# juno181/Ex4DGS

Hardware: AMD Instinct MI355X
Metric: fwd+bwd ms/frame @1M Gaussians 1352x1014; achieved HBM GB/s vs peak (lower is better)
Workload: dtype f32; 1 GPU; cfg3: 1.0M static+dynamic (K=35), 1352x1014; P=1000000, HW=1370928, sh_degree=3, step=GaussianRasterizer forward + backward on a resident frame, parallelism=frame-sharded x1

## Files before the change

### ex4dgs_amd/build.py

```python
import os
import shutil
import subprocess
import sys

from . import isa_check

HERE = os.path.dirname(os.path.abspath(__file__))
CSRC = os.path.join(HERE, "csrc")
LIB = os.path.join(CSRC, "libex4d_hip.so")
ARCH = "gfx950"

SOURCES = {
    "ex4d_preprocess.hip": ["-ffp-contract=off", "-fno-slp-vectorize"],
    "ex4d_binning.hip": [],
    "ex4d_rowsort.hip": [],
    "ex4d_composite.hip": ["-ffp-contract=fast", "-munsafe-fp-atomics", "-fno-slp-vectorize"],
    "ex4d_api.hip": [],
    "ex4d_attributes.hip": ["-ffp-contract=off"],
    "ex4d_loss.hip": [],
    "ex4d_frames.hip": ["-ffp-contract=off"],
    "ex4d_optim.hip": ["-ffp-contract=off"],
    "ex4d_knn.hip": ["-ffp-contract=off"],
    "ex4d_densify.hip": ["-ffp-contract=off"],
    "ex4d_growth.hip": ["-ffp-contract=off"],
    "ex4d_regularizers.hip": ["-ffp-contract=off"],
    "ex4d_trainer.hip": [],
}
COMMON = ["-O3", "-std=c++17", "-fPIC", f"--offload-arch={ARCH}", "-fno-fast-math", "-Wall", "-Wno-unused-function"]


def _hipcc():
    for cand in (shutil.which("hipcc"), "/opt/rocm/bin/hipcc"):
        if cand and os.path.exists(cand):
            return cand
    raise RuntimeError("hipcc not found: libex4d_hip.so cannot be built")


def _without_remarks(text):
    out, skip = [], 0
    for line in text.splitlines():
        if "-Rpass-analysis=kernel-resource-usage" in line:
            skip = 2
            continue
        if skip and (line.strip().startswith("|") or line.split("|")[0].strip().isdigit()):
            skip -= 1
            continue
        skip = 0
        if "remark" in line and "generated" in line:
            continue
        out.append(line + "\n")
    return "".join(out)


def _no_vgpr_spills(src, remarks, obj):
    name, bad = None, []
    for line in remarks.splitlines():
        if "Function Name:" in line:
            name = line.split("Function Name:")[1].split("[")[0].strip()
        elif "VGPRs Spill:" in line:
            n = int(line.split("VGPRs Spill:")[1].split("[")[0])
            if n:
                bad.append((name, n))
    if bad:
        if os.path.exists(obj):
            os.remove(obj)
        raise RuntimeError(f"{src}: vector-register spills in {bad}: restructure the kernel or relax its __launch_bounds__")


shift_amount_in_last_vgpr = isa_check.shift_amount_in_last_vgpr


def _no_shift_amount_in_last_vgpr(src, obj):
    bad = shift_amount_in_last_vgpr(obj)
    if bad:
        os.remove(obj)
        raise RuntimeError(f"{src}: 64-bit shifts with their shift amount in the wave's last vector register (wrong results on gfx950 for waves "
                           f"allocated at the top of the register file): {bad}; change the kernel's __launch_bounds__ / register pressure")


def _no_packed_shift_clamps(src, obj):
    bad = isa_check.packed_shift_clamps(obj)
    if bad:
        os.remove(obj)
        raise RuntimeError(f"{src}: v_ashr_pk_* (its destination's upper 16 bits are used as zero and are not, on gfx950): {bad}; clamp the "
                           f"accumulator before the shift")


def _report_wait_state_violations(src, obj):
    bad = isa_check.wait_state_violations(obj)
    for kernel, rule, cons, prod in bad[:20]:
        sys.stderr.write(f"{src}: wait states: {rule}: `{prod}` -> `{cons}` in {kernel[:60]}\n")
    return bad


def _stale(target, deps):
    if not os.path.exists(target):
        return True
    t = os.path.getmtime(target)
    return any(os.path.getmtime(d) > t for d in deps)


def build(force=False, verbose=False, extra_flags=()):
    hipcc = _hipcc()
    headers = [os.path.join(CSRC, "ex4d_internal.h"), os.path.join(HERE, "..", "include", "ex4d_rasterizer.h"),
               os.path.join(HERE, "..", "include", "ex4d_attributes.h"), os.path.join(HERE, "..", "include", "ex4d_loss.h"), os.path.join(HERE, "..", "include", "ex4d_optim.h"), os.path.join(HERE, "..", "include", "ex4d_knn.h"), os.path.join(HERE, "..", "include", "ex4d_trainer.h"),
               os.path.join(HERE, "..", "include", "ex4d_densify.h"), os.path.join(HERE, "..", "include", "ex4d_regularizers.h"),
               os.path.join(CSRC, "ex4d_reg_rows.h"),
               os.path.abspath(__file__)]
    objs = []
    for src, flags in SOURCES.items():
        s = os.path.join(CSRC, src)
        o = os.path.join(CSRC, src.replace(".hip", ".o"))
        objs.append(o)
        if force or _stale(o, [s] + headers):
            cmd = [hipcc] + COMMON + flags + list(extra_flags) + os.environ.get("EX4D_EXTRA_HIPCC_FLAGS", "").split() + \
                  ["-Rpass-analysis=kernel-resource-usage", "-c", s, "-o", o]
            if verbose:
                print(" ".join(cmd), flush=True)
            r = subprocess.run(cmd, stderr=subprocess.PIPE, text=True)
            remarks = r.stderr or ""
            sys.stderr.write(_without_remarks(remarks))
            if r.returncode:
                raise subprocess.CalledProcessError(r.returncode, cmd)
            _no_vgpr_spills(src, remarks, o)
            _no_shift_amount_in_last_vgpr(src, o)
            _no_packed_shift_clamps(src, o)
            _report_wait_state_violations(src, o)
    if force or _stale(LIB, objs):
        cmd = [hipcc, "-shared", "-fPIC", f"--offload-arch={ARCH}", "-o", LIB] + objs
        if verbose:
            print(" ".join(cmd), flush=True)
        subprocess.check_call(cmd)
    return LIB


if __name__ == "__main__":
    print(build(force="--force" in sys.argv, verbose=True))
```

### ex4dgs_amd/csrc/ex4d_api.hip

```cpp
#include "ex4d_internal.h"
#include <atomic>
#include <cstdarg>
#include <cstdio>
#include <cstdlib>
#include <cstring>
#include <mutex>

namespace {

std::atomic<bool> g_prof_on{false};
std::atomic<int> g_bwd_variant{4};
std::atomic<int> g_tile_ids{0};
std::atomic<int> g_tile_rows{1};
std::atomic<int> g_depth_msd{3};
struct DepthSortWatch {
    std::mutex mu;
    uint32_t *word = nullptr;
    bool tried = false;
    std::atomic<int> hold{0}, backoff{64}, trips{0};
    uint32_t *get()
    {
        std::lock_guard<std::mutex> lock(mu);
        if (!tried) {
            tried = true;
// ... 225 lines not shown
const char *ex4d_target_arch(void) { return "gfx950"; }

size_t ex4d_geom_bytes(int32_t P) { size_t t; carve_geom(nullptr, P, nullptr, &t); return t; }
size_t ex4d_binning_bytes(int32_t R, int32_t W, int32_t H) { size_t t; carve_binning(nullptr, (uint32_t)R, W, H, nullptr, &t); return t; }
size_t ex4d_img_bytes(int32_t W, int32_t H) { size_t t; carve_img(nullptr, W, H, nullptr, &t); return t; }
void ex4d_geom_layout(int32_t P, Ex4dGeomLayout *out) { carve_geom(nullptr, P, out, nullptr); }
void ex4d_binning_layout(int32_t R, int32_t W, int32_t H, Ex4dBinningLayout *out) { carve_binning(nullptr, (uint32_t)R, W, H, out, nullptr); }
void ex4d_img_layout(int32_t W, int32_t H, Ex4dImgLayout *out) { carve_img(nullptr, W, H, out, nullptr); }
size_t ex4d_backward_scratch_bytes(int32_t P) { return ex4d_align_up((size_t)P * 16 * sizeof(float)); }

static int forward_impl(
    const Ex4dParams *prm, ShSplit split,
    const float *background, const float *means3D, const float *dir3D, const float *shs, const float *colors_precomp,
    const float *opacities, const float *scales, const float *rotations, const float *cov3D_precomp,
    const float *viewmatrix, const float *projmatrix, const float *campos, const float *subpixel_offset,
    ex4d_alloc_fn geom_alloc, void *geom_user, ex4d_alloc_fn binning_alloc, void *binning_user,
    ex4d_alloc_fn img_alloc, void *img_user,
    float *out_color, int32_t *radii, float *out_depth, float *out_acc, float *out_flow, int32_t *out_idx,
    void *stream_, int32_t *num_rendered)
{
    g_err[0] = 0;
    hipStream_t stream = (hipStream_t)stream_;
    if (!prm || !num_rendered) return fail(EX4D_ERR_ARG, "null params");
    const int P = prm->P, W = prm->W, H = prm->H;
    if (P <= 0 || W <= 0 || H <= 0) return fail(EX4D_ERR_ARG, "P, W, H must be positive (P == 0 is handled by the caller)");
    if (!means3D || !opacities || !background || !viewmatrix || !projmatrix || !campos)
        return fail(EX4D_ERR_ARG, "means3D, opacities, background, viewmatrix, projmatrix, campos are required");
    const bool is_split = split.rest[0] != nullptr || split.rest[1] != nullptr;
    if (((shs != nullptr || is_split) ? 1 : 0) + (colors_precomp != nullptr ? 1 : 0) != 1 || (shs != nullptr && is_split))
        return fail(EX4D_ERR_ARG, "Please provide excatly one of either SHs or precomputed colors!");
    if (is_split && prm->M != 16) return fail(EX4D_ERR_ARG, "split SH needs M == 16 (dc [n,1,3] + rest [n,15,3])");
    if (((scales == nullptr || rotations == nullptr) && cov3D_precomp == nullptr) ||
        ((scales != nullptr || rotations != nullptr) && cov3D_precomp != nullptr))
        return fail(EX4D_ERR_ARG, "Please provide exactly one of either scale/rotation pair or precomputed 3D covariance!");
    if (shs && prm->M < (prm->D + 1) * (prm->D + 1)) return fail(EX4D_ERR_ARG, "sh has fewer coefficients than the active degree needs");
    if (!out_color || !radii || !out_depth || !out_acc || !out_flow || !out_idx) return fail(EX4D_ERR_ARG, "null output");
    const int gx = (W + EX4D_TILE - 1) / EX4D_TILE, gy = (H + EX4D_TILE - 1) / EX4D_TILE;
    const int T = gx * gy;
    const bool async = prm->instance_capacity > 0;
    if (prm->instance_capacity < 0) return fail(EX4D_ERR_ARG, "instance_capacity must be >= 0");
    if (async && prm->debug) return fail(EX4D_ERR_ARG, "debug (synchronise after every stage) and instance_capacity > 0 (asynchronous forward) exclude each other");

    void *geom_buf = geom_alloc(geom_user, ex4d_geom_bytes(P));
    if (!geom_buf) return fail(EX4D_ERR_ALLOC, "geometry buffer allocation failed");
    GeomState g = carve_geom(geom_buf, P, nullptr, nullptr);
    void *img_buf = img_alloc(img_user, ex4d_img_bytes(W, H));
    if (!img_buf) return fail(EX4D_ERR_ALLOC, "image buffer allocation failed");
    ImgState im = carve_img(img_buf, W, H, nullptr, nullptr);

    uint32_t key_base = 0, key_invisible = 0xFFFFFFFFu;
    int key_bits = 32;
    if (prm->min_depth >= 0.0f && prm->max_depth > prm->min_depth && prm->max_depth < 3.0e38f) {
        uint32_t lo, hi;
        memcpy(&lo, &prm->min_depth, 4); memcpy(&hi, &prm->max_depth, 4);
        key_base = lo;
        key_invisible = hi - lo + 1u;
        key_bits = 1;
        while (key_bits < 32 && (key_invisible >> key_bits) != 0u) key_bits++;
    }
    const bool packed_rects = gx <= 255 && gy <= 255;
    int msd_mode = g_depth_msd.load(std::memory_order_relaxed);
    uint32_t *msd_watch = nullptr;
    if (!(packed_rects && ex4d_depth_sort_msd_applies((uint32_t)P, key_bits))) msd_mode = 0;
    else if (msd_mode == 3) msd_mode = depth_sort_auto_msd(stream, async, &msd_watch) ? 2 : 0;
    const bool msd_depth = msd_mode != 0;
    int msd_bits = ex4d_depth_sort_msd_bits((uint32_t)P, key_bits);
    {
        const int forced = g_depth_msd_bits.load(std::memory_order_relaxed);
        if (forced == EX4D_DLS_MSD_BITS || (forced == EX4D_DLS_MSD_BITS - 1 && ex4d_depth_sort_msd_bits(1u, key_bits) == forced)) msd_bits = forced;
    }
    const bool start_in_b = (ex4d_radix_passes((uint32_t)P, key_bits) & 1) != 0;
    uint32_t *keys0 = start_in_b ? g.sort_keys_b : g.sort_keys_a, *vals0 = start_in_b ? g.sort_vals_b : g.depth_order;
    uint32_t *keys1 = start_in_b ? g.sort_keys_a : g.sort_keys_b, *vals1 = start_in_b ? g.depth_order : g.sort_vals_b;
    if (msd_depth) { keys0 = g.sort_keys_a; vals0 = g.sort_vals_a; }

    HIP_TRY(ex4d_prepare_rank_lds(stream));
    g_prof.begin(0, stream);
    if (async) HIP_TRY(ex4d_launch_zero(g.total, 8 * sizeof(uint32_t), stream));
    GeomState gw = g;
    if (!g_geom_debug.load(std::memory_order_relaxed)) {
        gw.cov3D = nullptr; gw.tiles_touched = nullptr;
        if (packed_rects) gw.rects = nullptr;
    }
    STAGE(ex4d_launch_preprocess_fwd(*prm, means3D, dir3D, scales, rotations, opacities, shs, cov3D_precomp, colors_precomp,
                                     viewmatrix, projmatrix, campos, radii, gw, g.total + 1, split,
                                     keys0, (uint32_t *)nullptr, key_base, key_invisible, packed_rects ? g.rects4 : nullptr, stream,
                                     msd_depth ? reinterpret_cast<uint32_t *>(g.key_ranges) : nullptr, async), prm, stream);
    MARK(0, "preprocess_fwd");
    const size_t nblk = (size_t)(P + 63) / 64;
    const size_t rb_words = (size_t)(g.block_totals - g.total) + 2 * nblk;
    if (!async) {
        if (!g_readback.init(rb_words)) return fail(EX4D_ERR_HIP, "pinned read-back buffer allocation failed");
        if (g_readback_side.load(std::memory_order_relaxed)) {
            HIP_TRY(hipEventRecord(g_readback.ev_pre, stream));
            HIP_TRY(hipStreamWaitEvent(g_readback.side, g_readback.ev_pre, 0));
            HIP_TRY(hipMemcpyAsync(g_readback.host, g.total, rb_words * sizeof(uint32_t), hipMemcpyDeviceToHost, g_readback.side));
            HIP_TRY(hipEventRecord(g_readback.ev, g_readback.side));
        } else {
            HIP_TRY(hipMemcpyAsync(g_readback.host, g.total, rb_words * sizeof(uint32_t), hipMemcpyDeviceToHost, stream));
            HIP_TRY(hipEventRecord(g_readback.ev, stream));
        }
    }
    const bool rows_sort = g_tile_rows.load(std::memory_order_relaxed) != 0 && ex4d_tile_sort_rows_applies(P, gx, gy);
    const bool fused_scan = msd_mode == 2 && !rows_sort;
    const bool lsd_gather = !msd_depth && rows_sort && packed_rects;
    if (msd_depth) {
        STAGE(ex4d_depth_sort_msd(g.sort_keys_a, g.sort_vals_a, g.rects4, g.sort_keys_b, g.depth_order, g.rects4_b, (uint32_t)P, key_invisible,
                                  g.total, g.key_ranges, g.sort_hist, g.bucket_starts, (uint32_t)g_depth_local_cap.load(std::memory_order_relaxed), stream,
                                  fused_scan ? g.sorted_offsets : nullptr, fused_scan ? g.bucket_sums : nullptr, T, (fused_scan || rows_sort) ? im.ranges : nullptr,
                                  g_depth_local_threads.load(std::memory_order_relaxed), msd_watch, msd_bits), prm, stream);
        MARK(0, "depth_sort");
        if (!fused_scan && !rows_sort) {
            STAGE(ex4d_launch_scan_tiles(P, nullptr, g.rects4_b, nullptr, nullptr, g.sorted_offsets, g.scan_block_sums, T, im.ranges, async ? g.total : nullptr, stream), prm, stream);
            MARK(0, "scan_tiles");
        }
    } else {
        bool in_first = true;
        STAGE(ex4d_radix_sort_pairs(keys0, vals0, keys1, vals1, (uint32_t)P, key_bits, g.sort_hist, &in_first, stream, nullptr, true,
                                    lsd_gather ? g.rects4 : nullptr, lsd_gather ? g.rects4_b : nullptr, lsd_gather ? im.ranges : nullptr, T), prm, stream);
        if (in_first == start_in_b) return fail(EX4D_ERR_HIP, "internal: depth sort ended in the wrong buffer");
        MARK(0, "depth_sort");
        if (!lsd_gather) {
            STAGE(ex4d_launch_scan_tiles(P, g.rects, packed_rects ? g.rects4 : nullptr, g.depth_order, g.sorted_rects, g.sorted_offsets, g.scan_block_sums, T, im.ranges, async ? g.total : nullptr, stream), prm, stream);
            MARK(0, "scan_tiles");
        }
    }
    const uint2 *dup_rects = (msd_depth || lsd_gather) ? nullptr : g.sorted_rects;
    const uint32_t *dup_rects4 = (msd_depth || lsd_gather) ? g.rects4_b : nullptr;
    uint32_t R = 0;
    uint32_t segment_sum = 0;
    const uint32_t *n_dev = nullptr;
    bool has_flow;
    if (async) {
        static_assert(sizeof(Ex4dFrameStatus) == 8 * sizeof(uint32_t), "Ex4dFrameStatus mirrors the first eight frame-flag words");
        const bool count_later = fused_scan || (rows_sort && msd_depth) || lsd_gather;
        if (!count_later) HIP_TRY(hipMemcpyAsync(num_rendered, g.total, sizeof(Ex4dFrameStatus), hipMemcpyDefault, stream));
        R = (uint32_t)prm->instance_capacity;
        segment_sum = 0;
        n_dev = g.total;
        has_flow = prm->assume_no_flow == 0;
    } else {
        {
            static const bool spin = []{ const char *e = getenv("EX4D_READBACK_SPIN"); return e ? atoi(e) != 0 : true; }();
            if (spin) {
                hipError_t q = hipErrorNotReady;
                for (int i = 0; i < 20000 && (q = hipEventQuery(g_readback.ev)) == hipErrorNotReady; i++) { }
                if (q == hipErrorNotReady) q = hipEventSynchronize(g_readback.ev);
                HIP_TRY(q);
            } else HIP_TRY(hipEventSynchronize(g_readback.ev));
        }
        uint32_t instance_sum = 0;
        uint32_t chunk_flags = 0;
        for (size_t i = 0; i < nblk; i++) {
            const uint32_t seg = g_readback.host[(size_t)(g.block_totals - g.total) + 2 * i + 1];
            instance_sum += g_readback.host[(size_t)(g.block_totals - g.total) + 2 * i];
            segment_sum += seg & 0x3FFFFFFFu;
            chunk_flags |= seg;
        }
        has_flow = (chunk_flags & EX4D_CHUNK_FLOW) != 0u;
        if (prm->prefiltered && (chunk_flags & EX4D_CHUNK_FILTERED))
            return fail(EX4D_ERR_PREFILTERED, "Point is filtered although prefiltered is set. This shouldn't happen!");
        R = instance_sum;
        if (R > 0x7FFFFFFFu) return fail(EX4D_ERR_ARG, "more than 2^31-1 tile instances");
        *num_rendered = (int32_t)R;
    }

    void *bin_buf = binning_alloc(binning_user, ex4d_binning_bytes((int32_t)R, W, H));
    if (!bin_buf) return fail(EX4D_ERR_ALLOC, "binning buffer allocation failed");
    BinState b = carve_binning(bin_buf, R, W, H, nullptr, nullptr);

    const int passes = ex4d_radix_passes(R, tile_bits(T));
    uint32_t *k0 = (passes % 2 == 0) ? b.tile_ids : b.keys_tmp;
    uint32_t *v0 = (passes % 2 == 0) ? b.point_list : b.vals_tmp;
    uint32_t *k1 = (passes % 2 == 0) ? b.keys_tmp : b.tile_ids;
    uint32_t *v1 = (passes % 2 == 0) ? b.vals_tmp : b.point_list;
    if (rows_sort) {
        if (R > 0) {
            STAGE(ex4d_tile_sort_rows(P, gx, gy, g.depth_order, dup_rects4, dup_rects, b.keys_tmp, b.point_list,
                                      g_tile_ids.load(std::memory_order_relaxed) ? b.tile_ids : nullptr, R, segment_sum, g.row_hist, b.sort_hist, im.ranges,
                                      (async && (msd_depth || lsd_gather)) ? g.total : nullptr, stream), prm, stream);
        }
        if (async && (msd_depth || lsd_gather)) HIP_TRY(hipMemcpyAsync(num_rendered, g.total, sizeof(Ex4dFrameStatus), hipMemcpyDefault, stream));
        MARK(0, "tile_sort");
    } else if (R > 0 && ex4d_tile_sort_msd_applies(P, tile_bits(T))) {
        STAGE(ex4d_launch_duplicate(P, W, H, g.depth_order, g.sorted_offsets, g.scan_block_sums, dup_rects, dup_rects4, b.tile_ids, b.vals_tmp, R, stream,
                                    fused_scan ? g.sort_keys_b : nullptr, g.total + EX4D_FLAG_DPARAMS, g.bucket_sums, g.total, msd_bits), prm, stream);
        if (async && fused_scan) HIP_TRY(hipMemcpyAsync(num_rendered, g.total, sizeof(Ex4dFrameStatus), hipMemcpyDefault, stream));
        MARK(0, "duplicate");
        STAGE(ex4d_tile_sort_msd(b.tile_ids, b.vals_tmp, b.keys_tmp, b.point_list, g_tile_ids.load(std::memory_order_relaxed) ? b.tile_ids : nullptr,
                                 R, tile_bits(T), b.sort_hist, im.ranges, stream, n_dev), prm, stream);
        MARK(0, "tile_sort");
        MARK(0, "tile_ranges");
    } else {
// ... 74 lines not shown
                        viewmatrix, projmatrix, campos, subpixel_offset, geom_alloc, geom_user, binning_alloc, binning_user,
                        img_alloc, img_user, out_color, radii, out_depth, out_acc, out_flow, out_idx, stream_, num_rendered);
}

static bool split_ok(const Ex4dParams *prm, const float *const dc[2], const float *const rest[2], int n_static)
{
    if (!prm || n_static < 0 || n_static > prm->P) return false;
    if (n_static > 0 && (!dc[0] || !rest[0])) return false;
    if (n_static < prm->P && (!dc[1] || !rest[1])) return false;
    return true;
}

int ex4d_forward_split_sh(
    const Ex4dParams *prm, const float *background, const float *means3D, const float *dir3D, const Ex4dSplitSH *shs,
    const float *opacities, const float *scales, const float *rotations, const float *cov3D_precomp,
    const float *viewmatrix, const float *projmatrix, const float *campos, const float *subpixel_offset,
    ex4d_alloc_fn geom_alloc, void *geom_user, ex4d_alloc_fn binning_alloc, void *binning_user,
    ex4d_alloc_fn img_alloc, void *img_user,
    float *out_color, int32_t *radii, float *out_depth, float *out_acc, float *out_flow, int32_t *out_idx,
    void *stream_, int32_t *num_rendered)
{
    g_err[0] = 0;
    if (!shs || !split_ok(prm, shs->dc, shs->rest, shs->n_static)) return fail(EX4D_ERR_ARG, "split SH: null tensor or n_static outside [0, P]");
    const ShSplit sp = { { shs->dc[0], shs->dc[1] }, { shs->rest[0], shs->rest[1] }, shs->n_static };
    return forward_impl(prm, sp, background, means3D, dir3D, nullptr, nullptr, opacities, scales, rotations, cov3D_precomp,
                        viewmatrix, projmatrix, campos, subpixel_offset, geom_alloc, geom_user, binning_alloc, binning_user,
                        img_alloc, img_user, out_color, radii, out_depth, out_acc, out_flow, out_idx, stream_, num_rendered);
}

int ex4d_backward(
    const Ex4dParams *prm, int32_t num_rendered,
    const float *background, const float *means3D, const int32_t *radii,
    const float *shs, const float *colors_precomp, const float *scales, const float *rotations,
    const float *cov3D_precomp, const float *viewmatrix, const float *projmatrix, const float *campos,
    const float *subpixel_offset, const float *out_depth, const float *out_acc,
    const void *geom_buffer, const void *binning_buffer, const void *img_buffer,
    const float *dL_dout_color, const float *dL_dout_depth, const float *dL_dout_flow, const float *dL_dout_acc,
    float *dL_dmeans2D, float *dL_dcolors, float *dL_dopacity, float *dL_dmeans3D, float *dL_dcov3D, float *dL_dsh,
    float *dL_dscales, float *dL_drotations, float *dL_ddir, void *bwd_scratch, void *stream_)
{
    return backward_impl(prm, kNoSplit, kNoSplitGrad, num_rendered, background, means3D, radii, shs, colors_precomp, scales, rotations,
                         cov3D_precomp, viewmatrix, projmatrix, campos, subpixel_offset, out_depth, out_acc, geom_buffer, binning_buffer,
                         img_buffer, dL_dout_color, dL_dout_depth, dL_dout_flow, dL_dout_acc, dL_dmeans2D, dL_dcolors, dL_dopacity,
                         dL_dmeans3D, dL_dcov3D, dL_dsh, dL_dscales, dL_drotations, dL_ddir, bwd_scratch, stream_);
}

int ex4d_backward_split_sh(
    const Ex4dParams *prm, int32_t num_rendered,
    const float *background, const float *means3D, const int32_t *radii,
    const Ex4dSplitSH *shs, const float *scales, const float *rotations,
    const float *cov3D_precomp, const float *viewmatrix, const float *projmatrix, const float *campos,
    const float *subpixel_offset, const float *out_depth, const float *out_acc,
    const void *geom_buffer, const void *binning_buffer, const void *img_buffer,
    const float *dL_dout_color, const float *dL_dout_depth, const float *dL_dout_flow, const float *dL_dout_acc,
    float *dL_dmeans2D, float *dL_dcolors, float *dL_dopacity, float *dL_dmeans3D, float *dL_dcov3D, const Ex4dSplitSHGrad *dL_dsh,
    float *dL_dscales, float *dL_drotations, float *dL_ddir, void *bwd_scratch, void *stream_)
{
    g_err[0] = 0;
    if (!shs || !dL_dsh || !split_ok(prm, shs->dc, shs->rest, shs->n_static) || dL_dsh->n_static != shs->n_static ||
        !split_ok(prm, (const float *const *)dL_dsh->dc, (const float *const *)dL_dsh->rest, dL_dsh->n_static))
        return fail(EX4D_ERR_ARG, "split SH: null tensor, n_static outside [0, P] or mismatching gradient split");
    if (prm->M != 16) return fail(EX4D_ERR_ARG, "split SH needs M == 16 (dc [n,1,3] + rest [n,15,3])");
    const ShSplit sp = { { shs->dc[0], shs->dc[1] }, { shs->rest[0], shs->rest[1] }, shs->n_static };
    const ShSplitGrad gsp = { { dL_dsh->dc[0], dL_dsh->dc[1] }, { dL_dsh->rest[0], dL_dsh->rest[1] }, dL_dsh->n_static };
    return backward_impl(prm, sp, gsp, num_rendered, background, means3D, radii, nullptr, nullptr, scales, rotations,
                         cov3D_precomp, viewmatrix, projmatrix, campos, subpixel_offset, out_depth, out_acc, geom_buffer, binning_buffer,
                         img_buffer, dL_dout_color, dL_dout_depth, dL_dout_flow, dL_dout_acc, dL_dmeans2D, dL_dcolors, dL_dopacity,
                         dL_dmeans3D, dL_dcov3D, nullptr, dL_dscales, dL_drotations, dL_ddir, bwd_scratch, stream_);
}

int ex4d_set_option(const char *name, int value)
{
    if (name && !strcmp(name, "composite_bwd_variant") && (value == 4 || value == 8)) { g_bwd_variant.store(value); return EX4D_OK; }
    if (name && !strcmp(name, "composite_fwd_asm") && (value == 0 || value == 1)) { ex4d_set_fwd_asm(value); return EX4D_OK; }
    if (name && !strcmp(name, "binning_tile_ids") && (value == 0 || value == 1)) { g_tile_ids.store(value); return EX4D_OK; }
    if (name && !strcmp(name, "composite_clamp_always") && (value == 0 || value == 1)) { ex4d_set_clamp_always(value); return EX4D_OK; }
    if (name && !strcmp(name, "composite_bwd_pairs") && (value == 0 || value == 1)) { ex4d_set_bwd_pairs(value); return EX4D_OK; }
    if (name && !strcmp(name, "tile_sort_rows") && (value == 0 || value == 1)) { g_tile_rows.store(value); return EX4D_OK; }
    if (name && !strcmp(name, "rank_lds_atomics") && value >= -1 && value <= 1) { ex4d_set_rank_lds(value); return EX4D_OK; }
    if (name && !strcmp(name, "rows_probe")) { ex4d_set_rows_probe(value); return EX4D_OK; }
    if (name && !strcmp(name, "preprocess_sh_predicate") && (value == 0 || value == 1)) { ex4d_set_preprocess_tune(value); return EX4D_OK; }
    if (name && !strcmp(name, "geom_debug_arrays") && (value == 0 || value == 1)) { g_geom_debug.store(value); return EX4D_OK; }
    if (name && !strcmp(name, "preprocess_fast_path") && (value == 0 || value == 1)) { ex4d_set_preprocess_fast(value); return EX4D_OK; }
    if (name && !strcmp(name, "depth_sort_msd") && value >= 0 && value <= 3) { g_depth_msd.store(value); g_depth_watch.reset(); return EX4D_OK; }
    if (name && !strcmp(name, "depth_sort_local_cap") && value >= 0 && value <= 8192) { g_depth_local_cap.store(value); return EX4D_OK; }
    if (name && !strcmp(name, "readback_side_stream") && (value == 0 || value == 1)) { g_readback_side.store(value); return EX4D_OK; }
    if (name && !strcmp(name, "depth_sort_msd_bits") && (value == 0 || value == EX4D_DLS_MSD_BITS - 1 || value == EX4D_DLS_MSD_BITS)) { g_depth_msd_bits.store(value); return EX4D_OK; }
    if (name && !strcmp(name, "depth_sort_local_threads") && (value == 0 || value == 256 || value == 512)) { g_depth_local_threads.store(value); return EX4D_OK; }
    return fail(EX4D_ERR_ARG, "unknown option or value out of range");
}

int ex4d_debug_bwd_stats(unsigned long long *out8, int reset) { return ex4d_bwd_stats(out8, 8, reset) == hipSuccess ? EX4D_OK : EX4D_ERR_HIP; }
int ex4d_debug_rows_prof(unsigned long long *out8, int reset) { return ex4d_rows_prof(out8, reset) == hipSuccess ? EX4D_OK : EX4D_ERR_HIP; }
int ex4d_debug_bwd_stats16(unsigned long long *out16, int reset) { return ex4d_bwd_stats(out16, 16, reset) == hipSuccess ? EX4D_OK : EX4D_ERR_HIP; }

int ex4d_get_option(const char *name)
{
    if (name && !strcmp(name, "composite_bwd_variant")) return g_bwd_variant.load();
    if (name && !strcmp(name, "composite_fwd_asm")) return ex4d_get_fwd_asm();
    if (name && !strcmp(name, "binning_tile_ids")) return g_tile_ids.load();
    if (name && !strcmp(name, "composite_clamp_always")) return ex4d_get_clamp_always();
    if (name && !strcmp(name, "composite_bwd_pairs")) return ex4d_get_bwd_pairs();
    if (name && !strcmp(name, "tile_sort_rows")) return g_tile_rows.load();
    if (name && !strcmp(name, "rank_lds_atomics")) return ex4d_get_rank_lds();
    if (name && !strcmp(name, "rank_lds_atomics_in_use")) return ex4d_rank_lds_in_use();
    if (name && !strcmp(name, "preprocess_sh_predicate")) return ex4d_get_preprocess_tune();
    if (name && !strcmp(name, "geom_debug_arrays")) return g_geom_debug.load();
    if (name && !strcmp(name, "preprocess_fast_path")) return ex4d_get_preprocess_fast();
    if (name && !strcmp(name, "depth_sort_msd")) return g_depth_msd.load();
    if (name && !strcmp(name, "depth_sort_hold")) return g_depth_watch.hold.load();
    if (name && !strcmp(name, "depth_sort_trips")) return g_depth_watch.trips.load();
    if (name && !strcmp(name, "depth_sort_local_cap")) return g_depth_local_cap.load();
    if (name && !strcmp(name, "readback_side_stream")) return g_readback_side.load();
    if (name && !strcmp(name, "depth_sort_msd_bits")) return g_depth_msd_bits.load();
    if (name && !strcmp(name, "depth_sort_local_threads")) return g_depth_local_threads.load();
    return -1;
}

void ex4d_profile_enable(int on) { g_prof_on.store(on != 0); }

int ex4d_profile_read(int which, float *ms, const char **names, int max_stages)
{
    std::lock_guard<std::mutex> lock(g_prof.mu);
    if (which < 0 || which > 1 || !g_prof.created) return 0;
    const int n = g_prof.n[which] < max_stages ? g_prof.n[which] : max_stages;
    if (n == 0) return 0;
    if (hipEventSynchronize(g_prof.ev[which][g_prof.n[which]]) != hipSuccess) return 0;
    for (int i = 0; i < n; i++) {
        float t = 0.f;
        (void)hipEventElapsedTime(&t, g_prof.ev[which][i], g_prof.ev[which][i + 1]);
        ms[i] = t;
        if (names) names[i] = g_prof.names[which][i];
    }
    return n;
}

int ex4d_mark_visible(int32_t P, const float *means3D, const float *viewmatrix, const float *projmatrix,
                      float min_depth, float max_depth, uint8_t *present, void *stream_)
{
    g_err[0] = 0;
    if (P <= 0) return EX4D_OK;
    if (!means3D || !viewmatrix || !projmatrix || !present) return fail(EX4D_ERR_ARG, "null argument");
    HIP_TRY(ex4d_launch_mark_visible(P, means3D, viewmatrix, projmatrix, min_depth, max_depth, present, (hipStream_t)stream_));
    return EX4D_OK;
}

}
```

### ex4dgs_amd/csrc/ex4d_binning.hip

```cpp
#include "ex4d_internal.h"
#include <atomic>
#include <mutex>

__device__ int ex4d_g_rank_lds = 0;

namespace {

__global__ __launch_bounds__(256) void lds_rank_probe_kernel(uint32_t seed, int trials, int ndigits, uint32_t *__restrict__ bad)
{
    __shared__ uint32_t cnt[4][256];
    const int lane = threadIdx.x & 63, wave = threadIdx.x >> 6;
    uint32_t x = seed ^ (blockIdx.x * 0x9E3779B9u) ^ (threadIdx.x * 0x85EBCA6Bu);
    uint32_t nb = 0;
    for (int t = 0; t < trials; t++) {
        for (int i = lane; i < 256; i += 64) cnt[wave][i] = 0;
        __builtin_amdgcn_fence(__ATOMIC_RELEASE, "wavefront"); __builtin_amdgcn_wave_barrier(); __builtin_amdgcn_fence(__ATOMIC_ACQUIRE, "wavefront");
        x = x * 1664525u + 1013904223u;
        const uint32_t d = (x >> 16) % (uint32_t)ndigits;
        uint32_t expect = 0, same = 0;
        for (int l = 0; l < 64; l++) { const uint32_t dl = __shfl(d, l, 64); if (dl == d) { same++; if (l < lane) expect++; } }
        const uint32_t got = atomicAdd(&cnt[wave][d], 1u);
        const uint32_t got2 = atomicAdd(&cnt[wave][d], 1u);
        if (got != expect || got2 != same + expect) nb++;
    }
    if (nb) atomicAdd(bad, nb);
}

__device__ __forceinline__ int to_int_sat(float f)
{
    if (f != f) return 0;
    if (f >= 2147483648.0f) return 2147483647;
    if (f <= -2147483648.0f) return (-2147483647 - 1);
    return (int)f;
}

template <int ITEMS, int BINS, int COPIES>
__global__ __launch_bounds__(RS_THREADS) void rs_histogram_kernel(const uint32_t *__restrict__ keys, uint32_t n, int shift,
    uint32_t mask, uint32_t nblocks, uint32_t *__restrict__ hist, const uint32_t *__restrict__ n_dev)
{
    if (n_dev) { const uint32_t nd = *n_dev; n = nd < n ? nd : n; }
    __shared__ uint32_t h_all[COPIES * (BINS + 1)];
    uint32_t *h = h_all + (COPIES > 1 ? (threadIdx.x % COPIES) * (BINS + 1) : 0);
    for (int b = threadIdx.x; b < COPIES * (BINS + 1); b += RS_THREADS) h_all[b] = 0;
    __syncthreads();
    const uint32_t base = blockIdx.x * (RS_THREADS * ITEMS);
    if (base < n) {
        uint32_t k[ITEMS];
#pragma unroll
        for (int it = 0; it < ITEMS; it++) {
            const uint32_t i = base + it * RS_THREADS + threadIdx.x;
            k[it] = keys[i < n ? i : n - 1];
        }
#pragma unroll
        for (int it = 0; it < ITEMS; it++) {
            const uint32_t i = base + it * RS_THREADS + threadIdx.x;
            if (i < n) atomicAdd(&h[(k[it] >> shift) & mask], 1u);
        }
    }
    __syncthreads();
    for (int b = threadIdx.x; b < BINS; b += RS_THREADS) {
        uint32_t c = 0;
#pragma unroll
        for (int k = 0; k < COPIES; k++) c += h_all[k * (BINS + 1) + b];
        hist[(size_t)b * nblocks + blockIdx.x] = c;
    }
}

__global__ __launch_bounds__(256) void rs_scan_rows_kernel(uint32_t nblocks, uint32_t *__restrict__ hist, uint32_t bins)
{
    __shared__ uint32_t wave_sums[4];
    __shared__ uint32_t carry_s;
    uint32_t *row = hist + (size_t)blockIdx.x * nblocks;
    const int lane = threadIdx.x & 63, wave = threadIdx.x >> 6;
    const bool vec = ((((uintptr_t)row) & 15) == 0);
    if (threadIdx.x == 0) carry_s = 0;
    __syncthreads();
    for (uint32_t base = 0; base < nblocks; base += 2048) {
        const uint32_t i0 = base + 8 * threadIdx.x;
        uint32_t v[8];
        if (vec && i0 + 8 <= nblocks) {
            const uint4 a = *reinterpret_cast<const uint4 *>(row + i0), b = *reinterpret_cast<const uint4 *>(row + i0 + 4);
            v[0] = a.x; v[1] = a.y; v[2] = a.z; v[3] = a.w; v[4] = b.x; v[5] = b.y; v[6] = b.z; v[7] = b.w;
        } else {
#pragma unroll
            for (int k = 0; k < 8; k++) v[k] = (i0 + k < nblocks) ? row[i0 + k] : 0u;
        }
        uint32_t run = 0;
#pragma unroll
        for (int k = 0; k < 8; k++) { const uint32_t t = v[k]; v[k] = run; run += t; }
        uint32_t x = run;
#pragma unroll
        for (int o = 1; o < 64; o <<= 1) { uint32_t y = __shfl_up(x, o, 64); if (lane >= o) x += y; }
        if (lane == 63) wave_sums[wave] = x;
        __syncthreads();
        uint32_t woff = carry_s + x - run;
        for (int w = 0; w < wave; w++) woff += wave_sums[w];
        if (vec && i0 + 8 <= nblocks) {
            *reinterpret_cast<uint4 *>(row + i0) = make_uint4(woff + v[0], woff + v[1], woff + v[2], woff + v[3]);
            *reinterpret_cast<uint4 *>(row + i0 + 4) = make_uint4(woff + v[4], woff + v[5], woff + v[6], woff + v[7]);
        } else {
#pragma unroll
            for (int k = 0; k < 8; k++) if (i0 + k < nblocks) row[i0 + k] = woff + v[k];
        }
        __syncthreads();
        if (threadIdx.x == 255) carry_s = woff + run;
        __syncthreads();
    }
    if (threadIdx.x == 0) hist[(size_t)bins * nblocks + blockIdx.x] = carry_s;
}

struct DlsParams { uint32_t kmin, shift, inv_key; };
__device__ __forceinline__ DlsParams dls_params(const uint32_t *__restrict__ dparams) { return { dparams[0], dparams[1], dparams[2] }; }
__device__ __forceinline__ uint32_t dls_digit(uint32_t key, const DlsParams &q, uint32_t bins) { return key == q.inv_key ? bins - 1u : (key - q.kmin) >> q.shift; }

__device__ __forceinline__ DlsParams dls_reduce_ranges(const uint2 *__restrict__ ranges, uint32_t nranges, uint32_t inv_key, uint32_t bins, uint32_t *s_red )
{
    uint32_t kmax = 0u, nkmin = 0u;
    for (uint32_t base = 0; base < nranges; base += 8u * RS_THREADS) {
        uint2 p[8];
#pragma unroll
        for (int j = 0; j < 8; j++) { const uint32_t i = base + j * RS_THREADS + threadIdx.x; p[j] = i < nranges ? ranges[i] : make_uint2(0u, 0u); }
#pragma unroll
        for (int j = 0; j < 8; j++) { kmax = p[j].x > kmax ? p[j].x : kmax; nkmin = p[j].y > nkmin ? p[j].y : nkmin; }
    }
#pragma unroll
    for (int o = 32; o > 0; o >>= 1) {
        const uint32_t a = __shfl_xor(kmax, o, 64), b = __shfl_xor(nkmin, o, 64);
        kmax = a > kmax ? a : kmax; nkmin = b > nkmin ? b : nkmin;
    }
    if ((threadIdx.x & 63) == 0) { s_red[threadIdx.x >> 6] = kmax; s_red[4 + (threadIdx.x >> 6)] = nkmin; }
    __syncthreads();
    for (int w = 0; w < RS_THREADS / 64; w++) { kmax = s_red[w] > kmax ? s_red[w] : kmax; nkmin = s_red[4 + w] > nkmin ? s_red[4 + w] : nkmin; }
    uint32_t kmin = ~nkmin, shift = 0;
    if (kmax == 0u) kmin = 0u;
    else {
        const uint32_t range = kmax - kmin;
        while ((range >> shift) > bins - 2u) shift++;
    }
    return { kmin, shift, inv_key };
}

template <int ITEMS, int BINS>
__global__ __launch_bounds__(RS_THREADS) void dls_histogram_kernel(const uint32_t *__restrict__ keys, uint32_t n, uint32_t nblocks,
    uint32_t *__restrict__ hist, uint32_t *__restrict__ dparams, const uint2 *__restrict__ ranges, uint32_t nranges, uint32_t inv_key)
{
    __shared__ uint32_t h[BINS];
    __shared__ uint32_t s_red[8];
    for (int b = threadIdx.x; b < BINS; b += RS_THREADS) h[b] = 0;
    const uint32_t base = blockIdx.x * (RS_THREADS * ITEMS);
    uint32_t k[ITEMS];
    if (base < n) {
#pragma unroll
        for (int it = 0; it < ITEMS; it++) {
            const uint32_t i = base + it * RS_THREADS + threadIdx.x;
            k[it] = keys[i < n ? i : n - 1];
        }
    }
    const DlsParams q = dls_reduce_ranges(ranges, nranges, inv_key, (uint32_t)BINS, s_red);
    if (blockIdx.x == 0 && threadIdx.x == 0) { dparams[0] = q.kmin; dparams[1] = q.shift; dparams[2] = q.inv_key; dparams[3] = 0u; }
    if (base < n) {
#pragma unroll
        for (int it = 0; it < ITEMS; it++) {
            const uint32_t i = base + it * RS_THREADS + threadIdx.x;
            if (i < n) atomicAdd(&h[dls_digit(k[it], q, BINS)], 1u);
        }
    }
    __syncthreads();
    for (int b = threadIdx.x; b < BINS; b += RS_THREADS) hist[(size_t)b * nblocks + blockIdx.x] = h[b];
}

typedef Ex4dTsBlock TsBlock;
__device__ __forceinline__ TsBlock ts_block_from_table(const Ex4dTsBlock *__restrict__ table, uint32_t b)
{
    const uint2 *p = reinterpret_cast<const uint2 *>(table + b);
    const uint2 a = p[0], c = p[1], e = p[2];
    return { a.x, a.y, c.x, c.y, e.x, e.y };
}
struct TsLocateLds { uint32_t cnt[257], fb[257], st[257], wave_sums[8]; };
__device__ __forceinline__ TsBlock ts_locate_block(const uint32_t *__restrict__ totals, int nbuckets, uint32_t b, TsLocateLds &L)
{
    const int tid = threadIdx.x, lane = tid & 63, wave = tid >> 6;
    const uint32_t cnt = tid < nbuckets ? totals[tid] : 0u;
    const uint32_t nblk = (cnt + RS_CHUNK - 1) / RS_CHUNK;
    uint32_t x = cnt, y = nblk;
#pragma unroll
    for (int o = 1; o < 64; o <<= 1) { const uint32_t a = __shfl_up(x, o, 64), c = __shfl_up(y, o, 64); if (lane >= o) { x += a; y += c; } }
    if (lane == 63) { L.wave_sums[wave] = x; L.wave_sums[4 + wave] = y; }
    __syncthreads();
    uint32_t st = x - cnt, fb = y - nblk;
    for (int w = 0; w < wave; w++) { st += L.wave_sums[w]; fb += L.wave_sums[4 + w]; }
    L.cnt[tid] = cnt; L.fb[tid] = fb; L.st[tid] = st;
    if (tid == 255) { L.fb[256] = fb + nblk; L.st[256] = st + cnt; L.cnt[256] = 0; }
    __syncthreads();
    TsBlock t = { 0u, 0u, 0u, 0u, 0u, 0u };
    if (b < L.fb[256]) {
        uint32_t h = 0;
#pragma unroll
        for (uint32_t step = 128; step > 0; step >>= 1) if (L.fb[h + step] <= b) h += step;
        const uint32_t within = (b - L.fb[h]) * RS_CHUNK;
        t.start = L.st[h] + within;
        t.count = L.cnt[h] - within < RS_CHUNK ? L.cnt[h] - within : RS_CHUNK;
        t.bucket = h; t.fb_first = L.fb[h]; t.fb_next = L.fb[h + 1]; t.bucket_start = L.st[h];
    }
    return t;
}
template <int ITEMS, int BINS, int MODE, int NBITS>
__global__ __launch_bounds__(RS_THREADS) void rs_scatter_kernel(const uint32_t *__restrict__ keys_in,
    const uint32_t *__restrict__ vals_in, uint32_t *__restrict__ keys_out, uint32_t *__restrict__ vals_out,
    uint32_t n, int shift, int nbits, uint32_t nblocks, const uint32_t *__restrict__ hist,
    int low_bits, const uint32_t *__restrict__ bucket_totals, int nbuckets, uint2 *__restrict__ ranges, const uint32_t *__restrict__ n_dev,
    const uint32_t *__restrict__ rects_in = nullptr, uint32_t *__restrict__ rects_out = nullptr, uint32_t *__restrict__ bucket_starts = nullptr,
    const uint32_t *__restrict__ dparams = nullptr, uint32_t range_stride = 0, uint32_t out_cap = 0xFFFFFFFFu,
    const Ex4dTsBlock *__restrict__ block_table = nullptr)
{
    if (n_dev) { const uint32_t nd = *n_dev; n = nd < n ? nd : n; }
    if (MODE == 0 && ranges) for (uint32_t i = blockIdx.x * RS_THREADS + threadIdx.x; i < range_stride; i += gridDim.x * RS_THREADS) ranges[i] = make_uint2(0u, 0u);
    if (MODE != 2 && blockIdx.x * (uint32_t)(RS_THREADS * ITEMS) >= n) return;
    __shared__ uint32_t wave_cnt[4][BINS];
    __shared__ uint32_t local_start[BINS];
    __shared__ uint32_t global_base[BINS];
    __shared__ uint32_t scan_tmp[8];
    constexpr int STAGE_WORDS = (MODE == 2 ? 1 : 2) * RS_THREADS * ITEMS;
    __shared__ __attribute__((aligned(16))) uint32_t stage_w[STAGE_WORDS];
    uint2 *const stage = reinterpret_cast<uint2 *>(stage_w);
    __shared__ uint32_t stage_r[MODE == 3 ? RS_THREADS * ITEMS : 1];
    static_assert(sizeof(TsLocateLds) <= sizeof(uint32_t) * STAGE_WORDS, "the block table's scratch lives in the staging area");
    static_assert(sizeof(uint32_t) * (4 * BINS + 2 * BINS + 8) + sizeof(uint32_t) * STAGE_WORDS + sizeof(uint32_t) * (MODE == 3 ? RS_THREADS * ITEMS : 1) <= 80 * 1024,
                  "rs_scatter_kernel: static LDS beyond 80 KB (two workgroups per CU)");
    const int tid = threadIdx.x, lane = tid & 63, wave = tid >> 6;
    if (NBITS > 0) nbits = NBITS;
    const uint32_t mask = (1u << nbits) - 1u;
    const int nbins = 1 << nbits;
    DlsParams dq = { 0u, 0u, 0u };
    if (MODE == 3) dq = dls_params(dparams);
    auto digit_of = [&](uint32_t k) -> uint32_t { return MODE == 3 ? dls_digit(k, dq, (uint32_t)BINS) : ((k >> shift) & mask); };
    for (int i = lane; i < BINS; i += 64) wave_cnt[wave][i] = 0;
    __builtin_amdgcn_fence(__ATOMIC_RELEASE, "wavefront");
    __builtin_amdgcn_wave_barrier();
    __builtin_amdgcn_fence(__ATOMIC_ACQUIRE, "wavefront");

    const bool lds_rank = ex4d_g_rank_lds != 0;
    constexpr uint32_t CHUNK = RS_THREADS * ITEMS;
    uint32_t block_first = blockIdx.x * CHUNK, block_end = n, bucket = 0;
    TsBlock tb = { 0u, 0u, 0u, 0u, 0u, 0u };
    if (MODE == 2) {
        if (block_table) tb = ts_block_from_table(block_table, blockIdx.x);
        else {
            TsLocateLds &loc = *reinterpret_cast<TsLocateLds *>(stage_w);
            tb = ts_locate_block(bucket_totals, nbuckets, blockIdx.x, loc);
            __syncthreads();
        }
        if (tb.count == 0) return;
        block_first = tb.start; block_end = tb.start + tb.count; bucket = tb.bucket;
        if (block_first >= out_cap) return;
        if (block_end > out_cap) block_end = out_cap;
    }
    const uint32_t base = block_first + wave * (CHUNK / 4);
    const uint64_t lt = (1ull << lane) - 1ull;
    constexpr int BPT_PRE = BINS / RS_THREADS;
    uint32_t pre_pf[BPT_PRE], pre_gt[BPT_PRE], pre_hb[BPT_PRE];
#pragma unroll
    for (int k = 0; k < BPT_PRE; k++) {
        const int d = tid * BPT_PRE + k;
        const bool live = d < nbins;
        if (MODE == 2) {
            pre_pf[k] = live ? hist[(size_t)d * nblocks + tb.fb_first] : 0u;
            pre_gt[k] = live ? hist[(size_t)d * nblocks + tb.fb_next] : 0u;
        } else {
            pre_pf[k] = 0u;
            pre_gt[k] = live ? hist[(size_t)BINS * nblocks + d] : 0u;
        }
        pre_hb[k] = live ? hist[(size_t)d * nblocks + blockIdx.x] : 0u;
    }
    uint32_t key[ITEMS], val[ITEMS], pos[ITEMS], rct[MODE == 3 ? ITEMS : 1];
#pragma unroll
    for (int it = 0; it < ITEMS; it++) {
        const uint32_t i = base + it * 64 + lane;
        const uint32_t ic = i < block_end ? i : block_end - 1;
        key[it] = keys_in[ic];
        val[it] = (MODE == 2) ? 0u : (vals_in ? vals_in[ic] : ic);
        if constexpr (MODE == 3) rct[it] = rects_in[ic];
    }
#pragma unroll
    for (int it = 0; it < ITEMS; it++) {
        const uint32_t i = base + it * 64 + lane;
        const bool valid = i < block_end;
        const uint32_t d = digit_of(key[it]);
        if (lds_rank) {
            pos[it] = valid ? atomicAdd(&wave_cnt[wave][d], 1u) : 0u;
            continue;
        }
        const uint64_t vmask = __builtin_amdgcn_ballot_w64(valid);
        uint32_t plo = (uint32_t)vmask, phi = (uint32_t)(vmask >> 32);
        if (NBITS > 0) {
#pragma unroll
            for (int b = 0; b < NBITS; b++) {
                const uint64_t bal = __builtin_amdgcn_ballot_w64((d & (1u << b)) != 0u);
                uint32_t flip;
                asm("v_cndmask_b32_e64 %0, -1, 0, %1" : "=v"(flip) : "s"(bal));
                plo &= (uint32_t)bal ^ flip;
                phi &= (uint32_t)(bal >> 32) ^ flip;
            }
        } else {
            for (int b = 0; b < nbits; b++) {
                const uint32_t bit = (d >> b) & 1u;
                const uint64_t bal = __builtin_amdgcn_ballot_w64(bit != 0u);
                const uint32_t flip = bit - 1u;
                plo &= (uint32_t)bal ^ flip;
                phi &= (uint32_t)(bal >> 32) ^ flip;
            }
// ... 229 lines not shown
        lo += nbits;
    }
    if (sv != xv) {
        for (uint32_t i = tid; i < n; i += DLS_THREADS) { xv[i] = sv[i]; xr[i] = sr[i]; }
    }
}

__device__ __forceinline__ uint32_t rect4_count(uint32_t r) { return ((r >> 16) & 0xFFu) * (r >> 24); }
template <int THREADS>
__device__ __forceinline__ uint32_t dls_scan_chunk(DlsLds<THREADS> &L, uint32_t cn, uint32_t carry)
{
    constexpr int DLS_WAVES = THREADS / 64;
    const int tid = threadIdx.x, lane = tid & 63, wave = tid >> 6;
    uint32_t v[DLS_ITEMS], run = 0;
#pragma unroll
    for (int q = 0; q < DLS_ITEMS; q++) { const uint32_t i = tid * DLS_ITEMS + q; run += (i < cn) ? L.buf[i] : 0u; v[q] = run; }
    uint32_t x = run;
#pragma unroll
    for (int o = 1; o < 64; o <<= 1) { const uint32_t y = __shfl_up(x, o, 64); if (lane >= o) x += y; }
    if (lane == 63) L.scan_tmp[wave] = x;
    __syncthreads();
    uint32_t excl = carry + x - run, total = 0;
    for (int w = 0; w < DLS_WAVES; w++) { const uint32_t t = L.scan_tmp[w]; if (w < wave) excl += t; total += t; }
#pragma unroll
    for (int q = 0; q < DLS_ITEMS; q++) { const uint32_t i = tid * DLS_ITEMS + q; if (i < cn) L.buf[i] = excl + v[q]; }
    __syncthreads();
    return total;
}
template <int THREADS>
__device__ __forceinline__ uint32_t dls_scan_from_memory(DlsLds<THREADS> &L, const uint32_t *rects, uint32_t *local_incl, uint32_t n)
{
    constexpr int DLS_THREADS = THREADS, DLS_CAP = THREADS * DLS_ITEMS;
    const int tid = threadIdx.x;
    uint32_t carry = 0;
    for (uint32_t c0 = 0; c0 < n; c0 += DLS_CAP) {
        const uint32_t cn = (n - c0) < DLS_CAP ? (n - c0) : DLS_CAP;
        uint32_t r[DLS_ITEMS];
#pragma unroll
        for (int j = 0; j < DLS_ITEMS; j++) { const uint32_t p = tid + j * DLS_THREADS; r[j] = p < cn ? rects[c0 + p] : 0u; }
#pragma unroll
        for (int j = 0; j < DLS_ITEMS; j++) { const uint32_t p = tid + j * DLS_THREADS; if (p < cn) L.buf[p] = rect4_count(r[j]); }
        __syncthreads();
        carry += dls_scan_chunk(L, cn, carry);
#pragma unroll
        for (int j = 0; j < DLS_ITEMS; j++) { const uint32_t p = tid + j * DLS_THREADS; if (p < cn) local_incl[c0 + p] = L.buf[p]; }
        __syncthreads();
    }
    return carry;
}

template <int THREADS, int NBITS>
__device__ __forceinline__ void dls_lds_pass(DlsLds<THREADS> &L, uint32_t n, uint32_t m, int sh, int nbits)
{
    const int tid = threadIdx.x, lane = tid & 63, wave = tid >> 6;
    if (NBITS > 0) nbits = NBITS;
    const uint32_t mask = (1u << nbits) - 1u;
    const uint32_t wbase = wave * m;
    for (int i = lane; i < (1 << nbits); i += 64) L.cnt[wave][i] = 0;
    dls_wave_sync();
    uint32_t word[DLS_ITEMS], pos[DLS_ITEMS];
#pragma unroll
    for (int it = 0; it < DLS_ITEMS; it++) {
        word[it] = 0u; pos[it] = 0u;
        if ((uint32_t)(it * 64) < m) {
            const uint32_t i = wbase + it * 64 + lane;
            const bool valid = i < n;
            word[it] = valid ? L.buf[i] : 0u;
            pos[it] = dls_rank<NBITS>(L.cnt[wave], (word[it] >> sh) & mask, nbits, valid, lane);
        }
    }
    __syncthreads();
    dls_scan_counts(L, nbits);
#pragma unroll
    for (int it = 0; it < DLS_ITEMS; it++) {
        if ((uint32_t)(it * 64) < m) {
            const uint32_t i = wbase + it * 64 + lane;
            if (i < n) L.buf[L.cnt[wave][(word[it] >> sh) & mask] + pos[it]] = word[it];
        }
    }
    __syncthreads();
}

template <int THREADS>
__global__ __launch_bounds__(THREADS, THREADS == 512 ? 4 : 5) void depth_local_sort_kernel(uint32_t *kb, uint32_t *vb, uint32_t *rb, uint32_t *ka, uint32_t *va, uint32_t *ra,
    const uint32_t *__restrict__ starts, const uint32_t *__restrict__ totals, const uint32_t *__restrict__ dparams, uint32_t cap,
    uint32_t *__restrict__ local_incl, uint32_t *__restrict__ bucket_sums, int T, uint2 *__restrict__ ranges, uint32_t *__restrict__ watch)
{
    constexpr int DLS_THREADS = THREADS, DLS_WAVES = THREADS / 64, DLS_CAP = THREADS * DLS_ITEMS, IDX_BITS = DlsLds<THREADS>::IDX_BITS;
    __shared__ DlsLds<THREADS> L;
    const uint32_t b = blockIdx.x;
    const int tid = threadIdx.x;
    if (ranges) for (int i = b * DLS_THREADS + tid; i < T; i += gridDim.x * DLS_THREADS) ranges[i] = make_uint2(0u, 0u);
    const uint32_t n = totals[b], s = starts[b];
    const DlsParams dq = dls_params(dparams);
    const int rem = (int)dq.shift;
    const uint32_t inv_digit = gridDim.x - 1u;
    if (b == inv_digit || n == 0u) {
        if (bucket_sums && tid == 0) bucket_sums[b] = 0u;
        return;
    }
    const bool sorted_already = n < 2u || rem == 0;
    if (sorted_already || n > cap) {
        if (n > cap && watch && tid == 0) __hip_atomic_store(watch, 1u, __ATOMIC_RELAXED, __HIP_MEMORY_SCOPE_SYSTEM);
        if (!sorted_already) {
            dls_sort_through_memory(L, kb + s, vb + s, rb + s, ka + s, va + s, ra + s, n, rem, dq.kmin); __threadfence(); __syncthreads();
        }
        if (local_incl) {
            const uint32_t sum = dls_scan_from_memory(L, rb + s, local_incl + s, n);
            if (tid == 0) bucket_sums[b] = sum;
        }
        return;
    }
    const uint32_t remmask = (1u << rem) - 1u;
    {
        uint32_t k[DLS_ITEMS];
#pragma unroll
        for (int j = 0; j < DLS_ITEMS; j++) { const uint32_t p = tid + j * DLS_THREADS; k[j] = p < n ? kb[s + p] : 0u; }
#pragma unroll
        for (int j = 0; j < DLS_ITEMS; j++) { const uint32_t p = tid + j * DLS_THREADS; if (p < n) L.buf[p] = (((k[j] - dq.kmin) & remmask) << IDX_BITS) | p; }
    }
    __syncthreads();
    const int npass = (rem + 8) / 9;
    const uint32_t m = ((n + DLS_WAVES * 64 - 1) / (DLS_WAVES * 64)) * 64;
    if (rem == 16) { dls_lds_pass<THREADS, 8>(L, n, m, IDX_BITS, 8); dls_lds_pass<THREADS, 8>(L, n, m, IDX_BITS + 8, 8); }
    else if (rem == 17) { dls_lds_pass<THREADS, 9>(L, n, m, IDX_BITS, 9); dls_lds_pass<THREADS, 8>(L, n, m, IDX_BITS + 9, 8); }
    else {
        for (int pass = 0, lo = 0; pass < npass; pass++) {
            const int nbits = dls_pass_bits(rem, lo, npass, pass);
            dls_lds_pass<THREADS, 0>(L, n, m, IDX_BITS + lo, nbits);
            lo += nbits;
        }
    }
    uint32_t v[DLS_ITEMS], r[DLS_ITEMS];
#pragma unroll
    for (int j = 0; j < DLS_ITEMS; j++) {
        const uint32_t p = tid + j * DLS_THREADS;
        v[j] = 0u; r[j] = 0u;
        if (p < n) { const uint32_t idx = L.buf[p] & (DLS_CAP - 1u); v[j] = vb[s + idx]; r[j] = rb[s + idx]; }
    }
    asm volatile("s_waitcnt vmcnt(0)" ::: "memory");
    __syncthreads();
#pragma unroll
    for (int j = 0; j < DLS_ITEMS; j++) {
        const uint32_t p = tid + j * DLS_THREADS;
        if (p < n) { vb[s + p] = v[j]; rb[s + p] = r[j]; if (local_incl) L.buf[p] = rect4_count(r[j]); }
    }
    if (local_incl) {
        __syncthreads();
        const uint32_t sum = dls_scan_chunk(L, n, 0u);
#pragma unroll
        for (int j = 0; j < DLS_ITEMS; j++) { const uint32_t p = tid + j * DLS_THREADS; if (p < n) local_incl[s + p] = L.buf[p]; }
        if (tid == 0) bucket_sums[b] = sum;
    }
}

__device__ __forceinline__ uint2 unpack_rect(uint32_t p) { return make_uint2((p & 0xFFu) | (((p >> 8) & 0xFFu) << 16), ((p >> 16) & 0xFFu) | ((p >> 24) << 16)); }
__global__ __launch_bounds__(256) void scan_tiles_local_kernel(int P, const uint2 *__restrict__ rects, const uint32_t *__restrict__ rects4,
    const uint32_t *__restrict__ order, uint2 *__restrict__ sorted_rects, uint32_t *__restrict__ out, uint32_t *__restrict__ block_sums,
    int T, uint2 *__restrict__ ranges, uint32_t *__restrict__ frame_total)
{
    for (int i = blockIdx.x * 256 + threadIdx.x; i < T; i += gridDim.x * 256) ranges[i] = make_uint2(0u, 0u);
    __shared__ uint32_t cnt[SCAN_CHUNK];
    __shared__ uint32_t wave_sums[4];
    const int lane = threadIdx.x & 63, wave = threadIdx.x >> 6;
    const int block_first = blockIdx.x * SCAN_CHUNK;
#pragma unroll
    for (int it = 0; it < SCAN_CHUNK / 256; it++) {
        const int i = block_first + it * 256 + threadIdx.x;
        uint2 rc = make_uint2(0u, 0u);
        if (i < P) { rc = rects4 ? unpack_rect(rects4[order ? order[i] : (uint32_t)i]) : rects[order[i]]; if (sorted_rects) sorted_rects[i] = rc; }
        cnt[it * 256 + threadIdx.x] = (rc.y & 0xFFFFu) * (rc.y >> 16);
    }
    __syncthreads();
    uint32_t v[8];
    uint32_t run = 0;
#pragma unroll
    for (int k = 0; k < 8; k++) { run += cnt[threadIdx.x * 8 + k]; v[k] = run; }
    uint32_t x = run;
#pragma unroll
// ... 120 lines not shown
}

__global__ __launch_bounds__(256) void zero_fill_kernel(uint4 *__restrict__ p, size_t n16, uint32_t tail_words)
{
    const uint4 z = make_uint4(0u, 0u, 0u, 0u);
    for (size_t i = (size_t)blockIdx.x * 256 + threadIdx.x; i < n16; i += (size_t)gridDim.x * 256) p[i] = z;
    if (blockIdx.x == 0 && threadIdx.x < tail_words) reinterpret_cast<uint32_t *>(p + n16)[threadIdx.x] = 0u;
}

__global__ __launch_bounds__(256) void tile_ranges_kernel(uint32_t R, const uint32_t *__restrict__ tile_ids, uint2 *__restrict__ ranges,
    const uint32_t *__restrict__ n_dev)
{
    if (n_dev) { const uint32_t nd = *n_dev; R = nd < R ? nd : R; }
    const uint32_t i = blockIdx.x * 256 + threadIdx.x;
    if (i >= R) return;
    const uint32_t cur = tile_ids[i];
    if (i == 0) ranges[cur].x = 0;
    else {
        const uint32_t prev = tile_ids[i - 1];
        if (cur != prev) { ranges[prev].y = i; ranges[cur].x = i; }
    }
    if (i == R - 1) ranges[cur].y = R;
}

}

static std::atomic<int> g_rank_lds_option{-1};
static std::mutex g_rank_lds_mu;
static int g_rank_lds_device = -1, g_rank_lds_value = 0;
void ex4d_set_rank_lds(int v) { std::lock_guard<std::mutex> lock(g_rank_lds_mu); g_rank_lds_option.store(v); g_rank_lds_device = -1; }
int ex4d_get_rank_lds() { return g_rank_lds_option.load(); }
int ex4d_rank_lds_in_use() { return g_rank_lds_value; }
hipError_t ex4d_prepare_rank_lds(hipStream_t stream)
{
    int dev = -1;
    if (hipGetDevice(&dev) != hipSuccess) return hipGetLastError();
    std::lock_guard<std::mutex> lock(g_rank_lds_mu);
    if (dev == g_rank_lds_device) return hipSuccess;
    hipStreamCaptureStatus st = hipStreamCaptureStatusNone;
    if (hipStreamIsCapturing(stream, &st) == hipSuccess && st != hipStreamCaptureStatusNone) return hipSuccess;
    (void)hipGetLastError();
    int want = g_rank_lds_option.load();
    if (want < 0) {
        uint32_t *bad = nullptr, h = 1;
        hipError_t e = hipMalloc((void **)&bad, sizeof(uint32_t));
        if (e != hipSuccess) return e;
        (void)hipMemset(bad, 0, sizeof(uint32_t));
        for (int nd : { 1, 3, 17, 64, 256 })
            hipLaunchKernelGGL(lds_rank_probe_kernel, dim3(256), dim3(256), 0, 0, 0x5EEDu + nd, 200, nd, bad);
        e = hipMemcpy(&h, bad, sizeof(uint32_t), hipMemcpyDeviceToHost);
        (void)hipFree(bad);
        if (e != hipSuccess) return e;
        want = h == 0u ? 1 : 0;
    }
    hipError_t e = hipMemcpyToSymbol(HIP_SYMBOL(ex4d_g_rank_lds), &want, sizeof(int));
    if (e != hipSuccess) return e;
    g_rank_lds_device = dev; g_rank_lds_value = want;
    return hipSuccess;
}

#define RS_SMALL_ITEMS 8
static inline int rs_items_for(uint32_t n) { return n <= (2u << 20) ? RS_SMALL_ITEMS : RS_ITEMS; }
static inline uint32_t rs_blocks_for(uint32_t n) { const uint32_t c = RS_THREADS * rs_items_for(n); return (n + c - 1) / c; }
static inline int rs_max_bits_for(uint32_t n) { return rs_items_for(n) == RS_SMALL_ITEMS ? 9 : 8; }
size_t ex4d_radix_hist_words(uint32_t n) { return (size_t)1024 * rs_blocks_for(n) + 1024; }
int ex4d_radix_passes(uint32_t n, int end_bit) { const int mb = rs_max_bits_for(n); return (end_bit + mb - 1) / mb; }

hipError_t ex4d_radix_sort_pairs(uint32_t *keys_a, uint32_t *vals_a, uint32_t *keys_b, uint32_t *vals_b,
    uint32_t n, int end_bit, uint32_t *hist, bool *result_in_a, hipStream_t stream, const uint32_t *n_dev, bool iota_values,
    const uint32_t *gather_in, uint32_t *gather_out, uint2 *zero_ranges, int num_ranges)
{
    *result_in_a = true;
    if (n == 0) return hipSuccess;
    const uint32_t nb = rs_blocks_for(n);
    const bool small = rs_items_for(n) == RS_SMALL_ITEMS;
    uint32_t *kin = keys_a, *vin = iota_values ? nullptr : vals_a, *kout = keys_b, *vout = vals_b;
    uint32_t *vnext = vals_a;
    const int npass = ex4d_radix_passes(n, end_bit);
    for (int pass = 0, shift = 0; pass < npass; pass++) {
        const int nbits = (end_bit - shift + (npass - pass) - 1) / (npass - pass);
        const uint32_t mask = (1u << nbits) - 1u;
        if (small) {
            hipLaunchKernelGGL((rs_histogram_kernel<RS_SMALL_ITEMS, 512, 1>), dim3(nb), dim3(RS_THREADS), 0, stream, kin, n, shift, mask, nb, hist, n_dev);
            hipLaunchKernelGGL(rs_scan_rows_kernel, dim3(1u << nbits), dim3(256), 0, stream, nb, hist, 512u);
            const bool last = pass == npass - 1;
#define RS_SMALL_SCATTER(NB) hipLaunchKernelGGL((rs_scatter_kernel<RS_SMALL_ITEMS, 512, 0, NB>), dim3(nb), dim3(RS_THREADS), 0, stream, kin, vin, kout, vout, n, shift, nbits, nb, hist, 0, nullptr, 0, \
                last ? zero_ranges : (uint2 *)nullptr, n_dev, last ? gather_in : (const uint32_t *)nullptr, last ? gather_out : (uint32_t *)nullptr, (uint32_t *)nullptr, (const uint32_t *)nullptr, (uint32_t)num_ranges)
            if (nbits == 9) RS_SMALL_SCATTER(9); else if (nbits == 8) RS_SMALL_SCATTER(8); else RS_SMALL_SCATTER(0);
#undef RS_SMALL_SCATTER
        } else {
            hipLaunchKernelGGL((rs_histogram_kernel<RS_ITEMS, 256, 1>), dim3(nb), dim3(RS_THREADS), 0, stream, kin, n, shift, mask, nb, hist, n_dev);
            hipLaunchKernelGGL(rs_scan_rows_kernel, dim3(1u << nbits), dim3(256), 0, stream, nb, hist, 256u);
            const bool last = pass == npass - 1;
            hipLaunchKernelGGL((rs_scatter_kernel<RS_ITEMS, 256, 0, 0>), dim3(nb), dim3(RS_THREADS), 0, stream, kin, vin, kout, vout, n, shift, nbits, nb, hist, 0, nullptr, 0,
                last ? zero_ranges : (uint2 *)nullptr, n_dev, last ? gather_in : (const uint32_t *)nullptr, last ? gather_out : (uint32_t *)nullptr, (uint32_t *)nullptr, (const uint32_t *)nullptr, (uint32_t)num_ranges);
        }
        uint32_t *t = kin; kin = kout; kout = t;
        t = (pass == 0) ? vnext : vin; vin = vout; vout = t;
        *result_in_a = !*result_in_a;
        shift += nbits;
    }
    return hipGetLastError();
}

bool ex4d_depth_sort_msd_applies(uint32_t n, int key_bits) { return n <= (1u << 26) && key_bits - (EX4D_DLS_MSD_BITS - 1) + DLS_IDX_BITS <= 32; }
int ex4d_depth_sort_msd_bits(uint32_t n, int key_bits)
{
    const int narrow = EX4D_DLS_MSD_BITS - 1;
    return (n <= 1300000u && key_bits - (narrow - 1) + DLS_IDX_BITS <= 32) ? narrow : EX4D_DLS_MSD_BITS;
}
template <int MB>
static hipError_t depth_sort_msd_launch(uint32_t *ka, uint32_t *va, uint32_t *ra, uint32_t *kb, uint32_t *vb, uint32_t *rb, uint32_t n, uint32_t inv_key,
    uint32_t *flags, const uint2 *wave_ranges, uint32_t *hist, uint32_t *starts, uint32_t local_cap, hipStream_t stream,
    uint32_t *local_incl, uint32_t *bucket_sums, int T, uint2 *ranges, int local_threads, uint32_t *watch)
{
    if (n == 0) return hipSuccess;
    constexpr int BINS = 1 << MB;
    const uint32_t nb = rs_blocks_for(n);
    const bool small = rs_items_for(n) == RS_SMALL_ITEMS;
    uint32_t *dparams = flags + EX4D_FLAG_DPARAMS;
    const uint32_t nranges = (n + 255u) / 256u;
    if (local_threads != 256 && local_threads != 512) local_threads = (MB < EX4D_DLS_MSD_BITS || n > 1200000u) ? 512 : 256;
    const uint32_t kcap = (uint32_t)local_threads * DLS_ITEMS;
    if (local_cap == 0 || local_cap > kcap) local_cap = kcap;
    if (small) {
        hipLaunchKernelGGL((dls_histogram_kernel<RS_SMALL_ITEMS, BINS>), dim3(nb), dim3(RS_THREADS), 0, stream, ka, n, nb, hist, dparams, wave_ranges, nranges, inv_key);
        hipLaunchKernelGGL(rs_scan_rows_kernel, dim3(BINS), dim3(256), 0, stream, nb, hist, (uint32_t)BINS);
        hipLaunchKernelGGL((rs_scatter_kernel<RS_SMALL_ITEMS, BINS, 3, MB>), dim3(nb), dim3(RS_THREADS), 0, stream, ka, (const uint32_t *)nullptr, kb, vb, n, 0, MB, nb, hist,
            0, (const uint32_t *)nullptr, 0, (uint2 *)nullptr, (const uint32_t *)nullptr, ra, rb, starts, (const uint32_t *)dparams);
    } else {
        hipLaunchKernelGGL((dls_histogram_kernel<RS_ITEMS, BINS>), dim3(nb), dim3(RS_THREADS), 0, stream, ka, n, nb, hist, dparams, wave_ranges, nranges, inv_key);
        hipLaunchKernelGGL(rs_scan_rows_kernel, dim3(BINS), dim3(256), 0, stream, nb, hist, (uint32_t)BINS);
        hipLaunchKernelGGL((rs_scatter_kernel<RS_ITEMS, BINS, 3, MB>), dim3(nb), dim3(RS_THREADS), 0, stream, ka, (const uint32_t *)nullptr, kb, vb, n, 0, MB, nb, hist,
            0, (const uint32_t *)nullptr, 0, (uint2 *)nullptr, (const uint32_t *)nullptr, ra, rb, starts, (const uint32_t *)dparams);
    }
    if (local_threads == 256)
        hipLaunchKernelGGL(depth_local_sort_kernel<256>, dim3(BINS), dim3(256), 0, stream, kb, vb, rb, ka, va, ra, starts, hist + (size_t)BINS * nb, (const uint32_t *)dparams, local_cap,
            local_incl, bucket_sums, T, ranges, watch);
    else
        hipLaunchKernelGGL(depth_local_sort_kernel<512>, dim3(BINS), dim3(512), 0, stream, kb, vb, rb, ka, va, ra, starts, hist + (size_t)BINS * nb, (const uint32_t *)dparams, local_cap,
            local_incl, bucket_sums, T, ranges, watch);
    return hipGetLastError();
}

hipError_t ex4d_depth_sort_msd(uint32_t *ka, uint32_t *va, uint32_t *ra, uint32_t *kb, uint32_t *vb, uint32_t *rb, uint32_t n, uint32_t inv_key,
    uint32_t *flags, const uint2 *wave_ranges, uint32_t *hist, uint32_t *starts, uint32_t local_cap, hipStream_t stream,
    uint32_t *local_incl, uint32_t *bucket_sums, int T, uint2 *ranges, int local_threads, uint32_t *watch, int msd_bits)
{
    if (msd_bits == EX4D_DLS_MSD_BITS - 1)
        return depth_sort_msd_launch<EX4D_DLS_MSD_BITS - 1>(ka, va, ra, kb, vb, rb, n, inv_key, flags, wave_ranges, hist, starts, local_cap, stream, local_incl, bucket_sums, T, ranges, local_threads, watch);
    return depth_sort_msd_launch<EX4D_DLS_MSD_BITS>(ka, va, ra, kb, vb, rb, n, inv_key, flags, wave_ranges, hist, starts, local_cap, stream, local_incl, bucket_sums, T, ranges, local_threads, watch);
}

bool ex4d_tile_sort_msd_applies(int P, int tile_bits)
{
    if (tile_bits < 9 || tile_bits > 16) return false;
    const int low_bits = (tile_bits + 1) / 2;
    return (uint64_t)P <= (1ull << (32 - low_bits));
}
static inline int ts_clamp_bits(int tile_bits) { return tile_bits > 16 ? 16 : (tile_bits < 2 ? 2 : tile_bits); }
static inline uint32_t ts_max_blocks(uint32_t R, int tile_bits) { return rs_num_blocks(R) + (1u << (tile_bits - (tile_bits + 1) / 2)) + 1u; }
size_t ex4d_tile_sort_hist_words(uint32_t R, int tile_bits) { return (size_t)256 * (rs_num_blocks(R) + 1) + (size_t)256 * (ts_max_blocks(R, ts_clamp_bits(tile_bits)) + 1); }

hipError_t ex4d_tile_sort_msd(const uint32_t *keys, const uint32_t *vals, uint32_t *packed, uint32_t *point_list, uint32_t *tile_ids_out,
    uint32_t R, int tile_bits, uint32_t *hist, uint2 *ranges, hipStream_t stream, const uint32_t *n_dev)
{
    if (R == 0) return hipSuccess;
    const int low_bits = (tile_bits + 1) / 2, high_bits = tile_bits - low_bits;
    const uint32_t nbA = rs_num_blocks(R), nbB = ts_max_blocks(R, tile_bits);
    uint32_t *histB = hist + (size_t)256 * (nbA + 1);
    const uint32_t *totals = hist + (size_t)256 * nbA;
    hipLaunchKernelGGL((rs_histogram_kernel<RS_ITEMS, 256, 8>), dim3(nbA), dim3(RS_THREADS), 0, stream, keys, R, low_bits, (1u << high_bits) - 1u, nbA, hist, n_dev);
    hipLaunchKernelGGL(rs_scan_rows_kernel, dim3(1u << high_bits), dim3(256), 0, stream, nbA, hist, 256u);
#define TS_SCATTER_A(NB) hipLaunchKernelGGL((rs_scatter_kernel<RS_ITEMS, 256, 1, NB>), dim3(nbA), dim3(RS_THREADS), 0, stream, keys, vals, packed, (uint32_t *)nullptr, \
        R, low_bits, high_bits, nbA, hist, low_bits, (const uint32_t *)nullptr, 0, (uint2 *)nullptr, n_dev)
    if (high_bits == 6) TS_SCATTER_A(6); else if (high_bits == 7) TS_SCATTER_A(7); else if (high_bits == 8) TS_SCATTER_A(8); else TS_SCATTER_A(0);
#undef TS_SCATTER_A
    hipLaunchKernelGGL(ts_histogram_kernel, dim3(nbB), dim3(RS_THREADS), 0, stream, packed, totals, 1 << high_bits, 32 - low_bits, nbB, histB);
    hipLaunchKernelGGL(rs_scan_rows_kernel, dim3(1u << low_bits), dim3(256), 0, stream, nbB, histB, 256u);
#define TS_SCATTER_B(NB) hipLaunchKernelGGL((rs_scatter_kernel<RS_ITEMS, 256, 2, NB>), dim3(nbB), dim3(RS_THREADS), 0, stream, packed, (const uint32_t *)nullptr, tile_ids_out, point_list, \
        R, 32 - low_bits, low_bits, nbB, histB, low_bits, totals, 1 << high_bits, ranges, (const uint32_t *)nullptr)
    if (low_bits == 7) TS_SCATTER_B(7); else if (low_bits == 8) TS_SCATTER_B(8); else TS_SCATTER_B(0);
#undef TS_SCATTER_B
    return hipGetLastError();
}

size_t ex4d_tile_sort_pass_b_hist_words(uint32_t R) { return (size_t)256 * (rs_num_blocks(R) + 258) + (size_t)6 * (rs_num_blocks(R) + 258); }
size_t ex4d_tile_sort_pass_b_table_offset(uint32_t R) { return (size_t)256 * (rs_num_blocks(R) + 258); }
hipError_t ex4d_tile_sort_pass_b(const uint32_t *packed, const uint32_t *totals, int nbuckets, int low_bits, uint32_t stride, uint32_t R, uint32_t cap,
    uint32_t *histB, uint32_t *point_list, uint32_t *tile_ids_out, uint2 *ranges, hipStream_t stream, const Ex4dTsBlock *block_table)
{
    if (R == 0) return hipSuccess;
    const uint32_t nbB = ex4d_tile_sort_pass_b_blocks(R, nbuckets);
    hipLaunchKernelGGL(ts_histogram_kernel, dim3(nbB), dim3(RS_THREADS), 0, stream, packed, totals, nbuckets, 32 - low_bits, nbB, histB, cap, block_table);
    hipLaunchKernelGGL(rs_scan_rows_kernel, dim3(1u << low_bits), dim3(256), 0, stream, nbB, histB, 256u);
#define TS_SCATTER_B(NB) hipLaunchKernelGGL((rs_scatter_kernel<RS_ITEMS, 256, 2, NB>), dim3(nbB), dim3(RS_THREADS), 0, stream, packed, (const uint32_t *)nullptr, tile_ids_out, point_list, \
        R, 32 - low_bits, low_bits, nbB, histB, low_bits, totals, nbuckets, ranges, (const uint32_t *)nullptr, (const uint32_t *)nullptr, (uint32_t *)nullptr, (uint32_t *)nullptr, \
        (const uint32_t *)nullptr, stride, cap, block_table)
    if (low_bits == 7) TS_SCATTER_B(7); else if (low_bits == 8) TS_SCATTER_B(8); else TS_SCATTER_B(0);
#undef TS_SCATTER_B
    return hipGetLastError();
}

hipError_t ex4d_launch_scan_tiles(int P, const uint2 *rects, const uint32_t *rects4, const uint32_t *order, uint2 *sorted_rects, uint32_t *sorted_offsets,
    uint32_t *block_sums, int T, uint2 *ranges, uint32_t *frame_total, hipStream_t stream)
{
    const int nb = (P + SCAN_CHUNK - 1) / SCAN_CHUNK;
    hipLaunchKernelGGL(scan_tiles_local_kernel, dim3(nb), dim3(256), 0, stream, P, rects, rects4, order, sorted_rects, sorted_offsets, block_sums, T, ranges, frame_total);
    return hipGetLastError();
}

hipError_t ex4d_launch_duplicate(int P, int W, int H, const uint32_t *order, const uint32_t *sorted_offsets,
    const uint32_t *block_sums, const uint2 *sorted_rects, const uint32_t *sorted_rects4, uint32_t *tile_keys, uint32_t *vals, uint32_t cap, hipStream_t stream,
    const uint32_t *bucket_keys, const uint32_t *dparams, const uint32_t *bucket_sums, uint32_t *frame_total, int msd_bits)
{
    const int gx = (W + EX4D_TILE - 1) / EX4D_TILE, gy = (H + EX4D_TILE - 1) / EX4D_TILE;
    hipLaunchKernelGGL(duplicate_kernel, dim3((P + 255) / 256), dim3(256), 0, stream, P, gx, gy, order, sorted_offsets, block_sums,
        sorted_rects, sorted_rects4, tile_keys, vals, cap, bucket_keys, dparams, bucket_sums, 1 << msd_bits, frame_total);
    return hipGetLastError();
}

hipError_t ex4d_launch_zero(void *ptr, size_t bytes, hipStream_t stream)
{
    const size_t n16 = bytes / 16;
    const uint32_t tail_words = (uint32_t)((bytes % 16) / 4);
    if (bytes == 0) return hipSuccess;
    size_t blocks = (n16 + 1023) / 1024;
    if (blocks > 8192) blocks = 8192;
    if (blocks == 0) blocks = 1;
    hipLaunchKernelGGL(zero_fill_kernel, dim3((unsigned)blocks), dim3(256), 0, stream, (uint4 *)ptr, n16, tail_words);
    return hipGetLastError();
}

hipError_t ex4d_launch_tile_ranges(uint32_t R, int T, const uint32_t *tile_ids, uint2 *ranges, hipStream_t stream, const uint32_t *n_dev)
{
    (void)T;
    if (R > 0)
        hipLaunchKernelGGL(tile_ranges_kernel, dim3((R + 255) / 256), dim3(256), 0, stream, R, tile_ids, ranges, n_dev);
    return hipGetLastError();
}
```

### ex4dgs_amd/csrc/ex4d_internal.h

```cpp
#pragma once
#include <hip/hip_runtime.h>
#include <stdint.h>
#include <stddef.h>
#include "../../include/ex4d_rasterizer.h"
#include "../../include/ex4d_attributes.h"

#define EX4D_ALIGN 256

static inline size_t ex4d_align_up(size_t x) { return (x + (EX4D_ALIGN - 1)) & ~(size_t)(EX4D_ALIGN - 1); }

#define EX4D_RECORD_FLOATS 16
#define EX4D_DLS_MSD_BITS 10
#define EX4D_CHUNK_FLOW 0x80000000u
#define EX4D_CHUNK_FILTERED 0x40000000u
#define EX4D_DSUMS_MARK 0x44535553u

struct GeomState {
    float4 *records;
    float *cov3D;
    uint8_t *clamped;
    uint32_t *tiles_touched;
    uint2 *rects;
    uint2 *sorted_rects;
    uint32_t *rects4;
    uint32_t *depth_order;
    uint32_t *sorted_offsets;
    uint32_t *sort_keys_a, *sort_keys_b, *sort_vals_b;
    uint32_t *bucket_sums;
    uint2 *key_ranges;
    uint32_t *sort_vals_a, *rects4_b, *bucket_starts;
    uint32_t *scan_block_sums;
    uint32_t *sort_hist;
    uint32_t *total;
    uint32_t *block_totals;
    uint32_t *row_hist;
    float *sh_dsums;
};
struct BinState {
    uint32_t *point_list;
    uint32_t *tile_ids;
    uint32_t *vals_tmp, *keys_tmp;
    uint32_t *sort_hist;
    uint32_t *qlist;
    uint32_t *qcount;
};
struct ImgState {
    float *final_T;
    uint32_t *n_contrib;
    uint2 *ranges;
};

#define RS_THREADS 256
#define RS_ITEMS 16
#define RS_CHUNK (RS_THREADS * RS_ITEMS)
#define RS_BINS 256
#define SCAN_CHUNK 2048

static inline uint32_t rs_num_blocks(uint32_t n) { return (n + RS_CHUNK - 1) / RS_CHUNK; }
struct Ex4dTsBlock { uint32_t start, count, bucket, fb_first, fb_next, bucket_start; };
static inline uint32_t ex4d_tile_sort_pass_b_blocks(uint32_t R, int nbuckets) { return rs_num_blocks(R) + (uint32_t)nbuckets + 1u; }

struct ShSplit { const float *dc[2]; const float *rest[2]; int n_static; };
struct ShSplitGrad { float *dc[2]; float *rest[2]; int n_static; };

hipError_t ex4d_launch_preprocess_fwd(const Ex4dParams &prm, const float *means3D, const float *dir3D, const float *scales,
    const float *rotations, const float *opacities, const float *shs, const float *cov3D_precomp,
    const float *colors_precomp, const float *viewmatrix, const float *projmatrix, const float *campos,
    int32_t *radii, GeomState g, uint32_t *prefilter_violation, ShSplit split,
    uint32_t *depth_keys, uint32_t *depth_vals, uint32_t depth_key_base, uint32_t depth_key_invisible, uint32_t *rects4, hipStream_t stream,
    uint32_t *key_range_slots = nullptr, bool global_flags = true);

hipError_t ex4d_launch_mark_visible(int P, const float *means3D, const float *viewmatrix, const float *projmatrix,
    float min_depth, float max_depth, uint8_t *present, hipStream_t stream);

hipError_t ex4d_launch_preprocess_bwd(const Ex4dParams &prm, const float *means3D, const int32_t *radii,
    const float *shs, const float *scales, const float *rotations, const float *cov3D_ptr,
    const float *viewmatrix, const float *projmatrix, const float *campos, GeomState g, const float *acc16,
    float *dL_dmeans2D, float *dL_dcolors, float *dL_dopacity, float *dL_dmeans3D, float *dL_dcov3D, float *dL_dsh,
    float *dL_dscales, float *dL_drotations, float *dL_ddir, ShSplit split, ShSplitGrad gsplit, hipStream_t stream);

hipError_t ex4d_radix_sort_pairs(uint32_t *keys_a, uint32_t *vals_a, uint32_t *keys_b, uint32_t *vals_b,
    uint32_t n, int end_bit, uint32_t *hist, bool *result_in_a, hipStream_t stream, const uint32_t *n_dev = nullptr, bool iota_values = false,
    const uint32_t *gather_in = nullptr, uint32_t *gather_out = nullptr, uint2 *zero_ranges = nullptr, int num_ranges = 0);
size_t ex4d_radix_hist_words(uint32_t n);
int ex4d_radix_passes(uint32_t n, int end_bit);

bool ex4d_tile_sort_msd_applies(int P, int tile_bits);
size_t ex4d_tile_sort_hist_words(uint32_t R, int tile_bits);
hipError_t ex4d_tile_sort_msd(const uint32_t *keys, const uint32_t *vals, uint32_t *packed, uint32_t *point_list, uint32_t *tile_ids_out,
    uint32_t R, int tile_bits, uint32_t *hist, uint2 *ranges, hipStream_t stream, const uint32_t *n_dev = nullptr);

bool ex4d_tile_sort_rows_applies(int P, int gx, int gy);
size_t ex4d_tile_sort_rows_geom_words(uint32_t P);
size_t ex4d_tile_sort_rows_hist_words(uint32_t R);
void ex4d_set_rows_probe(int v);
hipError_t ex4d_rows_prof(unsigned long long *out8, int reset);
hipError_t ex4d_tile_sort_rows(int P, int gx, int gy, const uint32_t *order, const uint32_t *r4, const uint2 *r8, uint32_t *words,
    uint32_t *point_list, uint32_t *tile_ids_out, uint32_t cap, uint32_t S, uint32_t *histA, uint32_t *histB, uint2 *ranges, uint32_t *frame_total, hipStream_t stream);

hipError_t ex4d_launch_scan_tiles(int P, const uint2 *rects, const uint32_t *rects4, const uint32_t *order, uint2 *sorted_rects, uint32_t *sorted_offsets,
    uint32_t *block_sums, int T, uint2 *ranges, uint32_t *frame_total, hipStream_t stream);
hipError_t ex4d_launch_duplicate(int P, int W, int H, const uint32_t *order, const uint32_t *sorted_offsets,
    const uint32_t *block_sums, const uint2 *sorted_rects, const uint32_t *sorted_rects4, uint32_t *tile_keys, uint32_t *vals, uint32_t cap, hipStream_t stream,
    const uint32_t *bucket_keys = nullptr, const uint32_t *dparams = nullptr, const uint32_t *bucket_sums = nullptr, uint32_t *frame_total = nullptr,
    int msd_bits = EX4D_DLS_MSD_BITS);

#define EX4D_FLAG_DPARAMS 8
#define EX4D_FLAG_WORDS 64
bool ex4d_depth_sort_msd_applies(uint32_t n, int key_bits);
hipError_t ex4d_depth_sort_msd(uint32_t *ka, uint32_t *va, uint32_t *ra, uint32_t *kb, uint32_t *vb, uint32_t *rb, uint32_t n, uint32_t inv_key,
    uint32_t *flags, const uint2 *wave_ranges, uint32_t *hist, uint32_t *starts, uint32_t local_cap, hipStream_t stream,
    uint32_t *local_incl, uint32_t *bucket_sums, int T, uint2 *ranges, int local_threads,
    uint32_t *watch = nullptr,
    int msd_bits = EX4D_DLS_MSD_BITS);
int ex4d_depth_sort_msd_bits(uint32_t n, int key_bits);
void ex4d_set_rank_lds(int v);
int ex4d_get_rank_lds();
int ex4d_rank_lds_in_use();
hipError_t ex4d_prepare_rank_lds(hipStream_t stream);
hipError_t ex4d_launch_zero(void *ptr, size_t bytes, hipStream_t stream);
hipError_t ex4d_launch_tile_ranges(uint32_t R, int T, const uint32_t *tile_ids, uint2 *ranges, hipStream_t stream, const uint32_t *n_dev = nullptr);

void ex4d_set_preprocess_tune(int v);
int ex4d_get_preprocess_tune();
void ex4d_set_preprocess_fast(int v);
int ex4d_get_preprocess_fast();
void ex4d_set_fwd_asm(int on);
int ex4d_get_fwd_asm();
void ex4d_set_clamp_always(int on);
int ex4d_get_clamp_always();
void ex4d_set_bwd_pairs(int on);
int ex4d_get_bwd_pairs();
hipError_t ex4d_launch_composite_fwd(const Ex4dParams &prm, const uint2 *ranges, const uint32_t *point_list,
    const float *subpixel_offset, const float4 *records, const float *bg, float *final_T, uint32_t *n_contrib,
    float *out_color, float *out_depth, float *out_acc, float *out_flow, int32_t *out_idx, uint32_t *qlist, uint32_t *qcount,
    bool has_flow, hipStream_t stream);

hipError_t ex4d_launch_composite_bwd(const Ex4dParams &prm, const uint2 *ranges, const uint32_t *point_list,
    const float *subpixel_offset, const float *bg, const float4 *records, const float *out_depth, const float *out_acc,
    const float *final_T, const uint32_t *n_contrib, const float *dL_dpix, const float *dL_ddepth,
    const float *dL_dflow, const float *dL_dacc, float *acc16, const uint32_t *qlist, const uint32_t *qcount,
    int variant, hipStream_t stream);

hipError_t ex4d_bwd_stats(unsigned long long *out, int count, int reset);
```

### ex4dgs_amd/csrc/ex4d_preprocess.hip

```cpp
#include "ex4d_internal.h"
#include <atomic>
#include <cstdlib>
#include <cstdlib>

namespace {

__constant__ float kSH_C0 = 0.28209479177387814f;
__constant__ float kSH_C1 = 0.4886025119029199f;
__constant__ float kSH_C2[5] = { 1.0925484305920792f, -1.0925484305920792f, 0.31539156525252005f,
                                 -1.0925484305920792f, 0.5462742152960396f };
__constant__ float kSH_C3[7] = { -0.5900435899266435f, 2.890611442640554f, -0.4570457994644658f, 0.3731763325901154f,
                                 -0.4570457994644658f, 1.445305721320277f, -0.5900435899266435f };

struct Mat3 { float m[3][3]; };

__device__ __forceinline__ Mat3 mul(const Mat3 &a, const Mat3 &b)
{
    Mat3 o;
#pragma unroll
    for (int c = 0; c < 3; c++)
#pragma unroll
        for (int r = 0; r < 3; r++)
            o.m[c][r] = a.m[0][r] * b.m[c][0] + a.m[1][r] * b.m[c][1] + a.m[2][r] * b.m[c][2];
    return o;
}
__device__ __forceinline__ Mat3 transpose(const Mat3 &a)
{
    Mat3 o;
#pragma unroll
    for (int c = 0; c < 3; c++)
#pragma unroll
        for (int r = 0; r < 3; r++)
            o.m[c][r] = a.m[r][c];
    return o;
}
__device__ __forceinline__ Mat3 from_columns(float a0, float a1, float a2, float b0, float b1, float b2, float c0, float c1, float c2)
{
    Mat3 o;
    o.m[0][0] = a0; o.m[0][1] = a1; o.m[0][2] = a2;
    o.m[1][0] = b0; o.m[1][1] = b1; o.m[1][2] = b2;
    o.m[2][0] = c0; o.m[2][1] = c1; o.m[2][2] = c2;
    return o;
}

__device__ __forceinline__ int to_int_sat(float f)
{
    if (f != f) return 0;
    if (f >= 2147483648.0f) return 2147483647;
    if (f <= -2147483648.0f) return (-2147483647 - 1);
    return (int)f;
}

__device__ __forceinline__ float3 xform4x3(float3 p, const float *m)
{
    return make_float3(m[0] * p.x + m[4] * p.y + m[8] * p.z + m[12],
                       m[1] * p.x + m[5] * p.y + m[9] * p.z + m[13],
                       m[2] * p.x + m[6] * p.y + m[10] * p.z + m[14]);
}
__device__ __forceinline__ float4 xform4x4(float3 p, const float *m)
{
    return make_float4(m[0] * p.x + m[4] * p.y + m[8] * p.z + m[12],
                       m[1] * p.x + m[5] * p.y + m[9] * p.z + m[13],
                       m[2] * p.x + m[6] * p.y + m[10] * p.z + m[14],
                       m[3] * p.x + m[7] * p.y + m[11] * p.z + m[15]);
}

__device__ __forceinline__ bool frustum_test(float3 p, const float *vm, const float *pm, float min_depth, float max_depth,
                                             float3 &p_view, float &ndc_x, float &ndc_y)
{
    float4 h = xform4x4(p, pm);
    float inv_w = 1.0f / (h.w + 0.0000001f);
    ndc_x = h.x * inv_w;
    ndc_y = h.y * inv_w;
    p_view = xform4x3(p, vm);
    return !((p_view.z <= min_depth) || (p_view.z > max_depth) ||
             ((double)ndc_x < -1.3 || (double)ndc_x > 1.3 || (double)ndc_y < -1.3 || (double)ndc_y > 1.3));
}

__device__ __forceinline__ void tile_rect(float px, float py, int radius, int gx, int gy, int &x0, int &y0, int &x1, int &y1)
{
    x0 = min(gx, max(0, to_int_sat((px - (float)radius) / (float)EX4D_TILE)));
    y0 = min(gy, max(0, to_int_sat((py - (float)radius) / (float)EX4D_TILE)));
    x1 = min(gx, max(0, to_int_sat((px + (float)radius + (float)EX4D_TILE - 1.0f) / (float)EX4D_TILE)));
    y1 = min(gy, max(0, to_int_sat((py + (float)radius + (float)EX4D_TILE - 1.0f) / (float)EX4D_TILE)));
}

__device__ __forceinline__ Mat3 rotation_from_quat(float r, float x, float y, float z)
{
    return from_columns(
        1.f - 2.f * (y * y + z * z), 2.f * (x * y - r * z), 2.f * (x * z + r * y),
        2.f * (x * y + r * z), 1.f - 2.f * (x * x + z * z), 2.f * (y * z - r * x),
        2.f * (x * z - r * y), 2.f * (y * z + r * x), 1.f - 2.f * (x * x + y * y));
}

struct Cov2DCtx { float3 t; float txtz, tytz, limx, limy; Mat3 Wm, T, Vrk, cov; };
__device__ __forceinline__ void cov2d_common(float3 mean, float fx, float fy, float tanx, float tany, const float *cov3D,
                                             const float *vm, Cov2DCtx &c)
{
    c.t = xform4x3(mean, vm);
    c.limx = 1.3f * tanx;
    c.limy = 1.3f * tany;
    c.txtz = c.t.x / c.t.z;
    c.tytz = c.t.y / c.t.z;
    c.t.x = fminf(c.limx, fmaxf(-c.limx, c.txtz)) * c.t.z;
    c.t.y = fminf(c.limy, fmaxf(-c.limy, c.tytz)) * c.t.z;
    Mat3 J = from_columns(fx / c.t.z, 0.0f, -(fx * c.t.x) / (c.t.z * c.t.z),
                          0.0f, fy / c.t.z, -(fy * c.t.y) / (c.t.z * c.t.z),
                          0.0f, 0.0f, 0.0f);
    c.Wm = from_columns(vm[0], vm[4], vm[8], vm[1], vm[5], vm[9], vm[2], vm[6], vm[10]);
    c.T = mul(c.Wm, J);
    c.Vrk = from_columns(cov3D[0], cov3D[1], cov3D[2], cov3D[1], cov3D[3], cov3D[4], cov3D[2], cov3D[4], cov3D[5]);
    Mat3 Tt = transpose(c.T);
    Mat3 Vt = transpose(c.Vrk);
    Mat3 TV = mul(Tt, Vt);
    c.cov = mul(TV, c.T);
}

template <int W>
__device__ __forceinline__ void wave_store_rows(float *__restrict__ dst_wave, const float (&vals)[W], float *lds, int nrows, int lane)
{
#pragma unroll
    for (int i = 0; i < W; i++) lds[lane * W + i] = vals[i];
    __builtin_amdgcn_fence(__ATOMIC_RELEASE, "wavefront");
    __builtin_amdgcn_wave_barrier();
    __builtin_amdgcn_fence(__ATOMIC_ACQUIRE, "wavefront");
#pragma unroll
    for (int i = 0; i < W; i++) {
        const int e = i * 64 + lane;
        if (e < nrows * W) dst_wave[e] = lds[e];
    }
    __builtin_amdgcn_fence(__ATOMIC_RELEASE, "wavefront");
    __builtin_amdgcn_wave_barrier();
    __builtin_amdgcn_fence(__ATOMIC_ACQUIRE, "wavefront");
}

__device__ __forceinline__ void cov3d_from_scale_rotation(float scale_modifier, float s0, float s1, float s2, float4 q, float (&cov3D)[6])
{
    Mat3 S = from_columns(1.0f, 0.f, 0.f, 0.f, 1.0f, 0.f, 0.f, 0.f, 1.0f);
    S.m[0][0] = scale_modifier * s0;
    S.m[1][1] = scale_modifier * s1;
    S.m[2][2] = scale_modifier * s2;
    Mat3 R = rotation_from_quat(q.x, q.y, q.z, q.w);
    Mat3 Mx = mul(S, R);
    Mat3 Sigma = mul(transpose(Mx), Mx);
    cov3D[0] = Sigma.m[0][0]; cov3D[1] = Sigma.m[0][1]; cov3D[2] = Sigma.m[0][2];
    cov3D[3] = Sigma.m[1][1]; cov3D[4] = Sigma.m[1][2]; cov3D[5] = Sigma.m[2][2];
}

#define SH_ROW 52

__device__ __forceinline__ void wave_sync_lds()
{
    __builtin_amdgcn_fence(__ATOMIC_RELEASE, "wavefront");
    __builtin_amdgcn_wave_barrier();
    __builtin_amdgcn_fence(__ATOMIC_ACQUIRE, "wavefront");
}

struct ShPrefetch { float4 v[13]; };
__device__ __forceinline__ bool mask_bit(uint64_t need, int g)
{
    const uint32_t half = (g & 32) ? (uint32_t)(need >> 32) : (uint32_t)need;
    return ((half >> (g & 31)) & 1u) != 0u;
}
__device__ __forceinline__ void wave_issue_sh(const float *__restrict__ shs_wave, ShPrefetch &pf, int nrows, int nvec, int lane, uint64_t need)
{
    const float4 *src = reinterpret_cast<const float4 *>(shs_wave);
    if (nrows == 64 && nvec == 12 && need == ~0ull) {
#pragma unroll
        for (int it = 0; it < 12; it++) pf.v[it] = src[it * 64 + lane];
        return;
    }
#pragma unroll
    for (int it = 0; it < 12; it++) {
        const int q = it * 64 + lane;
        const int g = q / 12, v = q - 12 * g;
        pf.v[it] = (g < nrows && v < nvec && mask_bit(need, g)) ? src[q] : make_float4(0.f, 0.f, 0.f, 0.f);
    }
}
__device__ __forceinline__ bool wave_issue_sh_split(const ShSplit &sp, int wave_first, int nrows, ShPrefetch &pf, int lane, uint64_t need)
{
    const bool all_dynamic = wave_first >= sp.n_static, all_static = wave_first + nrows <= sp.n_static;
    if (nrows <= 0 || !(all_dynamic || all_static)) return false;
    const int part = all_dynamic ? 1 : 0;
    const size_t r0 = (size_t)(wave_first - (part ? sp.n_static : 0));
    const float *rest = sp.rest[part] + r0 * 45, *dc = sp.dc[part] + r0 * 3;
    if (((((uintptr_t)rest) | ((uintptr_t)dc)) & 15) != 0 || nrows != 64) return false;
#pragma unroll
    for (int it = 0; it < 12; it++) {
        const int q = it * 64 + lane;
        const int r_lo = (4 * q) / 45, r_hi = (4 * q + 3) / 45;
        const bool want = q < 720 && (mask_bit(need, r_lo & 63) || mask_bit(need, r_hi & 63));
        pf.v[it] = want ? reinterpret_cast<const float4 *>(rest)[q] : make_float4(0.f, 0.f, 0.f, 0.f);
    }
    {
        const int r_lo = (4 * lane) / 3, r_hi = (4 * lane + 3) / 3;
        const bool want = lane < 48 && (mask_bit(need, r_lo & 63) || mask_bit(need, r_hi & 63));
        pf.v[12] = want ? reinterpret_cast<const float4 *>(dc)[lane] : make_float4(0.f, 0.f, 0.f, 0.f);
    }
    return true;
}

#define SH_HALF_FLOATS (32 * SH_ROW)
#define SH_HALF_DC_OFFSET (32 * 45)
__device__ __forceinline__ void wave_commit_sh_half(float *lds, const ShPrefetch &pf, int lane, int h)
{
#pragma unroll
    for (int i = 0; i < 6; i++) {
        const int it = 6 * h + i;
        const int q = it * 64 + lane;
        const int g = q / 12 - 32 * h, v = q % 12;
        *reinterpret_cast<float4 *>(lds + g * SH_ROW + 4 * v) = pf.v[it];
    }
    wave_sync_lds();
}
__device__ __forceinline__ void wave_commit_sh_split_half(float *lds, const ShPrefetch &pf, int lane, int h)
{
#pragma unroll
    for (int it = 0; it < 12; it++) {
        const int q = it * 64 + lane - 360 * h;
        if (q >= 0 && q < 360) reinterpret_cast<float4 *>(lds)[q] = pf.v[it];
    }
    const int d = lane - 24 * h;
    if (d >= 0 && d < 24) reinterpret_cast<float4 *>(lds + SH_HALF_DC_OFFSET)[d] = pf.v[12];
    wave_sync_lds();
}


__device__ __forceinline__ void wave_load_sh_half(const float *__restrict__ shs_wave, float *lds, int nrows, int nvec, int lane, int h, uint64_t need)
{
    const float4 *src = reinterpret_cast<const float4 *>(shs_wave);
    float4 t[6];
#pragma unroll
    for (int i = 0; i < 6; i++) {
        const int q = (6 * h + i) * 64 + lane;
        const int g = q / 12, v = q - 12 * g;
        t[i] = (g < nrows && v < nvec && mask_bit(need, g)) ? src[q] : make_float4(0.f, 0.f, 0.f, 0.f);
    }
#pragma unroll
    for (int i = 0; i < 6; i++) {
        const int q = (6 * h + i) * 64 + lane;
        const int g = q / 12 - 32 * h, v = q % 12;
        *reinterpret_cast<float4 *>(lds + g * SH_ROW + 4 * v) = t[i];
    }
    wave_sync_lds();
}
__device__ __forceinline__ bool wave_sh_split_stageable(const ShSplit &sp, int wave_first, int nrows)
{
    const bool all_dynamic = wave_first >= sp.n_static, all_static = wave_first + nrows <= sp.n_static;
    if (nrows != 64 || !(all_dynamic || all_static)) return false;
    const int part = all_dynamic ? 1 : 0;
    const size_t r0 = (size_t)(wave_first - (part ? sp.n_static : 0));
    return ((((uintptr_t)(sp.rest[part] + r0 * 45)) | ((uintptr_t)(sp.dc[part] + r0 * 3))) & 15) == 0;
}
__device__ __forceinline__ void wave_load_sh_split_half(const ShSplit &sp, int wave_first, float *lds, int lane, int h, uint64_t need)
{
    const int part = wave_first >= sp.n_static ? 1 : 0;
    const size_t r0 = (size_t)(wave_first - (part ? sp.n_static : 0)) + 32 * h;
    const float4 *rest = reinterpret_cast<const float4 *>(sp.rest[part] + r0 * 45);
    const uint32_t need_h = (uint32_t)(need >> (32 * h));
    float4 t[6];
#pragma unroll
    for (int i = 0; i < 6; i++) {
        const int q = i * 64 + lane;
        const int r_lo = (4 * q) / 45, r_hi = (4 * q + 3) / 45;
        const bool want = q < 360 && (((need_h >> r_lo) | (need_h >> (r_hi & 31))) & 1u);
        t[i] = want ? rest[q] : make_float4(0.f, 0.f, 0.f, 0.f);
    }
#pragma unroll
    for (int i = 0; i < 6; i++) { const int q = i * 64 + lane; if (q < 360) reinterpret_cast<float4 *>(lds)[q] = t[i]; }
    wave_sync_lds();
}

__device__ __forceinline__ void wave_store_sh_split_half(const ShSplitGrad &sp, int first, const float *lds, int lane)
{
    wave_sync_lds();
    const int part = first >= sp.n_static ? 1 : 0;
    const size_t r0 = (size_t)(first - (part ? sp.n_static : 0));
    float4 *rest = reinterpret_cast<float4 *>(sp.rest[part] + r0 * 45), *dc = reinterpret_cast<float4 *>(sp.dc[part] + r0 * 3);
#pragma unroll
    for (int i = 0; i < 6; i++) { const int q = i * 64 + lane; if (q < 360) rest[q] = reinterpret_cast<const float4 *>(lds)[q]; }
    if (lane < 24) dc[lane] = reinterpret_cast<const float4 *>(lds + SH_HALF_DC_OFFSET)[lane];
}

__device__ __forceinline__ void wave_store_sh_half(float *__restrict__ dst_half, const float *lds, int nrows, int lane)
{
    wave_sync_lds();
    float4 *dst = reinterpret_cast<float4 *>(dst_half);
#pragma unroll
    for (int it = 0; it < 6; it++) {
        const int q = it * 64 + lane;
        const int g = q / 12, v = q - 12 * g;
        if (g < nrows) dst[q] = *reinterpret_cast<const float4 *>(lds + g * SH_ROW + 4 * v);
    }
}





__device__ __forceinline__ void sh_direction_sums(const float *sh, int D, float x, float y, float z,
                                                  float (&dRGBdx)[3], float (&dRGBdy)[3], float (&dRGBdz)[3])
{
#define SHK(k) sh[3 * (k) + ch]
    if (D > 0) {
#pragma unroll
        for (int ch = 0; ch < 3; ch++) {
            dRGBdx[ch] = -kSH_C1 * SHK(3);
            dRGBdy[ch] = -kSH_C1 * SHK(1);
            dRGBdz[ch] = kSH_C1 * SHK(2);
        }
        if (D > 1) {
            const float xx = x * x, yy = y * y, zz = z * z, xy = x * y, yz = y * z, xz = x * z;
#pragma unroll
            for (int ch = 0; ch < 3; ch++) {
                dRGBdx[ch] += kSH_C2[0] * y * SHK(4) + kSH_C2[2] * 2.f * -x * SHK(6) + kSH_C2[3] * z * SHK(7) + kSH_C2[4] * 2.f * x * SHK(8);
                dRGBdy[ch] += kSH_C2[0] * x * SHK(4) + kSH_C2[1] * z * SHK(5) + kSH_C2[2] * 2.f * -y * SHK(6) + kSH_C2[4] * 2.f * -y * SHK(8);
                dRGBdz[ch] += kSH_C2[1] * y * SHK(5) + kSH_C2[2] * 2.f * 2.f * z * SHK(6) + kSH_C2[3] * x * SHK(7);
            }
            if (D > 2) {
#pragma unroll
                for (int ch = 0; ch < 3; ch++) {
                    dRGBdx[ch] += (
                        kSH_C3[0] * SHK(9) * 3.f * 2.f * xy +
                        kSH_C3[1] * SHK(10) * yz +
                        kSH_C3[2] * SHK(11) * -2.f * xy +
                        kSH_C3[3] * SHK(12) * -3.f * 2.f * xz +
                        kSH_C3[4] * SHK(13) * (-3.f * xx + 4.f * zz - yy) +
                        kSH_C3[5] * SHK(14) * 2.f * xz +
                        kSH_C3[6] * SHK(15) * 3.f * (xx - yy));
                    dRGBdy[ch] += (
                        kSH_C3[0] * SHK(9) * 3.f * (xx - yy) +
                        kSH_C3[1] * SHK(10) * xz +
                        kSH_C3[2] * SHK(11) * (-3.f * yy + 4.f * zz - xx) +
                        kSH_C3[3] * SHK(12) * -3.f * 2.f * yz +
                        kSH_C3[4] * SHK(13) * -2.f * xy +
                        kSH_C3[5] * SHK(14) * -2.f * yz +
                        kSH_C3[6] * SHK(15) * -3.f * 2.f * xy);
                    dRGBdz[ch] += (
                        kSH_C3[1] * SHK(10) * xy +
                        kSH_C3[2] * SHK(11) * 4.f * 2.f * yz +
                        kSH_C3[3] * SHK(12) * 3.f * (2.f * zz - xx - yy) +
                        kSH_C3[4] * SHK(13) * 4.f * 2.f * xz +
                        kSH_C3[5] * SHK(14) * (xx - yy));
                }
            }
        }
    }
#undef SHK
}

template <bool FAST>
__global__ __launch_bounds__(256) void preprocess_fwd_kernel(
    int P, int D_, int M_,
    const float *__restrict__ means3D, const float *__restrict__ dir3D, const float *__restrict__ scales, float scale_modifier,
    const float *__restrict__ rotations, const float *__restrict__ opacities, const float *__restrict__ shs,
    const float *__restrict__ cov3D_precomp_, const float *__restrict__ colors_precomp_,
    const float *__restrict__ viewmatrix, const float *__restrict__ projmatrix, const float *__restrict__ campos,
    int W, int H, float tanx, float tany, float fx, float fy, float kernel_size, float min_depth, float max_depth,
    int prefiltered, uint32_t *__restrict__ prefilter_violation,
    int32_t *__restrict__ radii, float4 *__restrict__ records, float *__restrict__ cov3Ds,
    uint8_t *__restrict__ clamped, uint32_t *__restrict__ tiles_touched, uint2 *__restrict__ rects,
    uint32_t *__restrict__ depth_keys, uint32_t *__restrict__ depth_vals, uint32_t depth_key_base, uint32_t depth_key_invisible,
    uint32_t *__restrict__ total_instances, const ShSplit sp_, float *__restrict__ sh_dsums, int sh_predicate, uint32_t *__restrict__ rects4,
    uint32_t *__restrict__ key_range_slots, int global_flags)
{
    const int D = FAST ? 3 : D_, M = FAST ? 16 : M_;
    const float *__restrict__ cov3D_precomp = FAST ? nullptr : cov3D_precomp_;
    const float *__restrict__ colors_precomp = FAST ? nullptr : colors_precomp_;
    ShSplit sp = sp_;
    if (FAST) { sp.dc[0] = sp.dc[1] = sp.rest[0] = sp.rest[1] = nullptr; sp.n_static = 0; __builtin_assume(shs != nullptr); }
    __shared__ __attribute__((aligned(16))) float sh_lds[4 * SH_HALF_FLOATS];
    const int lane = threadIdx.x & 63, wave = threadIdx.x >> 6;
    __shared__ uint32_t s_kr[4];
    if (key_range_slots) {
        if (threadIdx.x < 4) s_kr[threadIdx.x] = 0u;
        __syncthreads();
    }
    const int wc = (int)blockIdx.x * 4 + wave;
    if (wc >= ((P + 63) >> 6)) return;
    const int idx = wc * 64 + lane;
    const bool in_range = idx < P;
    float vm[16], pm[16];
#pragma unroll
    for (int i = 0; i < 16; i++) { vm[i] = viewmatrix[i]; pm[i] = projmatrix[i]; }

    const int ncoef = (D + 1) * (D + 1);
    const bool split = sp.rest[0] != nullptr || sp.rest[1] != nullptr;
    const bool staged = (shs != nullptr || split) && (M == 16);
    const int wave_first = wc * 64;
    const int wave_rows = (P - wave_first) < 64 ? (P - wave_first) : 64;
    ShPrefetch pf;
    bool prefetched = false;
    bool pre_ok = false;
    float3 pre_p = make_float3(0.f, 0.f, 0.f), pre_view = make_float3(0.f, 0.f, 0.f);
    float pre_nx = 0.f, pre_ny = 0.f;
    uint64_t need = ~0ull;
    if (sh_predicate) {
        if (in_range) {
            pre_p = make_float3(means3D[3 * (size_t)idx], means3D[3 * (size_t)idx + 1], means3D[3 * (size_t)idx + 2]);
            pre_ok = frustum_test(pre_p, vm, pm, min_depth, max_depth, pre_view, pre_nx, pre_ny);
        }
        need = __ballot(pre_ok);
    }
    if (staged) {
        if (split) prefetched = wave_issue_sh_split(sp, wave_first, wave_rows, pf, lane, need);
        else { wave_issue_sh(shs + (size_t)wave_first * 48, pf, wave_rows, (ncoef * 3 + 3) / 4, lane, need); prefetched = true; }
    }
    float4 in_q = make_float4(0.f, 0.f, 0.f, 0.f);
    float in_s0 = 0.f, in_s1 = 0.f, in_s2 = 0.f, in_op = 0.f, in_d0 = 0.f, in_d1 = 0.f, in_d2 = 0.f;
    if (in_range) {
        if (!cov3D_precomp) {
            in_q = reinterpret_cast<const float4 *>(rotations)[idx];
            in_s0 = scales[3 * (size_t)idx]; in_s1 = scales[3 * (size_t)idx + 1]; in_s2 = scales[3 * (size_t)idx + 2];
        }
        in_op = opacities[idx];
        if (dir3D) { in_d0 = dir3D[3 * (size_t)idx]; in_d1 = dir3D[3 * (size_t)idx + 1]; in_d2 = dir3D[3 * (size_t)idx + 2]; }
    }

    if (staged && prefetched) {
        float *lds0 = sh_lds + wave * SH_HALF_FLOATS;
        if (split) wave_commit_sh_split_half(lds0, pf, lane, 0);
        else wave_commit_sh_half(lds0, pf, lane, 0);
    }

    int out_radius = 0;
    uint32_t out_tiles = 0;
    uint32_t depth_key = depth_key_invisible;
    uint2 rect = make_uint2(0u, 0u);
    bool visible = false, filtered = false;
    float3 p = make_float3(0.f, 0.f, 0.f), conic = make_float3(0.f, 0.f, 0.f);
    float pix_x = 0.f, pix_y = 0.f, depth = 0.f, coef = 0.f;
    if (in_range) do {
        float3 p_view; float ndc_x, ndc_y;
        bool in_view;
        if (sh_predicate) { p = pre_p; p_view = pre_view; ndc_x = pre_nx; ndc_y = pre_ny; in_view = pre_ok; }
        else {
            p = make_float3(means3D[3 * (size_t)idx], means3D[3 * (size_t)idx + 1], means3D[3 * (size_t)idx + 2]);
            in_view = frustum_test(p, vm, pm, min_depth, max_depth, p_view, ndc_x, ndc_y);
        }
        if (!in_view) {
            if (prefiltered) { filtered = true; if (global_flags) atomicOr(prefilter_violation, 1u); }
            break;
        }
        float cov3D[6];
        if (cov3D_precomp) {
#pragma unroll
            for (int i = 0; i < 6; i++) cov3D[i] = cov3D_precomp[6 * (size_t)idx + i];
        } else {
            cov3d_from_scale_rotation(scale_modifier, in_s0, in_s1, in_s2, in_q, cov3D);
            if (cov3Ds) {
#pragma unroll
                for (int i = 0; i < 6; i++) cov3Ds[6 * (size_t)idx + i] = cov3D[i];
            }
        }
        Cov2DCtx c;
        cov2d_common(p, fx, fy, tanx, tany, cov3D, vm, c);
        const float det_0 = (float)fmax(1e-6, (double)(c.cov.m[0][0] * c.cov.m[1][1] - c.cov.m[0][1] * c.cov.m[0][1]));
        const float det_1 = (float)fmax(1e-6, (double)((c.cov.m[0][0] + kernel_size) * (c.cov.m[1][1] + kernel_size) - c.cov.m[0][1] * c.cov.m[0][1]));
        coef = (float)sqrt((double)det_0 / ((double)det_1 + 1e-6) + 1e-6);
        if ((double)det_0 <= 1e-6 || (double)det_1 <= 1e-6) coef = 0.0f;
        const float ca = c.cov.m[0][0] + kernel_size, cb = c.cov.m[0][1], cc = c.cov.m[1][1] + kernel_size;

        const float det = ca * cc - cb * cb;
        if (det == 0.0f) break;
        const float det_inv = 1.f / det;
        conic = make_float3(cc * det_inv, -cb * det_inv, ca * det_inv);
        const float mid = 0.5f * (ca + cc);
        const float lambda1 = mid + sqrtf(fmaxf(0.1f, mid * mid - det));
        const float lambda2 = mid - sqrtf(fmaxf(0.1f, mid * mid - det));
        const float my_radius = ceilf(3.f * sqrtf(fmaxf(lambda1, lambda2)));
        pix_x = (float)((((double)ndc_x + 1.0) * (double)W - 1.0) * 0.5);
        pix_y = (float)((((double)ndc_y + 1.0) * (double)H - 1.0) * 0.5);
        const int gx = (W + EX4D_TILE - 1) / EX4D_TILE, gy = (H + EX4D_TILE - 1) / EX4D_TILE;
        const int ri = to_int_sat(my_radius);
        int x0, y0, x1, y1;
        tile_rect(pix_x, pix_y, ri, gx, gy, x0, y0, x1, y1);
        const uint32_t area = (uint32_t)(x1 - x0) * (uint32_t)(y1 - y0);
        if (area == 0) break;
        rect = make_uint2((uint32_t)x0 | ((uint32_t)y0 << 16), (uint32_t)(x1 - x0) | ((uint32_t)(y1 - y0) << 16));
        visible = true;
        depth = p_view.z;
        out_radius = ri;
        out_tiles = area;
        depth_key = __float_as_uint(p_view.z) - depth_key_base;
    } while (0);

    if (key_range_slots) {
        uint32_t kmax = visible ? depth_key : 0u, nkmin = visible ? ~depth_key : 0u;
#pragma unroll
        for (int o = 32; o > 0; o >>= 1) {
            const uint32_t a = __shfl_xor(kmax, o, 64), b = __shfl_xor(nkmin, o, 64);
            kmax = a > kmax ? a : kmax; nkmin = b > nkmin ? b : nkmin;
        }
        if (lane == 0) {
            atomicMax(&s_kr[0], kmax); atomicMax(&s_kr[1], nkmin);
            const int nchunks = (P + 63) >> 6, mine = nchunks - (int)blockIdx.x * 4;
            const uint32_t t = atomicAdd(&s_kr[2], 1u);
            if ((int)t == (mine < 4 ? mine : 4) - 1)
                reinterpret_cast<uint2 *>(key_range_slots)[blockIdx.x] = make_uint2(__hip_atomic_load(&s_kr[0], __ATOMIC_RELAXED, __HIP_MEMORY_SCOPE_WORKGROUP),
                                                                                    __hip_atomic_load(&s_kr[1], __ATOMIC_RELAXED, __HIP_MEMORY_SCOPE_WORKGROUP));
        }
    }
    float coefv[16][3];
    if (staged) {
        float *lds = sh_lds + wave * SH_HALF_FLOATS;
        float tmp[48];
#pragma unroll
        for (int f = 0; f < 48; f++) tmp[f] = 0.f;
        const int r = lane & 31;
        if (split) {
            if (prefetched) {
#pragma unroll
                for (int h = 0; h < 2; h++) {
                    if (h == 1) wave_commit_sh_split_half(lds, pf, lane, 1);
                    if (visible && (lane >> 5) == h) {
#pragma unroll
                        for (int f = 0; f < 3; f++) tmp[f] = lds[SH_HALF_DC_OFFSET + r * 3 + f];
#pragma unroll
                        for (int f = 3; f < 48; f++) if (f < ncoef * 3) tmp[f] = lds[r * 45 + (f - 3)];
                    }
                    wave_sync_lds();
                }
            } else if (visible) {
                const int part = idx >= sp.n_static;
                const size_t row = (size_t)(idx - (part ? sp.n_static : 0));
#pragma unroll
                for (int f = 0; f < 3; f++) tmp[f] = sp.dc[part][row * 3 + f];
#pragma unroll
                for (int f = 3; f < 48; f++) if (f < ncoef * 3) tmp[f] = sp.rest[part][row * 45 + (f - 3)];
            }
        } else {
            const int nvec = (ncoef * 3 + 3) / 4;
#pragma unroll
            for (int h = 0; h < 2; h++) {
                if (h == 1) wave_commit_sh_half(lds, pf, lane, 1);
                if (visible && (lane >> 5) == h) {
                    const float4 *row = reinterpret_cast<const float4 *>(lds + r * SH_ROW);
#pragma unroll
                    for (int v = 0; v < 12; v++) {
                        if (v < nvec) { const float4 t4 = row[v]; tmp[4 * v] = t4.x; tmp[4 * v + 1] = t4.y; tmp[4 * v + 2] = t4.z; tmp[4 * v + 3] = t4.w; }
                    }
                }
                wave_sync_lds();
            }
        }
#pragma unroll
        for (int k = 0; k < 16; k++) { coefv[k][0] = tmp[3 * k]; coefv[k][1] = tmp[3 * k + 1]; coefv[k][2] = tmp[3 * k + 2]; }
    } else if (shs && visible) {
        const float *sh = shs + (size_t)idx * M * 3;
#pragma unroll
        for (int k = 0; k < 16; k++)
#pragma unroll
            for (int ch = 0; ch < 3; ch++) coefv[k][ch] = (k < ncoef && k < M) ? sh[3 * k + ch] : 0.f;
    }
    if (visible) {
        float res[3];
        if (colors_precomp) {
            res[0] = colors_precomp[3 * (size_t)idx]; res[1] = colors_precomp[3 * (size_t)idx + 1]; res[2] = colors_precomp[3 * (size_t)idx + 2];
        } else {
            float dx = p.x - campos[0], dy = p.y - campos[1], dz = p.z - campos[2];
            const float len = sqrtf(dx * dx + dy * dy + dz * dz);
            const float x = dx / len, y = dy / len, z = dz / len;
            uint8_t clamp_bits = 0;
#pragma unroll
            for (int ch = 0; ch < 3; ch++) {
#define SHK(k) coefv[k][ch]
                float result = kSH_C0 * SHK(0);
                if (D > 0) {
                    result = result - kSH_C1 * y * SHK(1) + kSH_C1 * z * SHK(2) - kSH_C1 * x * SHK(3);
                    if (D > 1) {
                        const float xx = x * x, yy = y * y, zz = z * z, xy = x * y, yz = y * z, xz = x * z;
                        result = result +
                            kSH_C2[0] * xy * SHK(4) +
                            kSH_C2[1] * yz * SHK(5) +
                            kSH_C2[2] * (2.0f * zz - xx - yy) * SHK(6) +
                            kSH_C2[3] * xz * SHK(7) +
                            kSH_C2[4] * (xx - yy) * SHK(8);
                        if (D > 2) {
                            result = result +
                                kSH_C3[0] * y * (3.0f * xx - yy) * SHK(9) +
                                kSH_C3[1] * xy * z * SHK(10) +
                                kSH_C3[2] * y * (4.0f * zz - xx - yy) * SHK(11) +
                                kSH_C3[3] * z * (2.0f * zz - 3.0f * xx - 3.0f * yy) * SHK(12) +
                                kSH_C3[4] * x * (4.0f * zz - xx - yy) * SHK(13) +
                                kSH_C3[5] * z * (xx - yy) * SHK(14) +
                                kSH_C3[6] * x * (xx - 3.0f * yy) * SHK(15);
                        }
                    }
                }
#undef SHK
                result += 0.5f;
                if (result < 0) clamp_bits |= (uint8_t)(1u << ch);
                res[ch] = fmaxf(result, 0.0f);
            }
            clamped[idx] = clamp_bits;
            if (sh_dsums) {
                float dRGBdx[3] = { 0, 0, 0 }, dRGBdy[3] = { 0, 0, 0 }, dRGBdz[3] = { 0, 0, 0 };
                sh_direction_sums(&coefv[0][0], D, x, y, z, dRGBdx, dRGBdy, dRGBdz);
                float *o = sh_dsums + 9 * (size_t)idx;
#pragma unroll
                for (int ch = 0; ch < 3; ch++) { o[ch] = dRGBdx[ch]; o[3 + ch] = dRGBdy[ch]; o[6 + ch] = dRGBdz[ch]; }
            }
        }
        const float w_op = in_op * coef;
        float tau;
        if (w_op < (1.0f / 255.0f)) tau = -__builtin_inff();
        else if (!(conic.x > 0.f && conic.z > 0.f && conic.x * conic.z - conic.y * conic.y > 0.f)) tau = __builtin_inff();
        else tau = logf(255.0f * w_op) + 0.01f;
        float4 *rec = records + 4 * (size_t)idx;
        rec[0] = make_float4(pix_x, pix_y, conic.x, conic.y);
        rec[1] = make_float4(conic.z, tau, -conic.y / conic.z, -conic.y / conic.x);
        rec[2] = make_float4(depth, res[0], res[1], res[2]);
        rec[3] = make_float4(in_d0, in_d1, in_d2, w_op);
    }
    const bool chunk_flow = __ballot(visible && (in_d0 != 0.f || in_d1 != 0.f || in_d2 != 0.f)) != 0ull;
    const bool chunk_filtered = prefiltered && __ballot(filtered) != 0ull;
    if (global_flags && chunk_flow) {
        if (lane == 0) prefilter_violation[1] = 1u;
    }
    if (idx == 0) prefilter_violation[2] = sh_dsums ? EX4D_DSUMS_MARK : 0u;
    if (in_range) {
        radii[idx] = out_radius;
        if (tiles_touched) tiles_touched[idx] = out_tiles;
        if (rects) rects[idx] = rect;
        if (rects4) rects4[idx] = (rect.x & 0xFFu) | ((rect.x >> 16) << 8) | ((rect.y & 0xFFu) << 16) | ((rect.y >> 16) << 24);
        depth_keys[idx] = depth_key;
        if (depth_vals) depth_vals[idx] = (uint32_t)idx;
    }
    uint32_t wave_sum = out_tiles, wave_seg = visible ? (rect.y >> 16) : 0u;
#pragma unroll
    for (int o = 32; o > 0; o >>= 1) { wave_sum += __shfl_xor(wave_sum, o, 64); wave_seg += __shfl_xor(wave_seg, o, 64); }
    if (lane == 0) reinterpret_cast<uint2 *>(total_instances)[wc] = make_uint2(wave_sum, wave_seg | (chunk_flow ? EX4D_CHUNK_FLOW : 0u) | (chunk_filtered ? EX4D_CHUNK_FILTERED : 0u));
}

__global__ __launch_bounds__(256) void mark_visible_kernel(int P, const float *__restrict__ means3D,
    const float *__restrict__ viewmatrix, const float *__restrict__ projmatrix, float min_depth, float max_depth,
    uint8_t *__restrict__ present)
{
    const int idx = blockIdx.x * 256 + threadIdx.x;
    if (idx >= P) return;
    float vm[16], pm[16];
#pragma unroll
    for (int i = 0; i < 16; i++) { vm[i] = viewmatrix[i]; pm[i] = projmatrix[i]; }
    const float3 p = make_float3(means3D[3 * (size_t)idx], means3D[3 * (size_t)idx + 1], means3D[3 * (size_t)idx + 2]);
    float3 pv; float nx, ny;
    present[idx] = frustum_test(p, vm, pm, min_depth, max_depth, pv, nx, ny) ? 1 : 0;
}

template <bool DSUMS>
__global__ __launch_bounds__(256) void preprocess_bwd_kernel(
    int P, int D, int M,
    const float *__restrict__ means3D, const int32_t *__restrict__ radii, const float *__restrict__ shs,
    const uint8_t *__restrict__ clamped, const float *__restrict__ scales, const float *__restrict__ rotations,
    float scale_modifier, const float *__restrict__ cov3Ds, const float *__restrict__ viewmatrix,
    const float *__restrict__ projmatrix, const float *__restrict__ campos,
    int W, int H, float fx, float fy, float tanx, float tany, float kernel_size,
    const float *__restrict__ acc16, const float4 *__restrict__ records,
    float *__restrict__ dL_dmeans2D, float *__restrict__ dL_dcolors, float *__restrict__ dL_dopacity,
    float *__restrict__ dL_dmeans3D, float *__restrict__ dL_dcov3D, float *__restrict__ dL_dsh,
    float *__restrict__ dL_dscales, float *__restrict__ dL_drotations, float *__restrict__ dL_ddir, const ShSplit sp, const ShSplitGrad gsp,
    const float *__restrict__ sh_dsums, const uint32_t *__restrict__ frame_flags)
{
    __shared__ __attribute__((aligned(16))) float sh_lds[4 * SH_HALF_FLOATS];
    const int idx = blockIdx.x * 256 + threadIdx.x;
    const int lane = threadIdx.x & 63, wave = threadIdx.x >> 6;
    const bool in_range = idx < P;
    const bool split = sp.rest[0] != nullptr || sp.rest[1] != nullptr;
    const bool staged = (shs != nullptr || split) && (M == 16);
    float *lds_row_base = sh_lds + wave * SH_HALF_FLOATS;
    const bool dsums_ok = !DSUMS || frame_flags[3] == EX4D_DSUMS_MARK;
    const int wave_first = blockIdx.x * 256 + wave * 64;
    const int wave_rows = (P - wave_first) < 64 ? (P - wave_first) : 64;
    const bool prefetched = staged && (split ? wave_sh_split_stageable(sp, wave_first, wave_rows) : true);
    int in_radius = 0;
    float4 in_r0 = make_float4(0.f, 0.f, 0.f, 0.f), in_r1 = in_r0, in_r2 = in_r0, in_r3 = in_r0, in_q = in_r0;
    float in_mean[3] = { 0.f, 0.f, 0.f }, in_cov[6] = { 0.f, 0.f, 0.f, 0.f, 0.f, 0.f }, in_s[3] = { 0.f, 0.f, 0.f };
    uint8_t in_clamped = 0;
    if (in_range) {
        in_radius = radii[idx];
        const float4 *row = reinterpret_cast<const float4 *>(acc16 + 16 * (size_t)idx);
        in_r0 = row[0]; in_r1 = row[1]; in_r2 = row[2]; in_r3 = row[3];
#pragma unroll
        for (int i = 0; i < 3; i++) in_mean[i] = means3D[3 * (size_t)idx + i];
        if (!scales) {
#pragma unroll
            for (int i = 0; i < 6; i++) in_cov[i] = cov3Ds[6 * (size_t)idx + i];
        }
        if (scales) {
            in_q = reinterpret_cast<const float4 *>(rotations)[idx];
#pragma unroll
            for (int i = 0; i < 3; i++) in_s[i] = scales[3 * (size_t)idx + i];
        }
        if (shs || split) in_clamped = clamped[idx];
    }
    const bool visible = in_range && (in_radius > 0);
    float g_mean2D[3] = { 0, 0, 0 }, g_color[3] = { 0, 0, 0 }, g_dir[3] = { 0, 0, 0 }, g_opacity = 0;
    float g_mean3D[3] = { 0, 0, 0 }, g_cov[6] = { 0, 0, 0, 0, 0, 0 }, g_scale[3] = { 0, 0, 0 }, g_rot[4] = { 0, 0, 0, 0 };
    float3 sh_dir = make_float3(0.f, 0.f, 0.f), sh_dir_orig = make_float3(0.f, 0.f, 0.f);
    float sh_dRGB[3] = { 0.f, 0.f, 0.f }, sh_j[3] = { 0.f, 0.f, 0.f };
    if (visible && (shs || split)) {
        const float3 dir_orig = make_float3(in_mean[0] - campos[0], in_mean[1] - campos[1], in_mean[2] - campos[2]);
        const float len = sqrtf(dir_orig.x * dir_orig.x + dir_orig.y * dir_orig.y + dir_orig.z * dir_orig.z);
        sh_dir = make_float3(dir_orig.x / len, dir_orig.y / len, dir_orig.z / len);
        sh_dir_orig = dir_orig;
        const float gc[3] = { in_r1.w, in_r2.x, in_r2.y };
#pragma unroll
        for (int ch = 0; ch < 3; ch++) sh_dRGB[ch] = gc[ch] * (((in_clamped >> ch) & 1) ? 0.f : 1.f);
    }
    if (shs || split) {
        float dRGBdx[3] = { 0, 0, 0 }, dRGBdy[3] = { 0, 0, 0 }, dRGBdz[3] = { 0, 0, 0 };
        const int r = lane & 31;
        const uint64_t need_rows = __ballot(visible);
        if (DSUMS) {
            if (visible) {
                const float *o = sh_dsums + 9 * (size_t)idx;
// ... 153 lines not shown
            }
        }
#undef DSH
    }
    bool store_staged = prefetched;
    if (split && prefetched) {
        const int part = wave_first >= gsp.n_static ? 1 : 0;
        const size_t r0 = (size_t)(wave_first - (part ? gsp.n_static : 0));
        store_staged = ((((uintptr_t)(gsp.rest[part] + r0 * 45)) | ((uintptr_t)(gsp.dc[part] + r0 * 3))) & 15) == 0;
    }
    if (M == 16 && split && !store_staged) {
        if (in_range) {
            const int part = idx >= gsp.n_static;
            const size_t row = (size_t)(idx - (part ? gsp.n_static : 0));
            float *dc = gsp.dc[part] + row * 3, *rest = gsp.rest[part] + row * 45;
#pragma unroll
            for (int ch = 0; ch < 3; ch++) dc[ch] = g_sh[0][ch];
#pragma unroll
            for (int k = 1; k < 16; k++)
#pragma unroll
                for (int ch = 0; ch < 3; ch++) rest[3 * (k - 1) + ch] = g_sh[k][ch];
        }
    } else if (M == 16) {
#pragma unroll
        for (int h = 0; h < 2; h++) {
            wave_sync_lds();
            if ((lane >> 5) == h) {
                const int r = lane & 31;
                if (split) {
#pragma unroll
                    for (int ch = 0; ch < 3; ch++) lds_row_base[SH_HALF_DC_OFFSET + r * 3 + ch] = g_sh[0][ch];
#pragma unroll
                    for (int k = 1; k < 16; k++)
#pragma unroll
                        for (int ch = 0; ch < 3; ch++) lds_row_base[r * 45 + 3 * (k - 1) + ch] = g_sh[k][ch];
                } else {
                    float4 *row = reinterpret_cast<float4 *>(lds_row_base + r * SH_ROW);
#pragma unroll
                    for (int v = 0; v < 12; v++) {
                        float t[4];
#pragma unroll
                        for (int e = 0; e < 4; e++) { const int f = 4 * v + e; t[e] = g_sh[f / 3][f % 3]; }
                        row[v] = make_float4(t[0], t[1], t[2], t[3]);
                    }
                }
            }
            const int first = wave_first + 32 * h;
            const int nrows_sh = (P - first) < 32 ? (P - first) : 32;
            if (split) wave_store_sh_split_half(gsp, first, lds_row_base, lane);
            else wave_store_sh_half(dL_dsh + (size_t)first * 48, lds_row_base, nrows_sh, lane);
        }
        wave_sync_lds();
    }
    {
        const int nrows = (P - wave_first) < 64 ? (P - wave_first) : 64;
        wave_store_rows<3>(dL_dmeans2D + 3 * (size_t)wave_first, g_mean2D, lds_row_base, nrows, lane);
        if (dL_dcolors) wave_store_rows<3>(dL_dcolors + 3 * (size_t)wave_first, g_color, lds_row_base, nrows, lane);
        wave_store_rows<3>(dL_dmeans3D + 3 * (size_t)wave_first, g_mean3D, lds_row_base, nrows, lane);
        wave_store_rows<3>(dL_dscales + 3 * (size_t)wave_first, g_scale, lds_row_base, nrows, lane);
        wave_store_rows<3>(dL_ddir + 3 * (size_t)wave_first, g_dir, lds_row_base, nrows, lane);
        if (dL_dcov3D) wave_store_rows<6>(dL_dcov3D + 6 * (size_t)wave_first, g_cov, lds_row_base, nrows, lane);
    }
    if (!in_range) return;
    dL_dopacity[idx] = g_opacity;
    reinterpret_cast<float4 *>(dL_drotations)[idx] = make_float4(g_rot[0], g_rot[1], g_rot[2], g_rot[3]);
    if (M != 16) {
#pragma unroll
        for (int k = 0; k < 16; k++)
            if (k < M) {
#pragma unroll
                for (int ch = 0; ch < 3; ch++) dL_dsh[((size_t)idx * M + k) * 3 + ch] = g_sh[k][ch];
            }
        for (int k = 16; k < M; k++)
            for (int ch = 0; ch < 3; ch++) dL_dsh[((size_t)idx * M + k) * 3 + ch] = 0.f;
    }
}

}

static int preprocess_option_default() { const char *e = getenv("EX4D_PREPROCESS_SH_PREDICATE"); return e ? (atoi(e) != 0) : 1; }
static std::atomic<int> g_preprocess_fast{1};
void ex4d_set_preprocess_fast(int v) { g_preprocess_fast.store(v); }
int ex4d_get_preprocess_fast() { return g_preprocess_fast.load(); }
static std::atomic<int> g_preprocess_tune{preprocess_option_default()};
void ex4d_set_preprocess_tune(int v) { g_preprocess_tune.store(v != 0); }
int ex4d_get_preprocess_tune() { return g_preprocess_tune.load(); }

hipError_t ex4d_launch_preprocess_fwd(const Ex4dParams &prm, const float *means3D, const float *dir3D, const float *scales,
    const float *rotations, const float *opacities, const float *shs, const float *cov3D_precomp,
    const float *colors_precomp, const float *viewmatrix, const float *projmatrix, const float *campos,
    int32_t *radii, GeomState g, uint32_t *prefilter_violation, ShSplit split,
    uint32_t *depth_keys, uint32_t *depth_vals, uint32_t depth_key_base, uint32_t depth_key_invisible, uint32_t *rects4, hipStream_t stream,
    uint32_t *key_range_slots, bool global_flags)
{
    const float fy = prm.H / (2.0f * prm.tanfovy);
    const float fx = prm.W / (2.0f * prm.tanfovx);
    const bool is_split = split.rest[0] != nullptr || split.rest[1] != nullptr;
    const bool fast = g_preprocess_fast.load(std::memory_order_relaxed) != 0 && shs != nullptr && !is_split && prm.D == 3 && prm.M == 16 &&
                      cov3D_precomp == nullptr && colors_precomp == nullptr && scales != nullptr && rotations != nullptr;
#define PF_ARGS prm.P, prm.D, prm.M, means3D, dir3D, scales, prm.scale_modifier, rotations, opacities, shs, cov3D_precomp, colors_precomp, \
        viewmatrix, projmatrix, campos, prm.W, prm.H, prm.tanfovx, prm.tanfovy, fx, fy, prm.kernel_size, \
        prm.min_depth, prm.max_depth, prm.prefiltered, prefilter_violation, \
        radii, g.records, g.cov3D, g.clamped, g.tiles_touched, g.rects, depth_keys, depth_vals, depth_key_base, depth_key_invisible, g.block_totals, split, \
        (prm.prepare_backward && (shs != nullptr || is_split)) ? g.sh_dsums : (float *)nullptr, \
        g_preprocess_tune.load(std::memory_order_relaxed), rects4, key_range_slots, global_flags ? 1 : 0
    if (fast) hipLaunchKernelGGL(preprocess_fwd_kernel<true>, dim3((prm.P + 255) / 256), dim3(256), 0, stream, PF_ARGS);
    else hipLaunchKernelGGL(preprocess_fwd_kernel<false>, dim3((prm.P + 255) / 256), dim3(256), 0, stream, PF_ARGS);
#undef PF_ARGS
    return hipGetLastError();
}

hipError_t ex4d_launch_mark_visible(int P, const float *means3D, const float *viewmatrix, const float *projmatrix,
    float min_depth, float max_depth, uint8_t *present, hipStream_t stream)
{
    hipLaunchKernelGGL(mark_visible_kernel, dim3((P + 255) / 256), dim3(256), 0, stream,
        P, means3D, viewmatrix, projmatrix, min_depth, max_depth, present);
    return hipGetLastError();
}

hipError_t ex4d_launch_preprocess_bwd(const Ex4dParams &prm, const float *means3D, const int32_t *radii,
    const float *shs, const float *scales, const float *rotations, const float *cov3D_ptr,
    const float *viewmatrix, const float *projmatrix, const float *campos, GeomState g, const float *acc16,
    float *dL_dmeans2D, float *dL_dcolors, float *dL_dopacity, float *dL_dmeans3D, float *dL_dcov3D, float *dL_dsh,
    float *dL_dscales, float *dL_drotations, float *dL_ddir, ShSplit split, ShSplitGrad gsplit, hipStream_t stream)
{
    const float fy = prm.H / (2.0f * prm.tanfovy);
    const float fx = prm.W / (2.0f * prm.tanfovx);
#define PB_ARGS prm.P, prm.D, prm.M, means3D, radii, shs, g.clamped, scales, rotations, prm.scale_modifier, cov3D_ptr, \
        viewmatrix, projmatrix, campos, prm.W, prm.H, fx, fy, prm.tanfovx, prm.tanfovy, prm.kernel_size, acc16, g.records, \
        dL_dmeans2D, dL_dcolors, dL_dopacity, dL_dmeans3D, dL_dcov3D, dL_dsh, dL_dscales, dL_drotations, dL_ddir, split, gsplit
    const bool has_sh = shs != nullptr || split.rest[0] != nullptr || split.rest[1] != nullptr;
    if (prm.prepare_backward && has_sh)
        hipLaunchKernelGGL(preprocess_bwd_kernel<true>, dim3((prm.P + 255) / 256), dim3(256), 0, stream, PB_ARGS, (const float *)g.sh_dsums, (const uint32_t *)g.total);
    else
        hipLaunchKernelGGL(preprocess_bwd_kernel<false>, dim3((prm.P + 255) / 256), dim3(256), 0, stream, PB_ARGS, (const float *)nullptr, (const uint32_t *)g.total);
#undef PB_ARGS
    return hipGetLastError();
}
```

Baseline: 0.6548 ms/frame.

## Offload SH colour evaluation onto extra rider blocks of depth-sort kernels

```diff
diff --git a/ex4dgs_amd/build.py b/ex4dgs_amd/build.py
--- a/ex4dgs_amd/build.py
+++ b/ex4dgs_amd/build.py
@@ -105,7 +105,7 @@
     headers = [os.path.join(CSRC, "ex4d_internal.h"), os.path.join(HERE, "..", "include", "ex4d_rasterizer.h"),
                os.path.join(HERE, "..", "include", "ex4d_attributes.h"), os.path.join(HERE, "..", "include", "ex4d_loss.h"), os.path.join(HERE, "..", "include", "ex4d_optim.h"), os.path.join(HERE, "..", "include", "ex4d_knn.h"), os.path.join(HERE, "..", "include", "ex4d_trainer.h"),
                os.path.join(HERE, "..", "include", "ex4d_densify.h"), os.path.join(HERE, "..", "include", "ex4d_regularizers.h"),
-               os.path.join(CSRC, "ex4d_reg_rows.h"),
+               os.path.join(CSRC, "ex4d_reg_rows.h"), os.path.join(CSRC, "ex4d_sh_colour.h"),
                os.path.abspath(__file__)]
     objs = []
     for src, flags in SOURCES.items():
diff --git a/ex4dgs_amd/csrc/ex4d_api.hip b/ex4dgs_amd/csrc/ex4d_api.hip
--- a/ex4dgs_amd/csrc/ex4d_api.hip
+++ b/ex4dgs_amd/csrc/ex4d_api.hip
@@ -331,10 +331,11 @@
         gw.cov3D = nullptr; gw.tiles_touched = nullptr;
         if (packed_rects) gw.rects = nullptr;
     }
+    ShRide sh_ride = {};
     STAGE(ex4d_launch_preprocess_fwd(*prm, means3D, dir3D, scales, rotations, opacities, shs, cov3D_precomp, colors_precomp,
                                      viewmatrix, projmatrix, campos, radii, gw, g.total + 1, split,
                                      keys0, (uint32_t *)nullptr, key_base, key_invisible, packed_rects ? g.rects4 : nullptr, stream,
-                                     msd_depth ? reinterpret_cast<uint32_t *>(g.key_ranges) : nullptr, async), prm, stream);
+                                     msd_depth ? reinterpret_cast<uint32_t *>(g.key_ranges) : nullptr, async, msd_depth ? &sh_ride : nullptr), prm, stream);
     MARK(0, "preprocess_fwd");
     const size_t nblk = (size_t)(P + 63) / 64;
     const size_t rb_words = (size_t)(g.block_totals - g.total) + 2 * nblk;
@@ -357,7 +358,7 @@
         STAGE(ex4d_depth_sort_msd(g.sort_keys_a, g.sort_vals_a, g.rects4, g.sort_keys_b, g.depth_order, g.rects4_b, (uint32_t)P, key_invisible,
                                   g.total, g.key_ranges, g.sort_hist, g.bucket_starts, (uint32_t)g_depth_local_cap.load(std::memory_order_relaxed), stream,
                                   fused_scan ? g.sorted_offsets : nullptr, fused_scan ? g.bucket_sums : nullptr, T, (fused_scan || rows_sort) ? im.ranges : nullptr,
-                                  g_depth_local_threads.load(std::memory_order_relaxed), msd_watch, msd_bits), prm, stream);
+                                  g_depth_local_threads.load(std::memory_order_relaxed), msd_watch, msd_bits, &sh_ride), prm, stream);
         MARK(0, "depth_sort");
         if (!fused_scan && !rows_sort) {
             STAGE(ex4d_launch_scan_tiles(P, nullptr, g.rects4_b, nullptr, nullptr, g.sorted_offsets, g.scan_block_sums, T, im.ranges, async ? g.total : nullptr, stream), prm, stream);
@@ -598,6 +599,7 @@
     if (name && !strcmp(name, "preprocess_sh_predicate") && (value == 0 || value == 1)) { ex4d_set_preprocess_tune(value); return EX4D_OK; }
     if (name && !strcmp(name, "geom_debug_arrays") && (value == 0 || value == 1)) { g_geom_debug.store(value); return EX4D_OK; }
     if (name && !strcmp(name, "preprocess_fast_path") && (value == 0 || value == 1)) { ex4d_set_preprocess_fast(value); return EX4D_OK; }
+    if (name && !strcmp(name, "preprocess_sh_ride") && value >= 0 && value <= 2) { ex4d_set_preprocess_sh_ride(value); return EX4D_OK; }
     if (name && !strcmp(name, "depth_sort_msd") && value >= 0 && value <= 3) { g_depth_msd.store(value); g_depth_watch.reset(); return EX4D_OK; }
     if (name && !strcmp(name, "depth_sort_local_cap") && value >= 0 && value <= 8192) { g_depth_local_cap.store(value); return EX4D_OK; }
     if (name && !strcmp(name, "readback_side_stream") && (value == 0 || value == 1)) { g_readback_side.store(value); return EX4D_OK; }
@@ -623,6 +625,7 @@
     if (name && !strcmp(name, "preprocess_sh_predicate")) return ex4d_get_preprocess_tune();
     if (name && !strcmp(name, "geom_debug_arrays")) return g_geom_debug.load();
     if (name && !strcmp(name, "preprocess_fast_path")) return ex4d_get_preprocess_fast();
+    if (name && !strcmp(name, "preprocess_sh_ride")) return ex4d_get_preprocess_sh_ride();
     if (name && !strcmp(name, "depth_sort_msd")) return g_depth_msd.load();
     if (name && !strcmp(name, "depth_sort_hold")) return g_depth_watch.hold.load();
     if (name && !strcmp(name, "depth_sort_trips")) return g_depth_watch.trips.load();
diff --git a/ex4dgs_amd/csrc/ex4d_binning.hip b/ex4dgs_amd/csrc/ex4d_binning.hip
--- a/ex4dgs_amd/csrc/ex4d_binning.hip
+++ b/ex4dgs_amd/csrc/ex4d_binning.hip
@@ -1,6 +1,9 @@
 #include "ex4d_internal.h"
+#include "ex4d_sh_colour.h"
 #include <atomic>
 #include <mutex>
+#include <cstdio>
+#include <cstdlib>
 
 __device__ int ex4d_g_rank_lds = 0;
 
@@ -66,10 +69,15 @@
     }
 }
 
-__global__ __launch_bounds__(256) void rs_scan_rows_kernel(uint32_t nblocks, uint32_t *__restrict__ hist, uint32_t bins)
-{
-    __shared__ uint32_t wave_sums[4];
-    __shared__ uint32_t carry_s;
+template <bool RIDE>
+__global__ __launch_bounds__(256) void rs_scan_rows_kernel(uint32_t nblocks, uint32_t *__restrict__ hist, uint32_t bins, const ShRide ride)
+{
+    struct Own { uint32_t wave_sums[4]; uint32_t carry_s; };
+    __shared__ __attribute__((aligned(16))) unsigned char smem[RIDE && 4 * SH_RIDE_SLICE_BYTES > sizeof(Own) ? 4 * SH_RIDE_SLICE_BYTES : sizeof(Own)];
+    if (RIDE && blockIdx.x >= bins) { sh_ride_block(ride, (int)(blockIdx.x - bins), 4, smem); return; }
+    Own &own = *reinterpret_cast<Own *>(smem);
+    uint32_t (&wave_sums)[4] = own.wave_sums;
+    uint32_t &carry_s = own.carry_s;
     uint32_t *row = hist + (size_t)blockIdx.x * nblocks;
     const int lane = threadIdx.x & 63, wave = threadIdx.x >> 6;
     const bool vec = ((((uintptr_t)row) & 15) == 0);
@@ -142,10 +150,15 @@
 
 template <int ITEMS, int BINS>
 __global__ __launch_bounds__(RS_THREADS) void dls_histogram_kernel(const uint32_t *__restrict__ keys, uint32_t n, uint32_t nblocks,
-    uint32_t *__restrict__ hist, uint32_t *__restrict__ dparams, const uint2 *__restrict__ ranges, uint32_t nranges, uint32_t inv_key)
-{
-    __shared__ uint32_t h[BINS];
-    __shared__ uint32_t s_red[8];
+    uint32_t *__restrict__ hist, uint32_t *__restrict__ dparams, const uint2 *__restrict__ ranges, uint32_t nranges, uint32_t inv_key, const ShRide ride)
+{
+    struct Own { uint32_t h[BINS]; uint32_t s_red[8]; };
+    __shared__ __attribute__((aligned(16))) unsigned char smem[4 * SH_RIDE_SLICE_BYTES > sizeof(Own) ? 4 * SH_RIDE_SLICE_BYTES : sizeof(Own)];
+    static_assert(RS_THREADS == 256, "four SH wave slices per rider workgroup");
+    if (blockIdx.x >= nblocks) { sh_ride_block(ride, (int)(blockIdx.x - nblocks), 4, smem); return; }
+    Own &own = *reinterpret_cast<Own *>(smem);
+    uint32_t (&h)[BINS] = own.h;
+    uint32_t (&s_red)[8] = own.s_red;
     for (int b = threadIdx.x; b < BINS; b += RS_THREADS) h[b] = 0;
     const uint32_t base = blockIdx.x * (RS_THREADS * ITEMS);
     uint32_t k[ITEMS];
@@ -211,21 +224,35 @@
     int low_bits, const uint32_t *__restrict__ bucket_totals, int nbuckets, uint2 *__restrict__ ranges, const uint32_t *__restrict__ n_dev,
     const uint32_t *__restrict__ rects_in = nullptr, uint32_t *__restrict__ rects_out = nullptr, uint32_t *__restrict__ bucket_starts = nullptr,
     const uint32_t *__restrict__ dparams = nullptr, uint32_t range_stride = 0, uint32_t out_cap = 0xFFFFFFFFu,
-    const Ex4dTsBlock *__restrict__ block_table = nullptr)
-{
+    const Ex4dTsBlock *__restrict__ block_table = nullptr, const ShRide ride = ShRide{})
+{
+    constexpr int STAGE_WORDS = (MODE == 2 ? 1 : 2) * RS_THREADS * ITEMS;
+    struct Own {
+        uint32_t wave_cnt[4][BINS];
+        uint32_t local_start[BINS];
+        uint32_t global_base[BINS];
+        uint32_t scan_tmp[8];
+        __attribute__((aligned(16))) uint32_t stage_w[STAGE_WORDS];
+        uint32_t stage_r[MODE == 3 ? RS_THREADS * ITEMS : 1];
+    };
+    constexpr size_t RIDE_BYTES = MODE == 3 ? 4 * SH_RIDE_SLICE_BYTES : 0;
+    __shared__ __attribute__((aligned(16))) unsigned char smem[sizeof(Own) > RIDE_BYTES ? sizeof(Own) : RIDE_BYTES];
+    if constexpr (MODE == 3) {
+        if (blockIdx.x >= nblocks) { sh_ride_block(ride, (int)(blockIdx.x - nblocks), 4, smem); return; }
+    }
     if (n_dev) { const uint32_t nd = *n_dev; n = nd < n ? nd : n; }
     if (MODE == 0 && ranges) for (uint32_t i = blockIdx.x * RS_THREADS + threadIdx.x; i < range_stride; i += gridDim.x * RS_THREADS) ranges[i] = make_uint2(0u, 0u);
     if (MODE != 2 && blockIdx.x * (uint32_t)(RS_THREADS * ITEMS) >= n) return;
-    __shared__ uint32_t wave_cnt[4][BINS];
-    __shared__ uint32_t local_start[BINS];
-    __shared__ uint32_t global_base[BINS];
-    __shared__ uint32_t scan_tmp[8];
-    constexpr int STAGE_WORDS = (MODE == 2 ? 1 : 2) * RS_THREADS * ITEMS;
-    __shared__ __attribute__((aligned(16))) uint32_t stage_w[STAGE_WORDS];
+    Own &own = *reinterpret_cast<Own *>(smem);
+    uint32_t (&wave_cnt)[4][BINS] = own.wave_cnt;
+    uint32_t (&local_start)[BINS] = own.local_start;
+    uint32_t (&global_base)[BINS] = own.global_base;
+    uint32_t (&scan_tmp)[8] = own.scan_tmp;
+    uint32_t *const stage_w = own.stage_w;
     uint2 *const stage = reinterpret_cast<uint2 *>(stage_w);
-    __shared__ uint32_t stage_r[MODE == 3 ? RS_THREADS * ITEMS : 1];
+    uint32_t *const stage_r = own.stage_r;
     static_assert(sizeof(TsLocateLds) <= sizeof(uint32_t) * STAGE_WORDS, "the block table's scratch lives in the staging area");
-    static_assert(sizeof(uint32_t) * (4 * BINS + 2 * BINS + 8) + sizeof(uint32_t) * STAGE_WORDS + sizeof(uint32_t) * (MODE == 3 ? RS_THREADS * ITEMS : 1) <= 80 * 1024,
+    static_assert(sizeof(smem) <= 80 * 1024,
                   "rs_scatter_kernel: static LDS beyond 80 KB (two workgroups per CU)");
     const int tid = threadIdx.x, lane = tid & 63, wave = tid >> 6;
     if (NBITS > 0) nbits = NBITS;
@@ -621,19 +648,23 @@
 }
 
 template <int THREADS>
-__global__ __launch_bounds__(THREADS, THREADS == 512 ? 4 : 5) void depth_local_sort_kernel(uint32_t *kb, uint32_t *vb, uint32_t *rb, uint32_t *ka, uint32_t *va, uint32_t *ra,
+__global__ __launch_bounds__(THREADS, 4) void depth_local_sort_kernel(uint32_t *kb, uint32_t *vb, uint32_t *rb, uint32_t *ka, uint32_t *va, uint32_t *ra,
     const uint32_t *__restrict__ starts, const uint32_t *__restrict__ totals, const uint32_t *__restrict__ dparams, uint32_t cap,
-    uint32_t *__restrict__ local_incl, uint32_t *__restrict__ bucket_sums, int T, uint2 *__restrict__ ranges, uint32_t *__restrict__ watch)
+    uint32_t *__restrict__ local_incl, uint32_t *__restrict__ bucket_sums, int T, uint2 *__restrict__ ranges, uint32_t *__restrict__ watch,
+    uint32_t nbins, const ShRide ride)
 {
     constexpr int DLS_THREADS = THREADS, DLS_WAVES = THREADS / 64, DLS_CAP = THREADS * DLS_ITEMS, IDX_BITS = DlsLds<THREADS>::IDX_BITS;
-    __shared__ DlsLds<THREADS> L;
+    constexpr size_t RIDE_BYTES = (size_t)DLS_WAVES * SH_RIDE_SLICE_BYTES;
+    __shared__ __attribute__((aligned(16))) unsigned char smem[sizeof(DlsLds<THREADS>) > RIDE_BYTES ? sizeof(DlsLds<THREADS>) : RIDE_BYTES];
+    if (blockIdx.x >= nbins) { sh_ride_block(ride, (int)(blockIdx.x - nbins), DLS_WAVES, smem); return; }
+    DlsLds<THREADS> &L = *reinterpret_cast<DlsLds<THREADS> *>(smem);
     const uint32_t b = blockIdx.x;
     const int tid = threadIdx.x;
-    if (ranges) for (int i = b * DLS_THREADS + tid; i < T; i += gridDim.x * DLS_THREADS) ranges[i] = make_uint2(0u, 0u);
+    if (ranges) for (int i = b * DLS_THREADS + tid; i < T; i += nbins * DLS_THREADS) ranges[i] = make_uint2(0u, 0u);
     const uint32_t n = totals[b], s = starts[b];
     const DlsParams dq = dls_params(dparams);
     const int rem = (int)dq.shift;
-    const uint32_t inv_digit = gridDim.x - 1u;
+    const uint32_t inv_digit = nbins - 1u;
     if (b == inv_digit || n == 0u) {
         if (bucket_sums && tid == 0) bucket_sums[b] = 0u;
         return;
@@ -920,7 +951,7 @@
         const uint32_t mask = (1u << nbits) - 1u;
         if (small) {
             hipLaunchKernelGGL((rs_histogram_kernel<RS_SMALL_ITEMS, 512, 1>), dim3(nb), dim3(RS_THREADS), 0, stream, kin, n, shift, mask, nb, hist, n_dev);
-            hipLaunchKernelGGL(rs_scan_rows_kernel, dim3(1u << nbits), dim3(256), 0, stream, nb, hist, 512u);
+            hipLaunchKernelGGL(rs_scan_rows_kernel<false>, dim3(1u << nbits), dim3(256), 0, stream, nb, hist, 512u, ShRide{});
             const bool last = pass == npass - 1;
 #define RS_SMALL_SCATTER(NB) hipLaunchKernelGGL((rs_scatter_kernel<RS_SMALL_ITEMS, 512, 0, NB>), dim3(nb), dim3(RS_THREADS), 0, stream, kin, vin, kout, vout, n, shift, nbits, nb, hist, 0, nullptr, 0, \
                 last ? zero_ranges : (uint2 *)nullptr, n_dev, last ? gather_in : (const uint32_t *)nullptr, last ? gather_out : (uint32_t *)nullptr, (uint32_t *)nullptr, (const uint32_t *)nullptr, (uint32_t)num_ranges)
@@ -928,7 +959,7 @@
 #undef RS_SMALL_SCATTER
         } else {
             hipLaunchKernelGGL((rs_histogram_kernel<RS_ITEMS, 256, 1>), dim3(nb), dim3(RS_THREADS), 0, stream, kin, n, shift, mask, nb, hist, n_dev);
-            hipLaunchKernelGGL(rs_scan_rows_kernel, dim3(1u << nbits), dim3(256), 0, stream, nb, hist, 256u);
+            hipLaunchKernelGGL(rs_scan_rows_kernel<false>, dim3(1u << nbits), dim3(256), 0, stream, nb, hist, 256u, ShRide{});
             const bool last = pass == npass - 1;
             hipLaunchKernelGGL((rs_scatter_kernel<RS_ITEMS, 256, 0, 0>), dim3(nb), dim3(RS_THREADS), 0, stream, kin, vin, kout, vout, n, shift, nbits, nb, hist, 0, nullptr, 0,
                 last ? zero_ranges : (uint2 *)nullptr, n_dev, last ? gather_in : (const uint32_t *)nullptr, last ? gather_out : (uint32_t *)nullptr, (uint32_t *)nullptr, (const uint32_t *)nullptr, (uint32_t)num_ranges);
@@ -947,10 +978,29 @@
     const int narrow = EX4D_DLS_MSD_BITS - 1;
     return (n <= 1300000u && key_bits - (narrow - 1) + DLS_IDX_BITS <= 32) ? narrow : EX4D_DLS_MSD_BITS;
 }
+static const int *sh_ride_permille()
+{
+    static int pm[3] = { 0, 0, 420 };
+    static const bool parsed = [] {
+        const char *e = getenv("EX4D_SH_RIDE_SPLIT");
+        int a, b, c;
+        if (e && sscanf(e, "%d,%d,%d", &a, &b, &c) == 3 && a >= 0 && b >= 0 && c >= 0 && a + b + c <= 1000) { pm[0] = a; pm[1] = b; pm[2] = c; }
+        return true;
+    }();
+    (void)parsed;
+    return pm;
+}
+void ex4d_sh_ride_split(int count, int out[4])
+{
+    const int *pm = sh_ride_permille();
+    int left = count;
+    for (int i = 0; i < 3; i++) { out[i] = (int)(((long long)count * pm[i]) / 1000); left -= out[i]; }
+    out[3] = left;
+}
 template <int MB>
 static hipError_t depth_sort_msd_launch(uint32_t *ka, uint32_t *va, uint32_t *ra, uint32_t *kb, uint32_t *vb, uint32_t *rb, uint32_t n, uint32_t inv_key,
     uint32_t *flags, const uint2 *wave_ranges, uint32_t *hist, uint32_t *starts, uint32_t local_cap, hipStream_t stream,
-    uint32_t *local_incl, uint32_t *bucket_sums, int T, uint2 *ranges, int local_threads, uint32_t *watch)
+    uint32_t *local_incl, uint32_t *bucket_sums, int T, uint2 *ranges, int local_threads, uint32_t *watch, const ShRide *ride)
 {
     if (n == 0) return hipSuccess;
     constexpr int BINS = 1 << MB;
@@ -961,33 +1011,40 @@
     if (local_threads != 256 && local_threads != 512) local_threads = (MB < EX4D_DLS_MSD_BITS || n > 1200000u) ? 512 : 256;
     const uint32_t kcap = (uint32_t)local_threads * DLS_ITEMS;
     if (local_cap == 0 || local_cap > kcap) local_cap = kcap;
-    if (small) {
-        hipLaunchKernelGGL((dls_histogram_kernel<RS_SMALL_ITEMS, BINS>), dim3(nb), dim3(RS_THREADS), 0, stream, ka, n, nb, hist, dparams, wave_ranges, nranges, inv_key);
-        hipLaunchKernelGGL(rs_scan_rows_kernel, dim3(BINS), dim3(256), 0, stream, nb, hist, (uint32_t)BINS);
-        hipLaunchKernelGGL((rs_scatter_kernel<RS_SMALL_ITEMS, BINS, 3, MB>), dim3(nb), dim3(RS_THREADS), 0, stream, ka, (const uint32_t *)nullptr, kb, vb, n, 0, MB, nb, hist,
-            0, (const uint32_t *)nullptr, 0, (uint2 *)nullptr, (const uint32_t *)nullptr, ra, rb, starts, (const uint32_t *)dparams);
-    } else {
-        hipLaunchKernelGGL((dls_histogram_kernel<RS_ITEMS, BINS>), dim3(nb), dim3(RS_THREADS), 0, stream, ka, n, nb, hist, dparams, wave_ranges, nranges, inv_key);
-        hipLaunchKernelGGL(rs_scan_rows_kernel, dim3(BINS), dim3(256), 0, stream, nb, hist, (uint32_t)BINS);
-        hipLaunchKernelGGL((rs_scatter_kernel<RS_ITEMS, BINS, 3, MB>), dim3(nb), dim3(RS_THREADS), 0, stream, ka, (const uint32_t *)nullptr, kb, vb, n, 0, MB, nb, hist,
-            0, (const uint32_t *)nullptr, 0, (uint2 *)nullptr, (const uint32_t *)nullptr, ra, rb, starts, (const uint32_t *)dparams);
-    }
+    ShRide r[4] = { ShRide{}, ShRide{}, ShRide{}, ShRide{} };
+    uint32_t extra[4] = { 0u, 0u, 0u, 0u };
+    if (ride && ride->count > 0) {
+        int part[4];
+        ex4d_sh_ride_split(ride->count, part);
+        for (int i = 0, first = ride->first; i < 4; i++) {
+            r[i] = *ride; r[i].first = first; r[i].count = part[i];
+            extra[i] = ex4d_sh_ride_blocks(r[i], i == 3 ? local_threads / 64 : 4);
+            first += part[i];
+        }
+    }
+#define DLS_PARTITION(ITEMS_) \
+        hipLaunchKernelGGL((dls_histogram_kernel<ITEMS_, BINS>), dim3(nb + extra[0]), dim3(RS_THREADS), 0, stream, ka, n, nb, hist, dparams, wave_ranges, nranges, inv_key, r[0]); \
+        hipLaunchKernelGGL(rs_scan_rows_kernel<true>, dim3(BINS + extra[1]), dim3(256), 0, stream, nb, hist, (uint32_t)BINS, r[1]); \
+        hipLaunchKernelGGL((rs_scatter_kernel<ITEMS_, BINS, 3, MB>), dim3(nb + extra[2]), dim3(RS_THREADS), 0, stream, ka, (const uint32_t *)nullptr, kb, vb, n, 0, MB, nb, hist, \
+            0, (const uint32_t *)nullptr, 0, (uint2 *)nullptr, (const uint32_t *)nullptr, ra, rb, starts, (const uint32_t *)dparams, 0u, 0xFFFFFFFFu, (const Ex4dTsBlock *)nullptr, r[2])
+    if (small) { DLS_PARTITION(RS_SMALL_ITEMS); } else { DLS_PARTITION(RS_ITEMS); }
+#undef DLS_PARTITION
     if (local_threads == 256)
-        hipLaunchKernelGGL(depth_local_sort_kernel<256>, dim3(BINS), dim3(256), 0, stream, kb, vb, rb, ka, va, ra, starts, hist + (size_t)BINS * nb, (const uint32_t *)dparams, local_cap,
-            local_incl, bucket_sums, T, ranges, watch);
+        hipLaunchKernelGGL(depth_local_sort_kernel<256>, dim3(BINS + extra[3]), dim3(256), 0, stream, kb, vb, rb, ka, va, ra, starts, hist + (size_t)BINS * nb, (const uint32_t *)dparams, local_cap,
+            local_incl, bucket_sums, T, ranges, watch, (uint32_t)BINS, r[3]);
     else
-        hipLaunchKernelGGL(depth_local_sort_kernel<512>, dim3(BINS), dim3(512), 0, stream, kb, vb, rb, ka, va, ra, starts, hist + (size_t)BINS * nb, (const uint32_t *)dparams, local_cap,
-            local_incl, bucket_sums, T, ranges, watch);
+        hipLaunchKernelGGL(depth_local_sort_kernel<512>, dim3(BINS + extra[3]), dim3(512), 0, stream, kb, vb, rb, ka, va, ra, starts, hist + (size_t)BINS * nb, (const uint32_t *)dparams, local_cap,
+            local_incl, bucket_sums, T, ranges, watch, (uint32_t)BINS, r[3]);
     return hipGetLastError();
 }
 
 hipError_t ex4d_depth_sort_msd(uint32_t *ka, uint32_t *va, uint32_t *ra, uint32_t *kb, uint32_t *vb, uint32_t *rb, uint32_t n, uint32_t inv_key,
     uint32_t *flags, const uint2 *wave_ranges, uint32_t *hist, uint32_t *starts, uint32_t local_cap, hipStream_t stream,
-    uint32_t *local_incl, uint32_t *bucket_sums, int T, uint2 *ranges, int local_threads, uint32_t *watch, int msd_bits)
+    uint32_t *local_incl, uint32_t *bucket_sums, int T, uint2 *ranges, int local_threads, uint32_t *watch, int msd_bits, const ShRide *ride)
 {
     if (msd_bits == EX4D_DLS_MSD_BITS - 1)
-        return depth_sort_msd_launch<EX4D_DLS_MSD_BITS - 1>(ka, va, ra, kb, vb, rb, n, inv_key, flags, wave_ranges, hist, starts, local_cap, stream, local_incl, bucket_sums, T, ranges, local_threads, watch);
-    return depth_sort_msd_launch<EX4D_DLS_MSD_BITS>(ka, va, ra, kb, vb, rb, n, inv_key, flags, wave_ranges, hist, starts, local_cap, stream, local_incl, bucket_sums, T, ranges, local_threads, watch);
+        return depth_sort_msd_launch<EX4D_DLS_MSD_BITS - 1>(ka, va, ra, kb, vb, rb, n, inv_key, flags, wave_ranges, hist, starts, local_cap, stream, local_incl, bucket_sums, T, ranges, local_threads, watch, ride);
+    return depth_sort_msd_launch<EX4D_DLS_MSD_BITS>(ka, va, ra, kb, vb, rb, n, inv_key, flags, wave_ranges, hist, starts, local_cap, stream, local_incl, bucket_sums, T, ranges, local_threads, watch, ride);
 }
 
 bool ex4d_tile_sort_msd_applies(int P, int tile_bits)
@@ -1009,13 +1066,13 @@
     uint32_t *histB = hist + (size_t)256 * (nbA + 1);
     const uint32_t *totals = hist + (size_t)256 * nbA;
     hipLaunchKernelGGL((rs_histogram_kernel<RS_ITEMS, 256, 8>), dim3(nbA), dim3(RS_THREADS), 0, stream, keys, R, low_bits, (1u << high_bits) - 1u, nbA, hist, n_dev);
-    hipLaunchKernelGGL(rs_scan_rows_kernel, dim3(1u << high_bits), dim3(256), 0, stream, nbA, hist, 256u);
+    hipLaunchKernelGGL(rs_scan_rows_kernel<false>, dim3(1u << high_bits), dim3(256), 0, stream, nbA, hist, 256u, ShRide{});
 #define TS_SCATTER_A(NB) hipLaunchKernelGGL((rs_scatter_kernel<RS_ITEMS, 256, 1, NB>), dim3(nbA), dim3(RS_THREADS), 0, stream, keys, vals, packed, (uint32_t *)nullptr, \
         R, low_bits, high_bits, nbA, hist, low_bits, (const uint32_t *)nullptr, 0, (uint2 *)nullptr, n_dev)
     if (high_bits == 6) TS_SCATTER_A(6); else if (high_bits == 7) TS_SCATTER_A(7); else if (high_bits == 8) TS_SCATTER_A(8); else TS_SCATTER_A(0);
 #undef TS_SCATTER_A
     hipLaunchKernelGGL(ts_histogram_kernel, dim3(nbB), dim3(RS_THREADS), 0, stream, packed, totals, 1 << high_bits, 32 - low_bits, nbB, histB);
-    hipLaunchKernelGGL(rs_scan_rows_kernel, dim3(1u << low_bits), dim3(256), 0, stream, nbB, histB, 256u);
+    hipLaunchKernelGGL(rs_scan_rows_kernel<false>, dim3(1u << low_bits), dim3(256), 0, stream, nbB, histB, 256u, ShRide{});
 #define TS_SCATTER_B(NB) hipLaunchKernelGGL((rs_scatter_kernel<RS_ITEMS, 256, 2, NB>), dim3(nbB), dim3(RS_THREADS), 0, stream, packed, (const uint32_t *)nullptr, tile_ids_out, point_list, \
         R, 32 - low_bits, low_bits, nbB, histB, low_bits, totals, 1 << high_bits, ranges, (const uint32_t *)nullptr)
     if (low_bits == 7) TS_SCATTER_B(7); else if (low_bits == 8) TS_SCATTER_B(8); else TS_SCATTER_B(0);
@@ -1031,7 +1088,7 @@
     if (R == 0) return hipSuccess;
     const uint32_t nbB = ex4d_tile_sort_pass_b_blocks(R, nbuckets);
     hipLaunchKernelGGL(ts_histogram_kernel, dim3(nbB), dim3(RS_THREADS), 0, stream, packed, totals, nbuckets, 32 - low_bits, nbB, histB, cap, block_table);
-    hipLaunchKernelGGL(rs_scan_rows_kernel, dim3(1u << low_bits), dim3(256), 0, stream, nbB, histB, 256u);
+    hipLaunchKernelGGL(rs_scan_rows_kernel<false>, dim3(1u << low_bits), dim3(256), 0, stream, nbB, histB, 256u, ShRide{});
 #define TS_SCATTER_B(NB) hipLaunchKernelGGL((rs_scatter_kernel<RS_ITEMS, 256, 2, NB>), dim3(nbB), dim3(RS_THREADS), 0, stream, packed, (const uint32_t *)nullptr, tile_ids_out, point_list, \
         R, 32 - low_bits, low_bits, nbB, histB, low_bits, totals, nbuckets, ranges, (const uint32_t *)nullptr, (const uint32_t *)nullptr, (uint32_t *)nullptr, (uint32_t *)nullptr, \
         (const uint32_t *)nullptr, stride, cap, block_table)
diff --git a/ex4dgs_amd/csrc/ex4d_internal.h b/ex4dgs_amd/csrc/ex4d_internal.h
--- a/ex4dgs_amd/csrc/ex4d_internal.h
+++ b/ex4dgs_amd/csrc/ex4d_internal.h
@@ -63,12 +63,22 @@
 struct ShSplit { const float *dc[2]; const float *rest[2]; int n_static; };
 struct ShSplitGrad { float *dc[2]; float *rest[2]; int n_static; };
 
+struct ShRide {
+    const float *shs, *means3D, *campos;
+    const int32_t *radii;
+    float4 *records;
+    uint8_t *clamped;
+    float *sh_dsums;
+    int P, first, count;
+};
+static inline uint32_t ex4d_sh_ride_blocks(const ShRide &r, int waves) { return r.count > 0 ? (uint32_t)((r.count + waves - 1) / waves) : 0u; }
+
 hipError_t ex4d_launch_preprocess_fwd(const Ex4dParams &prm, const float *means3D, const float *dir3D, const float *scales,
     const float *rotations, const float *opacities, const float *shs, const float *cov3D_precomp,
     const float *colors_precomp, const float *viewmatrix, const float *projmatrix, const float *campos,
     int32_t *radii, GeomState g, uint32_t *prefilter_violation, ShSplit split,
     uint32_t *depth_keys, uint32_t *depth_vals, uint32_t depth_key_base, uint32_t depth_key_invisible, uint32_t *rects4, hipStream_t stream,
-    uint32_t *key_range_slots = nullptr, bool global_flags = true);
+    uint32_t *key_range_slots = nullptr, bool global_flags = true, ShRide *ride = nullptr);
 
 hipError_t ex4d_launch_mark_visible(int P, const float *means3D, const float *viewmatrix, const float *projmatrix,
     float min_depth, float max_depth, uint8_t *present, hipStream_t stream);
@@ -112,7 +122,8 @@
     uint32_t *flags, const uint2 *wave_ranges, uint32_t *hist, uint32_t *starts, uint32_t local_cap, hipStream_t stream,
     uint32_t *local_incl, uint32_t *bucket_sums, int T, uint2 *ranges, int local_threads,
     uint32_t *watch = nullptr,
-    int msd_bits = EX4D_DLS_MSD_BITS);
+    int msd_bits = EX4D_DLS_MSD_BITS,
+    const ShRide *ride = nullptr);
 int ex4d_depth_sort_msd_bits(uint32_t n, int key_bits);
 void ex4d_set_rank_lds(int v);
 int ex4d_get_rank_lds();
@@ -125,6 +136,9 @@
 int ex4d_get_preprocess_tune();
 void ex4d_set_preprocess_fast(int v);
 int ex4d_get_preprocess_fast();
+void ex4d_set_preprocess_sh_ride(int v);
+int ex4d_get_preprocess_sh_ride();
+void ex4d_sh_ride_split(int count, int out[4]);
 void ex4d_set_fwd_asm(int on);
 int ex4d_get_fwd_asm();
 void ex4d_set_clamp_always(int on);
diff --git a/ex4dgs_amd/csrc/ex4d_preprocess.hip b/ex4dgs_amd/csrc/ex4d_preprocess.hip
--- a/ex4dgs_amd/csrc/ex4d_preprocess.hip
+++ b/ex4dgs_amd/csrc/ex4d_preprocess.hip
@@ -1,16 +1,10 @@
 #include "ex4d_internal.h"
+#include "ex4d_sh_colour.h"
 #include <atomic>
 #include <cstdlib>
 #include <cstdlib>
 
 namespace {
-
-__constant__ float kSH_C0 = 0.28209479177387814f;
-__constant__ float kSH_C1 = 0.4886025119029199f;
-__constant__ float kSH_C2[5] = { 1.0925484305920792f, -1.0925484305920792f, 0.31539156525252005f,
-                                 -1.0925484305920792f, 0.5462742152960396f };
-__constant__ float kSH_C3[7] = { -0.5900435899266435f, 2.890611442640554f, -0.4570457994644658f, 0.3731763325901154f,
-                                 -0.4570457994644658f, 1.445305721320277f, -0.5900435899266435f };
 
 struct Mat3 { float m[3][3]; };
 
@@ -147,36 +141,6 @@
     cov3D[3] = Sigma.m[1][1]; cov3D[4] = Sigma.m[1][2]; cov3D[5] = Sigma.m[2][2];
 }
 
-#define SH_ROW 52
-
-__device__ __forceinline__ void wave_sync_lds()
-{
-    __builtin_amdgcn_fence(__ATOMIC_RELEASE, "wavefront");
-    __builtin_amdgcn_wave_barrier();
-    __builtin_amdgcn_fence(__ATOMIC_ACQUIRE, "wavefront");
-}
-
-struct ShPrefetch { float4 v[13]; };
-__device__ __forceinline__ bool mask_bit(uint64_t need, int g)
-{
-    const uint32_t half = (g & 32) ? (uint32_t)(need >> 32) : (uint32_t)need;
-    return ((half >> (g & 31)) & 1u) != 0u;
-}
-__device__ __forceinline__ void wave_issue_sh(const float *__restrict__ shs_wave, ShPrefetch &pf, int nrows, int nvec, int lane, uint64_t need)
-{
-    const float4 *src = reinterpret_cast<const float4 *>(shs_wave);
-    if (nrows == 64 && nvec == 12 && need == ~0ull) {
-#pragma unroll
-        for (int it = 0; it < 12; it++) pf.v[it] = src[it * 64 + lane];
-        return;
-    }
-#pragma unroll
-    for (int it = 0; it < 12; it++) {
-        const int q = it * 64 + lane;
-        const int g = q / 12, v = q - 12 * g;
-        pf.v[it] = (g < nrows && v < nvec && mask_bit(need, g)) ? src[q] : make_float4(0.f, 0.f, 0.f, 0.f);
-    }
-}
 __device__ __forceinline__ bool wave_issue_sh_split(const ShSplit &sp, int wave_first, int nrows, ShPrefetch &pf, int lane, uint64_t need)
 {
     const bool all_dynamic = wave_first >= sp.n_static, all_static = wave_first + nrows <= sp.n_static;
@@ -199,20 +163,6 @@
     }
     return true;
 }
-
-#define SH_HALF_FLOATS (32 * SH_ROW)
-#define SH_HALF_DC_OFFSET (32 * 45)
-__device__ __forceinline__ void wave_commit_sh_half(float *lds, const ShPrefetch &pf, int lane, int h)
-{
-#pragma unroll
-    for (int i = 0; i < 6; i++) {
-        const int it = 6 * h + i;
-        const int q = it * 64 + lane;
-        const int g = q / 12 - 32 * h, v = q % 12;
-        *reinterpret_cast<float4 *>(lds + g * SH_ROW + 4 * v) = pf.v[it];
-    }
-    wave_sync_lds();
-}
 __device__ __forceinline__ void wave_commit_sh_split_half(float *lds, const ShPrefetch &pf, int lane, int h)
 {
 #pragma unroll
@@ -298,58 +248,8 @@
 
 
 
-__device__ __forceinline__ void sh_direction_sums(const float *sh, int D, float x, float y, float z,
-                                                  float (&dRGBdx)[3], float (&dRGBdy)[3], float (&dRGBdz)[3])
-{
-#define SHK(k) sh[3 * (k) + ch]
-    if (D > 0) {
-#pragma unroll
-        for (int ch = 0; ch < 3; ch++) {
-            dRGBdx[ch] = -kSH_C1 * SHK(3);
-            dRGBdy[ch] = -kSH_C1 * SHK(1);
-            dRGBdz[ch] = kSH_C1 * SHK(2);
-        }
-        if (D > 1) {
-            const float xx = x * x, yy = y * y, zz = z * z, xy = x * y, yz = y * z, xz = x * z;
-#pragma unroll
-            for (int ch = 0; ch < 3; ch++) {
-                dRGBdx[ch] += kSH_C2[0] * y * SHK(4) + kSH_C2[2] * 2.f * -x * SHK(6) + kSH_C2[3] * z * SHK(7) + kSH_C2[4] * 2.f * x * SHK(8);
-                dRGBdy[ch] += kSH_C2[0] * x * SHK(4) + kSH_C2[1] * z * SHK(5) + kSH_C2[2] * 2.f * -y * SHK(6) + kSH_C2[4] * 2.f * -y * SHK(8);
-                dRGBdz[ch] += kSH_C2[1] * y * SHK(5) + kSH_C2[2] * 2.f * 2.f * z * SHK(6) + kSH_C2[3] * x * SHK(7);
-            }
-            if (D > 2) {
-#pragma unroll
-                for (int ch = 0; ch < 3; ch++) {
-                    dRGBdx[ch] += (
-                        kSH_C3[0] * SHK(9) * 3.f * 2.f * xy +
-                        kSH_C3[1] * SHK(10) * yz +
-                        kSH_C3[2] * SHK(11) * -2.f * xy +
-                        kSH_C3[3] * SHK(12) * -3.f * 2.f * xz +
-                        kSH_C3[4] * SHK(13) * (-3.f * xx + 4.f * zz - yy) +
-                        kSH_C3[5] * SHK(14) * 2.f * xz +
-                        kSH_C3[6] * SHK(15) * 3.f * (xx - yy));
-                    dRGBdy[ch] += (
-                        kSH_C3[0] * SHK(9) * 3.f * (xx - yy) +
-                        kSH_C3[1] * SHK(10) * xz +
-                        kSH_C3[2] * SHK(11) * (-3.f * yy + 4.f * zz - xx) +
-                        kSH_C3[3] * SHK(12) * -3.f * 2.f * yz +
-                        kSH_C3[4] * SHK(13) * -2.f * xy +
-                        kSH_C3[5] * SHK(14) * -2.f * yz +
-                        kSH_C3[6] * SHK(15) * -3.f * 2.f * xy);
-                    dRGBdz[ch] += (
-                        kSH_C3[1] * SHK(10) * xy +
-                        kSH_C3[2] * SHK(11) * 4.f * 2.f * yz +
-                        kSH_C3[3] * SHK(12) * 3.f * (2.f * zz - xx - yy) +
-                        kSH_C3[4] * SHK(13) * 4.f * 2.f * xz +
-                        kSH_C3[5] * SHK(14) * (xx - yy));
-                }
-            }
-        }
-    }
-#undef SHK
-}
-
-template <bool FAST>
+
+template <bool FAST, bool COLOUR = true>
 __global__ __launch_bounds__(256) void preprocess_fwd_kernel(
     int P, int D_, int M_,
     const float *__restrict__ means3D, const float *__restrict__ dir3D, const float *__restrict__ scales, float scale_modifier,
@@ -369,7 +269,8 @@
     const float *__restrict__ colors_precomp = FAST ? nullptr : colors_precomp_;
     ShSplit sp = sp_;
     if (FAST) { sp.dc[0] = sp.dc[1] = sp.rest[0] = sp.rest[1] = nullptr; sp.n_static = 0; __builtin_assume(shs != nullptr); }
-    __shared__ __attribute__((aligned(16))) float sh_lds[4 * SH_HALF_FLOATS];
+    static_assert(FAST || COLOUR, "the geometry half exists for the FAST input combination only");
+    __shared__ __attribute__((aligned(16))) float sh_lds[COLOUR ? 4 * SH_HALF_FLOATS : 4];
     const int lane = threadIdx.x & 63, wave = threadIdx.x >> 6;
     __shared__ uint32_t s_kr[4];
     if (key_range_slots) {
@@ -386,7 +287,7 @@
 
     const int ncoef = (D + 1) * (D + 1);
     const bool split = sp.rest[0] != nullptr || sp.rest[1] != nullptr;
-    const bool staged = (shs != nullptr || split) && (M == 16);
+    const bool staged = COLOUR && (shs != nullptr || split) && (M == 16);
     const int wave_first = wc * 64;
     const int wave_rows = (P - wave_first) < 64 ? (P - wave_first) : 64;
     ShPrefetch pf;
@@ -502,7 +403,8 @@
         }
     }
     float coefv[16][3];
-    if (staged) {
+    if (!COLOUR) {
+    } else if (staged) {
         float *lds = sh_lds + wave * SH_HALF_FLOATS;
         float tmp[48];
 #pragma unroll
@@ -554,45 +456,15 @@
             for (int ch = 0; ch < 3; ch++) coefv[k][ch] = (k < ncoef && k < M) ? sh[3 * k + ch] : 0.f;
     }
     if (visible) {
-        float res[3];
-        if (colors_precomp) {
+        float res[3] = { 0.f, 0.f, 0.f };
+        if (!COLOUR) {
+        } else if (colors_precomp) {
             res[0] = colors_precomp[3 * (size_t)idx]; res[1] = colors_precomp[3 * (size_t)idx + 1]; res[2] = colors_precomp[3 * (size_t)idx + 2];
         } else {
             float dx = p.x - campos[0], dy = p.y - campos[1], dz = p.z - campos[2];
             const float len = sqrtf(dx * dx + dy * dy + dz * dz);
             const float x = dx / len, y = dy / len, z = dz / len;
-            uint8_t clamp_bits = 0;
-#pragma unroll
-            for (int ch = 0; ch < 3; ch++) {
-#define SHK(k) coefv[k][ch]
-                float result = kSH_C0 * SHK(0);
-                if (D > 0) {
-                    result = result - kSH_C1 * y * SHK(1) + kSH_C1 * z * SHK(2) - kSH_C1 * x * SHK(3);
-                    if (D > 1) {
-                        const float xx = x * x, yy = y * y, zz = z * z, xy = x * y, yz = y * z, xz = x * z;
-                        result = result +
-                            kSH_C2[0] * xy * SHK(4) +
-                            kSH_C2[1] * yz * SHK(5) +
-                            kSH_C2[2] * (2.0f * zz - xx - yy) * SHK(6) +
-                            kSH_C2[3] * xz * SHK(7) +
-                            kSH_C2[4] * (xx - yy) * SHK(8);
-                        if (D > 2) {
-                            result = result +
-                                kSH_C3[0] * y * (3.0f * xx - yy) * SHK(9) +
-                                kSH_C3[1] * xy * z * SHK(10) +
-                                kSH_C3[2] * y * (4.0f * zz - xx - yy) * SHK(11) +
-                                kSH_C3[3] * z * (2.0f * zz - 3.0f * xx - 3.0f * yy) * SHK(12) +
-                                kSH_C3[4] * x * (4.0f * zz - xx - yy) * SHK(13) +
-                                kSH_C3[5] * z * (xx - yy) * SHK(14) +
-                                kSH_C3[6] * x * (xx - 3.0f * yy) * SHK(15);
-                        }
-                    }
-                }
-#undef SHK
-                result += 0.5f;
-                if (result < 0) clamp_bits |= (uint8_t)(1u << ch);
-                res[ch] = fmaxf(result, 0.0f);
-            }
+            const uint8_t clamp_bits = sh_eval_rgb(coefv, D, x, y, z, res);
             clamped[idx] = clamp_bits;
             if (sh_dsums) {
                 float dRGBdx[3] = { 0, 0, 0 }, dRGBdy[3] = { 0, 0, 0 }, dRGBdz[3] = { 0, 0, 0 };
@@ -610,7 +482,8 @@
         float4 *rec = records + 4 * (size_t)idx;
         rec[0] = make_float4(pix_x, pix_y, conic.x, conic.y);
         rec[1] = make_float4(conic.z, tau, -conic.y / conic.z, -conic.y / conic.x);
-        rec[2] = make_float4(depth, res[0], res[1], res[2]);
+        if (COLOUR) rec[2] = make_float4(depth, res[0], res[1], res[2]);
+        else reinterpret_cast<float *>(rec + 2)[0] = depth;
         rec[3] = make_float4(in_d0, in_d1, in_d2, w_op);
     }
     const bool chunk_flow = __ballot(visible && (in_d0 != 0.f || in_d1 != 0.f || in_d2 != 0.f)) != 0ull;
@@ -631,6 +504,12 @@
 #pragma unroll
     for (int o = 32; o > 0; o >>= 1) { wave_sum += __shfl_xor(wave_sum, o, 64); wave_seg += __shfl_xor(wave_seg, o, 64); }
     if (lane == 0) reinterpret_cast<uint2 *>(total_instances)[wc] = make_uint2(wave_sum, wave_seg | (chunk_flow ? EX4D_CHUNK_FLOW : 0u) | (chunk_filtered ? EX4D_CHUNK_FILTERED : 0u));
+}
+
+__global__ __launch_bounds__(256) void sh_colour_kernel(const ShRide r)
+{
+    __shared__ __attribute__((aligned(16))) unsigned char smem[4 * SH_RIDE_SLICE_BYTES];
+    sh_ride_block(r, (int)blockIdx.x, 4, smem);
 }
 
 __global__ __launch_bounds__(256) void mark_visible_kernel(int P, const float *__restrict__ means3D,
@@ -950,6 +829,9 @@
 static std::atomic<int> g_preprocess_fast{1};
 void ex4d_set_preprocess_fast(int v) { g_preprocess_fast.store(v); }
 int ex4d_get_preprocess_fast() { return g_preprocess_fast.load(); }
+static std::atomic<int> g_preprocess_sh_ride{0};
+void ex4d_set_preprocess_sh_ride(int v) { g_preprocess_sh_ride.store(v); }
+int ex4d_get_preprocess_sh_ride() { return g_preprocess_sh_ride.load(); }
 static std::atomic<int> g_preprocess_tune{preprocess_option_default()};
 void ex4d_set_preprocess_tune(int v) { g_preprocess_tune.store(v != 0); }
 int ex4d_get_preprocess_tune() { return g_preprocess_tune.load(); }
@@ -959,8 +841,9 @@
     const float *colors_precomp, const float *viewmatrix, const float *projmatrix, const float *campos,
     int32_t *radii, GeomState g, uint32_t *prefilter_violation, ShSplit split,
     uint32_t *depth_keys, uint32_t *depth_vals, uint32_t depth_key_base, uint32_t depth_key_invisible, uint32_t *rects4, hipStream_t stream,
-    uint32_t *key_range_slots, bool global_flags)
-{
+    uint32_t *key_range_slots, bool global_flags, ShRide *ride)
+{
+    if (ride) ride->count = 0;
     const float fy = prm.H / (2.0f * prm.tanfovy);
     const float fx = prm.W / (2.0f * prm.tanfovx);
     const bool is_split = split.rest[0] != nullptr || split.rest[1] != nullptr;
@@ -972,7 +855,15 @@
         radii, g.records, g.cov3D, g.clamped, g.tiles_touched, g.rects, depth_keys, depth_vals, depth_key_base, depth_key_invisible, g.block_totals, split, \
         (prm.prepare_backward && (shs != nullptr || is_split)) ? g.sh_dsums : (float *)nullptr, \
         g_preprocess_tune.load(std::memory_order_relaxed), rects4, key_range_slots, global_flags ? 1 : 0
-    if (fast) hipLaunchKernelGGL(preprocess_fwd_kernel<true>, dim3((prm.P + 255) / 256), dim3(256), 0, stream, PF_ARGS);
+    const int ride_opt = g_preprocess_sh_ride.load(std::memory_order_relaxed);
+    const bool riding = fast && ride_opt == 1 && ride != nullptr && key_range_slots != nullptr;
+    if (fast && prm.P > 0 && (riding || ride_opt == 2)) {
+        hipLaunchKernelGGL((preprocess_fwd_kernel<true, false>), dim3((prm.P + 255) / 256), dim3(256), 0, stream, PF_ARGS);
+        ShRide r = { shs, means3D, campos, radii, g.records, g.clamped, prm.prepare_backward ? g.sh_dsums : (float *)nullptr, prm.P, 0, (prm.P + 63) / 64 };
+        if (riding) *ride = r;
+        else hipLaunchKernelGGL(sh_colour_kernel, dim3(ex4d_sh_ride_blocks(r, 4)), dim3(256), 0, stream, r);
+    }
+    else if (fast) hipLaunchKernelGGL(preprocess_fwd_kernel<true>, dim3((prm.P + 255) / 256), dim3(256), 0, stream, PF_ARGS);
     else hipLaunchKernelGGL(preprocess_fwd_kernel<false>, dim3((prm.P + 255) / 256), dim3(256), 0, stream, PF_ARGS);
 #undef PF_ARGS
     return hipGetLastError();
diff --git a/ex4dgs_amd/csrc/ex4d_sh_colour.h b/ex4dgs_amd/csrc/ex4d_sh_colour.h
--- /dev/null
+++ b/ex4dgs_amd/csrc/ex4d_sh_colour.h
@@ -0,0 +1,212 @@
+#pragma once
+#include "ex4d_internal.h"
+
+namespace {
+
+__constant__ float kSH_C0 = 0.28209479177387814f;
+__constant__ float kSH_C1 = 0.4886025119029199f;
+__constant__ float kSH_C2[5] = { 1.0925484305920792f, -1.0925484305920792f, 0.31539156525252005f,
+                                 -1.0925484305920792f, 0.5462742152960396f };
+__constant__ float kSH_C3[7] = { -0.5900435899266435f, 2.890611442640554f, -0.4570457994644658f, 0.3731763325901154f,
+                                 -0.4570457994644658f, 1.445305721320277f, -0.5900435899266435f };
+
+#define SH_ROW 52
+
+__device__ __forceinline__ void wave_sync_lds()
+{
+    __builtin_amdgcn_fence(__ATOMIC_RELEASE, "wavefront");
+    __builtin_amdgcn_wave_barrier();
+    __builtin_amdgcn_fence(__ATOMIC_ACQUIRE, "wavefront");
+}
+
+struct ShPrefetch { float4 v[13]; };
+__device__ __forceinline__ bool mask_bit(uint64_t need, int g)
+{
+    const uint32_t half = (g & 32) ? (uint32_t)(need >> 32) : (uint32_t)need;
+    return ((half >> (g & 31)) & 1u) != 0u;
+}
+__device__ __forceinline__ void wave_issue_sh(const float *__restrict__ shs_wave, ShPrefetch &pf, int nrows, int nvec, int lane, uint64_t need)
+{
+    const float4 *src = reinterpret_cast<const float4 *>(shs_wave);
+    if (nrows == 64 && nvec == 12 && need == ~0ull) {
+#pragma unroll
+        for (int it = 0; it < 12; it++) pf.v[it] = src[it * 64 + lane];
+        return;
+    }
+    if (nrows == 64 && nvec == 12) {
+#pragma unroll
+        for (int it = 0; it < 12; it++) {
+            const int q = it * 64 + lane;
+            pf.v[it] = mask_bit(need, q / 12) ? src[q] : make_float4(0.f, 0.f, 0.f, 0.f);
+        }
+        return;
+    }
+#pragma unroll
+    for (int it = 0; it < 12; it++) {
+        const int q = it * 64 + lane;
+        const int g = q / 12, v = q - 12 * g;
+        pf.v[it] = (g < nrows && v < nvec && mask_bit(need, g)) ? src[q] : make_float4(0.f, 0.f, 0.f, 0.f);
+    }
+}
+
+#define SH_HALF_FLOATS (32 * SH_ROW)
+#define SH_HALF_DC_OFFSET (32 * 45)
+__device__ __forceinline__ void wave_commit_sh_half(float *lds, const ShPrefetch &pf, int lane, int h)
+{
+#pragma unroll
+    for (int i = 0; i < 6; i++) {
+        const int it = 6 * h + i;
+        const int q = it * 64 + lane;
+        const int g = q / 12 - 32 * h, v = q % 12;
+        *reinterpret_cast<float4 *>(lds + g * SH_ROW + 4 * v) = pf.v[it];
+    }
+    wave_sync_lds();
+}
+
+__device__ __forceinline__ uint8_t sh_eval_rgb(const float (&coefv)[16][3], int D, float x, float y, float z, float (&res)[3])
+{
+#pragma clang fp contract(off)
+    uint8_t clamp_bits = 0;
+#pragma unroll
+    for (int ch = 0; ch < 3; ch++) {
+#define SHK(k) coefv[k][ch]
+        float result = kSH_C0 * SHK(0);
+        if (D > 0) {
+            result = result - kSH_C1 * y * SHK(1) + kSH_C1 * z * SHK(2) - kSH_C1 * x * SHK(3);
+            if (D > 1) {
+                const float xx = x * x, yy = y * y, zz = z * z, xy = x * y, yz = y * z, xz = x * z;
+                result = result +
+                    kSH_C2[0] * xy * SHK(4) +
+                    kSH_C2[1] * yz * SHK(5) +
+                    kSH_C2[2] * (2.0f * zz - xx - yy) * SHK(6) +
+                    kSH_C2[3] * xz * SHK(7) +
+                    kSH_C2[4] * (xx - yy) * SHK(8);
+                if (D > 2) {
+                    result = result +
+                        kSH_C3[0] * y * (3.0f * xx - yy) * SHK(9) +
+                        kSH_C3[1] * xy * z * SHK(10) +
+                        kSH_C3[2] * y * (4.0f * zz - xx - yy) * SHK(11) +
+                        kSH_C3[3] * z * (2.0f * zz - 3.0f * xx - 3.0f * yy) * SHK(12) +
+                        kSH_C3[4] * x * (4.0f * zz - xx - yy) * SHK(13) +
+                        kSH_C3[5] * z * (xx - yy) * SHK(14) +
+                        kSH_C3[6] * x * (xx - 3.0f * yy) * SHK(15);
+                }
+            }
+        }
+#undef SHK
+        result += 0.5f;
+        if (result < 0) clamp_bits |= (uint8_t)(1u << ch);
+        res[ch] = fmaxf(result, 0.0f);
+    }
+    return clamp_bits;
+}
+
+__device__ __forceinline__ void sh_direction_sums(const float *sh, int D, float x, float y, float z,
+                                                  float (&dRGBdx)[3], float (&dRGBdy)[3], float (&dRGBdz)[3])
+{
+#pragma clang fp contract(off)
+#define SHK(k) sh[3 * (k) + ch]
+    if (D > 0) {
+#pragma unroll
+        for (int ch = 0; ch < 3; ch++) {
+            dRGBdx[ch] = -kSH_C1 * SHK(3);
+            dRGBdy[ch] = -kSH_C1 * SHK(1);
+            dRGBdz[ch] = kSH_C1 * SHK(2);
+        }
+        if (D > 1) {
+            const float xx = x * x, yy = y * y, zz = z * z, xy = x * y, yz = y * z, xz = x * z;
+#pragma unroll
+            for (int ch = 0; ch < 3; ch++) {
+                dRGBdx[ch] += kSH_C2[0] * y * SHK(4) + kSH_C2[2] * 2.f * -x * SHK(6) + kSH_C2[3] * z * SHK(7) + kSH_C2[4] * 2.f * x * SHK(8);
+                dRGBdy[ch] += kSH_C2[0] * x * SHK(4) + kSH_C2[1] * z * SHK(5) + kSH_C2[2] * 2.f * -y * SHK(6) + kSH_C2[4] * 2.f * -y * SHK(8);
+                dRGBdz[ch] += kSH_C2[1] * y * SHK(5) + kSH_C2[2] * 2.f * 2.f * z * SHK(6) + kSH_C2[3] * x * SHK(7);
+            }
+            if (D > 2) {
+#pragma unroll
+                for (int ch = 0; ch < 3; ch++) {
+                    dRGBdx[ch] += (
+                        kSH_C3[0] * SHK(9) * 3.f * 2.f * xy +
+                        kSH_C3[1] * SHK(10) * yz +
+                        kSH_C3[2] * SHK(11) * -2.f * xy +
+                        kSH_C3[3] * SHK(12) * -3.f * 2.f * xz +
+                        kSH_C3[4] * SHK(13) * (-3.f * xx + 4.f * zz - yy) +
+                        kSH_C3[5] * SHK(14) * 2.f * xz +
+                        kSH_C3[6] * SHK(15) * 3.f * (xx - yy));
+                    dRGBdy[ch] += (
+                        kSH_C3[0] * SHK(9) * 3.f * (xx - yy) +
+                        kSH_C3[1] * SHK(10) * xz +
+                        kSH_C3[2] * SHK(11) * (-3.f * yy + 4.f * zz - xx) +
+                        kSH_C3[3] * SHK(12) * -3.f * 2.f * yz +
+                        kSH_C3[4] * SHK(13) * -2.f * xy +
+                        kSH_C3[5] * SHK(14) * -2.f * yz +
+                        kSH_C3[6] * SHK(15) * -3.f * 2.f * xy);
+                    dRGBdz[ch] += (
+                        kSH_C3[1] * SHK(10) * xy +
+                        kSH_C3[2] * SHK(11) * 4.f * 2.f * yz +
+                        kSH_C3[3] * SHK(12) * 3.f * (2.f * zz - xx - yy) +
+                        kSH_C3[4] * SHK(13) * 4.f * 2.f * xz +
+                        kSH_C3[5] * SHK(14) * (xx - yy));
+                }
+            }
+        }
+    }
+#undef SHK
+}
+
+#define SH_RIDE_SLICE_BYTES (SH_HALF_FLOATS * 4)
+__device__ __forceinline__ void sh_colour_chunk(const ShRide &r, int chunk, float *lds, int lane)
+{
+#pragma clang fp contract(off)
+    const int idx = chunk * 64 + lane;
+    const bool visible = idx < r.P && r.radii[idx] > 0;
+    const uint64_t need = __ballot(visible);
+    if (need == 0ull) return;
+    const int wave_first = chunk * 64;
+    const int wave_rows = (r.P - wave_first) < 64 ? (r.P - wave_first) : 64;
+    ShPrefetch pf;
+    wave_issue_sh(r.shs + (size_t)wave_first * 48, pf, wave_rows, 12, lane, need);
+    float3 p = make_float3(0.f, 0.f, 0.f);
+    if (visible) p = make_float3(r.means3D[3 * (size_t)idx], r.means3D[3 * (size_t)idx + 1], r.means3D[3 * (size_t)idx + 2]);
+    float coefv[16][3];
+    {
+        float tmp[48];
+        const int row_in_half = lane & 31;
+#pragma unroll
+        for (int h = 0; h < 2; h++) {
+            wave_commit_sh_half(lds, pf, lane, h);
+            if (h == 0 || lane >= 32) {
+                const float4 *row = reinterpret_cast<const float4 *>(lds + row_in_half * SH_ROW);
+#pragma unroll
+                for (int v = 0; v < 12; v++) { const float4 t4 = row[v]; tmp[4 * v] = t4.x; tmp[4 * v + 1] = t4.y; tmp[4 * v + 2] = t4.z; tmp[4 * v + 3] = t4.w; }
+            }
+            wave_sync_lds();
+        }
+#pragma unroll
+        for (int k = 0; k < 16; k++) { coefv[k][0] = tmp[3 * k]; coefv[k][1] = tmp[3 * k + 1]; coefv[k][2] = tmp[3 * k + 2]; }
+    }
+    if (!visible) return;
+    float dx = p.x - r.campos[0], dy = p.y - r.campos[1], dz = p.z - r.campos[2];
+    const float len = sqrtf(dx * dx + dy * dy + dz * dz);
+    const float x = dx / len, y = dy / len, z = dz / len;
+    float res[3];
+    r.clamped[idx] = sh_eval_rgb(coefv, 3, x, y, z, res);
+    if (r.sh_dsums) {
+        float dRGBdx[3] = { 0, 0, 0 }, dRGBdy[3] = { 0, 0, 0 }, dRGBdz[3] = { 0, 0, 0 };
+        sh_direction_sums(&coefv[0][0], 3, x, y, z, dRGBdx, dRGBdy, dRGBdz);
+        float *o = r.sh_dsums + 9 * (size_t)idx;
+#pragma unroll
+        for (int ch = 0; ch < 3; ch++) { o[ch] = dRGBdx[ch]; o[3 + ch] = dRGBdy[ch]; o[6 + ch] = dRGBdz[ch]; }
+    }
+    float *rgb = reinterpret_cast<float *>(r.records + 4 * (size_t)idx + 2) + 1;
+    rgb[0] = res[0]; rgb[1] = res[1]; rgb[2] = res[2];
+}
+
+__device__ __forceinline__ void sh_ride_block(const ShRide &r, int rb, int waves, unsigned char *smem)
+{
+    const int lane = threadIdx.x & 63, wave = threadIdx.x >> 6;
+    const int c = rb * waves + wave;
+    if (c >= r.count) return;
+    sh_colour_chunk(r, r.first + c, reinterpret_cast<float *>(smem) + wave * SH_HALF_FLOATS, lane);
+}
+
+}
```

Result: slower. 0.6622 ms/frame (+1.1%).
